# RaduAlexandru/permuto_sdf

Measured on AMD Instinct MI355X. Metric: ray-samples/sec (encode+MLP+composite), higher is better.
Workload: dtype f32 (MLP products on 2 fp16 operand pieces per fp32 value, fp32 accumulation; the 3-piece / 24-bit figure is value_fp32_equivalent_24bit)

## Files before the change

include/psdf.h:

```cpp
#ifndef PSDF_H
#define PSDF_H
#include <stdint.h>
#ifdef __cplusplus
extern "C" {
#endif

int64_t psdf_encode_convention(int which);
int psdf_encode_set_conventions(uint32_t hash_multiplier, int rank_tie_raises_later);

int psdf_encode_set_forward_pairs(int pairs);

int psdf_encode_forward(int pos_dim, int nr_feat, int64_t N, int nr_levels, int capacity, const float* positions,
    const float* lattice, const float* scale_factor, const float* shifts, const float* window, int concat_points,
    float points_scaling, float* sliced, void* stream);

int psdf_encode_forward_mark(int pos_dim, int nr_feat, int64_t N, int nr_levels, int capacity, const float* positions,
    const float* lattice, const float* scale_factor, const float* shifts, const float* window, int concat_points,
    float points_scaling, float* sliced, unsigned char* touched_blocks, int block_rows_log2, void* stream);

int psdf_encode_backward(int pos_dim, int nr_feat, int64_t N, int nr_levels, int capacity, const float* positions,
    const float* lattice, const float* scale_factor, const float* shifts, const float* window, int concat_points,
    float points_scaling, const float* grad_sliced, float* grad_lattice, float* grad_positions, void* stream);

int64_t psdf_encode_backward_workspace_bytes(int pos_dim, int nr_feat, int64_t N, int nr_levels, int capacity);
int psdf_encode_backward_ws(int pos_dim, int nr_feat, int64_t N, int nr_levels, int capacity, const float* positions,
    const float* lattice, const float* scale_factor, const float* shifts, const float* window, int concat_points,
    float points_scaling, const float* grad_sliced, float* grad_lattice, float* grad_positions, void* workspace,
    int64_t workspace_bytes, void* stream);
int psdf_encode_backward_level_shares(int* counts, int max_levels);


int psdf_encode_double_backward(int pos_dim, int nr_feat, int64_t N, int nr_levels, int capacity, const float*
    positions, const float* lattice, const float* scale_factor, const float* shifts, const float* window, int
    concat_points, float points_scaling, const float* dd_positions, const float* grad_sliced, float* grad_lattice,
    float* grad_grad_sliced, void* stream);
int psdf_encode_double_backward_ws(int pos_dim, int nr_feat, int64_t N, int nr_levels, int capacity, const float* positions,
                                   const float* lattice, const float* scale_factor, const float* shifts, const float* window,
                                   int concat_points, float points_scaling, const float* dd_positions, const float* grad_sliced,
                                   float* grad_lattice, float* grad_grad_sliced, const float* grad_sliced_direct,
                                   void* workspace, int64_t workspace_bytes, void* stream);

int psdf_mlp_pack_f16(int n_layers, const int* dims, const float* const* weights, const float* const* biases, float* packed,
    void* stream);
int psdf_mlp_forward_f16(int n_layers, const int* dims, int64_t N, const float* X, const float* packed, float* Y, void* stream);

int psdf_mlp_forward_set_form(int waves);
int psdf_mlp_forward_last_form(void);

int psdf_neus_composite_forward(int nr_rays, const int* start_end, int equal, int fixed, int max_nr_samples, const float* sdf,
    const float* dirs, const float* gradients, const float* dt, const float* rgb, const float* inv_s, float cos_anneal_ratio,
    float* pred, float* bg, float* weights, void* stream);
int psdf_neus_composite_backward(int nr_rays, const int* start_end, int equal, int fixed, int max_nr_samples, int max_per_ray,
    const float* grad_pred, const float* grad_bg, const float* sdf, const float* dirs, const float* gradients, const float* dt,
    const float* rgb, const float* inv_s, float cos_anneal_ratio, int reference_compat, float* grad_sdf, float* grad_gradients,
    float* grad_rgb, float* grad_inv_s, void* stream);

int psdf_nerf_composite_forward(int nr_rays, const int* start_end, int equal, int fixed, int max_nr_samples, const float* raw_density,
                                const float* dt, const float* rgb, const float* fg_pred, const float* fg_bg, float* pred_bg,
                                float* pred, void* stream);
int psdf_nerf_composite_backward(int nr_rays, const int* start_end, int equal, int fixed, int max_nr_samples, int max_per_ray,
                                 const float* grad_pred, const float* fg_bg, const float* raw_density, const float* dt,
                                 const float* rgb, int reference_compat, float* grad_raw_density, float* grad_rgb,
                                 float* grad_fg_bg, void* stream);

int psdf_last_path(int family);
enum {
  PSDF_MLP_OP_FORWARD = 0,
  PSDF_MLP_OP_FORWARD_F16 = 1,
  PSDF_MLP_OP_FORWARD_WIDE_F16 = 2,
  PSDF_MLP_OP_BACKWARD = 3,
  PSDF_MLP_OP_BACKWARD_DATA = 4,
  PSDF_MLP_OP_BACKWARD_DATA_MASKED = 5,
  PSDF_MLP_OP_DOUBLE_BACKWARD = 6,
  PSDF_MLP_OP_DOUBLE_BACKWARD_PLUS = 7
};
int psdf_mlp_supported(int op, int n_layers, const int* dims);

int psdf_mlp_backward_split(int n_layers, const int* dims, int64_t N, const float* X, const float* const* weights,
    const float* const* biases, const float* dY, float* dX, float* const* dW, float* const* db, void* stream);

int psdf_mlp_backward_split_f16(int n_layers, const int* dims, int64_t N, const float* X, const float* const* weights,
    const float* const* biases, const float* dY, float* dX, float* const* dW, float* const* db, void* stream);
int psdf_mlp_backward_split_f16_form(void);
unsigned psdf_mlp_f16_range_events(void);

int psdf_mlp_forward_wide_f16(int n_layers, const int* dims, int64_t N, const float* X, const float* const* weights,
    const float* const* biases, float* Y, void* stream);
int psdf_mlp_backward_wide_form(void);
int psdf_mlp_backward_wide(int n_layers, const int* dims, int64_t N, const float* X, const float* const* weights,
    const float* const* biases, const float* dY, float* dX, float* const* dW, float* const* db, void* stream);

int psdf_lipshitz_normalize_forward(int out, int in, const float* W, const float* c, float* Wn, void* stream);
int psdf_lipshitz_normalize_backward(int out, int in, const float* W, const float* c, const float* grad_Wn, float* grad_W,
    float* grad_c, void* stream);
int psdf_lipshitz_normalize_forward_multi(int n_layers, const int* out, const int* in, const float* const* W, const float* const* c,
                                          float* const* Wn, void* stream);
int psdf_lipshitz_normalize_backward_multi(int n_layers, const int* out, const int* in, const float* const* W, const float* const* c,
                                           const float* const* grad_Wn, float* const* grad_W, float* const* grad_c, void* stream);

int psdf_neus_alpha_forward(int64_t N, const float* sdf, const float* dirs, const float* gradients, const float* dt,
    const float* inv_s, float cos_anneal_ratio, float* alpha, float* one_minus_alpha, void* stream);
int psdf_neus_alpha_backward(int64_t N, const float* grad_alpha, const float* sdf, const float* dirs, const float*
    gradients, const float* dt, const float* inv_s, float cos_anneal_ratio, float* grad_sdf, float* grad_gradients,
    float* grad_inv_s, void* stream);
int psdf_l1_loss(int64_t R, int C, const float* pred, const float* gt, const unsigned char* mask, float scale,
    float* loss, float* grad_pred, void* stream);
int psdf_eikonal_loss(int64_t N, const float* gradients, float scale, float* loss, float* grad_gradients, void* stream);
int psdf_normalize3(int64_t N, const float* x, const float* grad_y, float* out, void* stream);
int psdf_sigmoid_rows(int64_t N, int C, const float* x_fm, float* y, void* stream);
int psdf_sigmoid_rows_backward(int64_t N, int C, const float* grad_y, const float* y, float* grad_x_fm, void* stream);
int psdf_curvature_shift(int64_t N, const float* points, const float* gradients, const float* rand_directions, float
    epsilon, const float* grad_shifted, float* out, void* stream);
int psdf_curvature_loss(int64_t N, const float* gradients, const float* gradients_shifted, float scale, float* loss,
    float* grad_gradients, float* grad_gradients_shifted, void* stream);
int psdf_offsurface_loss(int64_t N, const float* sdf, float sharpness, float scale, float* loss, float* grad_sdf, void*
    stream);
int psdf_nerf_alpha_forward(int64_t N, const float* raw_density, const float* dt, float* alpha, float* one_minus_alpha,
    void* stream);
int psdf_nerf_alpha_backward(int64_t N, const float* raw_density, const float* dt, const float* grad_alpha, const float*
    grad_one_minus_alpha, float* grad_raw_density, void* stream);

int64_t psdf_mlp_packed_size(int n_layers, const int* dims);

int psdf_mlp_pack(int n_layers, const int* dims, const float* const* weights, const float* const* biases, float*
    packed, void* stream);

int psdf_mlp_forward(int n_layers, const int* dims, int64_t N, const float* X, const float* packed, float* Y, void*
    stream);

int psdf_encode_forward_masked(int pos_dim, int nr_feat, int64_t N, int nr_levels, int capacity, const float* positions,
    const float* lattice, const float* scale_factor, const float* shifts, const float* window, int concat_points, float
    points_scaling, const uint8_t* skip, float* sliced, void* stream);
int psdf_mlp_forward_masked(int n_layers, const int* dims, int64_t N, const float* X, const float* packed, const uint8_t*
    skip, float* Y, void* stream);
int psdf_mlp_backward_data_masked(int n_layers, const int* dims, int64_t N, const float* X, const float* const* weights,
    const float* const* biases, const float* dY, const uint8_t* skip, float* dX, void* stream);
int psdf_encode_backward_positions_masked(int pos_dim, int nr_feat, int64_t N, int nr_levels, int capacity, const float*
    positions, const float* lattice, const float* scale_factor, const float* shifts, const float* window, int
    concat_points, float points_scaling, const float* grad_sliced, const uint8_t* skip, float* grad_positions, void*
    stream);

int psdf_mlp_backward(int n_layers, const int* dims, int64_t N, const float* X, const float* const* weights, const
    float* const* biases, const float* dY, float* dX, float* const* dW, float* const* db, void* stream);

int psdf_mlp_double_backward(int n_layers, const int* dims, int64_t N, const float* X, const float* const* weights,
    const float* const* biases, const float* dY, const float* V, float* dX2, float* const* dW, float* const* db,
    void* stream);
int psdf_mlp_double_backward_plus(int n_layers, const int* dims, int64_t N, const float* X, const float* const* weights,
    const float* const* biases, const float* dY, const float* V, const float* dY2, float* dX2, float* const* dW,
    float* const* db, void* stream);

int psdf_encode_mlp_forward(int64_t N, int nr_levels, int capacity, const float* positions, const float* lattice,
    const float* scale_factor, const float* shifts, const float* window, int concat_points, float points_scaling,
    int n_layers, const int* dims, const float* packed, const uint8_t* skip, float* feat, float* Y, void* stream);

int psdf_adamw_step(int64_t n, float* param, const float* grad, float* exp_avg, float* exp_avg_sq, float lr, float
    beta1, float beta2, float eps, float weight_decay, int step, float grad_scale, void* stream);

int psdf_adamw_step_multi(int n_tensors, const int64_t* sizes, float* const* params, const float* const* grads, float*
    const* exp_avgs, float* const* exp_avg_sqs, float lr, float beta1, float beta2, float eps, float weight_decay, int
    step, float grad_scale, void* stream);

int psdf_adamw_step_blocks(int64_t n_blocks, int block_elems, float* param, float* grad, float* exp_avg, float*
    exp_avg_sq, unsigned char* touched, unsigned char* active, float lr, float beta1, float beta2, float eps, int step,
    float grad_scale, int zero_grad, void* stream);
int psdf_adamw_step_blocks_multi(int n_tensors, const int64_t* n_blocks, const int* block_elems, float* const* params,
    float* const* grads, float* const* exp_avgs, float* const* exp_avg_sqs, unsigned char* const* touched,
// ... 219 lines not shown
```

permuto_sdf_amd/csrc/composite_fused.hip:

```cpp
#include <type_traits>

#include "composite_device.h"

using namespace psdf;

namespace {

__global__ void __launch_bounds__(PSDF_BLOCK)
    neus_composite_fwd_kernel(int nr_rays, RayIndex ri, const float* __restrict__ sdf, const float* __restrict__ dirs,
                              const float* __restrict__ gradients, const float* __restrict__ dt, const float* __restrict__ rgb,
                              const float* __restrict__ inv_s_ptr, float cos_anneal_ratio, float* __restrict__ pred,
                              float* __restrict__ bg, float* __restrict__ weights) {
  const int lane = lane_id();
  const float inv_s = inv_s_ptr[0];
  RAY_LOOP(ray, nr_rays) {
    int s, e;
    ri.get(ray, s, e);
    if (!ri.valid(s, e)) {
      if (lane == 0) {
        pred[3 * ray] = pred[3 * ray + 1] = pred[3 * ray + 2] = 0.f;
        if (bg) bg[ray] = 1.f;
      }
      continue;
    }
    float r = 0.f, g = 0.f, b = 0.f;
    const float T_bg = sweep(
        s, e - s, lane,
        [&](int64_t m) {
          return clip01(section(sdf[m], ld3(dirs + 3 * m), ld3(gradients + 3 * m), dt[m], inv_s, cos_anneal_ratio).q);
        },
        [&](int64_t m, float a, float T) {
          const float w = a * T;
          if (weights) weights[m] = w;
          r += w * rgb[3 * m];
          g += w * rgb[3 * m + 1];
          b += w * rgb[3 * m + 2];
        });
    r = wave_sum(r);
    g = wave_sum(g);
    b = wave_sum(b);
    if (lane == 0) {
      pred[3 * ray] = r;
      pred[3 * ray + 1] = g;
      pred[3 * ray + 2] = b;
      if (bg) bg[ray] = T_bg;
    }
  }
}

template <int K>
__global__ void __launch_bounds__(PSDF_BLOCK)
    neus_composite_bwd_kernel(int nr_rays, RayIndex ri, const float* __restrict__ g_pred, const float* __restrict__ g_bg,
                              const float* __restrict__ sdf, const float* __restrict__ dirs, const float* __restrict__ gradients,
                              const float* __restrict__ dt, const float* __restrict__ rgb, const float* __restrict__ inv_s_ptr,
                              float cos_anneal_ratio, int compat, float* __restrict__ g_sdf, float* __restrict__ g_gradients,
                              float* __restrict__ g_rgb, float* __restrict__ g_inv_s) {
  const int lane = lane_id();
  const float inv_s = inv_s_ptr[0], rr = cos_anneal_ratio;
  float gs_acc = 0.f;
  RAY_LOOP(ray, nr_rays) {
    int s, e;
    ri.get(ray, s, e);
    if (!ri.valid(s, e)) continue;
    const int n = e - s;
    if (n > 64 * K) {
      poison_ray(s, n, lane, [&](int64_t m, float bad) {
        g_sdf[m] = bad;
        if (g_rgb) g_rgb[3 * m] = g_rgb[3 * m + 1] = g_rgb[3 * m + 2] = bad;
        if (g_gradients) st3(g_gradients + 3 * m, mk3(bad, bad, bad));
      });
      continue;
    }
    const float gx = g_pred[3 * ray], gy = g_pred[3 * ray + 1], gz = g_pred[3 * ray + 2];
    float a_[K], T_[K], gw_[K], v_[K];
    Transmittance tr;
#pragma unroll
    for (int k = 0; k < K; k++) {
      a_[k] = T_[k] = gw_[k] = v_[k] = 0.f;
      if (64 * k >= n) continue;
      const Sample c = sweep_chunk(tr, s, n, 64 * k, lane, [&](int64_t m) {
        return clip01(section(sdf[m], ld3(dirs + 3 * m), ld3(gradients + 3 * m), dt[m], inv_s, rr).q);
      });
      if (c.in) {
        const float cx = rgb[3 * c.m], cy = rgb[3 * c.m + 1], cz = compat ? cy : rgb[3 * c.m + 2];
        const float w = c.a * c.T;
        const float gw = gx * cx + gy * cy + gz * cz;
        if (g_rgb) {
          g_rgb[3 * c.m] = gx * w;
          g_rgb[3 * c.m + 1] = gy * w;
          g_rgb[3 * c.m + 2] = gz * w;
        }
        a_[k] = c.a;
        T_[k] = c.T;
        gw_[k] = gw;
        v_[k] = (gw * c.a) * c.T;
      }
    }
    const float gb = (g_bg ? g_bg[ray] : 0.f) * tr.carry;
    SuffixStep sfx;
#pragma unroll
    for (int k = K - 1; k >= 0; k--) {
      if (64 * k >= n) continue;
      const int i = 64 * k + lane;
      const float g_om = sfx.g_one_minus(v_[k], a_[k], &gb, i, n, lane);
      if (i < n) {
        const int64_t m = s + i;
        const float g_alpha = gw_[k] * T_[k] - g_om;
        const v3 dir = ld3(dirs + 3 * m);
        const float d = dt[m];
        const Section sc = section(sdf[m], dir, ld3(gradients + 3 * m), d, inv_s, rr);
        const SectionGrad sg = section_backward(sc, g_alpha, d, inv_s, rr);
        gs_acc += sg.g_inv_s;
        g_sdf[m] = sg.g_sdf;
        if (g_gradients) st3(g_gradients + 3 * m, sg.g_tc * dir);
      }
    }
  }
  if (g_inv_s) {
    gs_acc = wave_sum(gs_acc);
    if (lane == 0 && gs_acc != 0.f) atomicAdd(g_inv_s, gs_acc);
  }
}

__global__ void __launch_bounds__(PSDF_BLOCK)
    nerf_composite_fwd_kernel(int nr_rays, RayIndex ri, const float* __restrict__ raw, const float* __restrict__ dt,
                              const float* __restrict__ rgb, const float* __restrict__ fg_pred, const float* __restrict__ fg_bg,
                              float* __restrict__ pred_bg, float* __restrict__ pred) {
  const int lane = lane_id();
  RAY_LOOP(ray, nr_rays) {
    int s, e;
    ri.get(ray, s, e);
    float r = 0.f, g = 0.f, b = 0.f;
    if (ri.valid(s, e)) {
      sweep(
          s, e - s, lane, [&](int64_t m) { return nerf_alpha(raw[m], dt[m]).a; },
          [&](int64_t m, float a, float T) {
            const float w = a * T;
            r += w * rgb[3 * m];
            g += w * rgb[3 * m + 1];
            b += w * rgb[3 * m + 2];
          });
      r = wave_sum(r);
      g = wave_sum(g);
      b = wave_sum(b);
    }
    if (lane == 0) {
      pred_bg[3 * ray] = r;
      pred_bg[3 * ray + 1] = g;
      pred_bg[3 * ray + 2] = b;
      if (pred) {
        const float t = fg_bg[ray];
        pred[3 * ray] = fg_pred[3 * ray] + t * r;
        pred[3 * ray + 1] = fg_pred[3 * ray + 1] + t * g;
        pred[3 * ray + 2] = fg_pred[3 * ray + 2] + t * b;
      }
    }
  }
}

template <int K>
__global__ void __launch_bounds__(PSDF_BLOCK)
    nerf_composite_bwd_kernel(int nr_rays, RayIndex ri, const float* __restrict__ g_pred, const float* __restrict__ fg_bg,
                              const float* __restrict__ raw, const float* __restrict__ dt, const float* __restrict__ rgb,
                              int compat, float* __restrict__ g_raw, float* __restrict__ g_rgb, float* __restrict__ g_fg_bg) {
  const int lane = lane_id();
  RAY_LOOP(ray, nr_rays) {
    int s, e;
    ri.get(ray, s, e);
    const float t = fg_bg ? fg_bg[ray] : 1.f;
    const float ux = g_pred[3 * ray], uy = g_pred[3 * ray + 1], uz = g_pred[3 * ray + 2];
    if (!ri.valid(s, e)) {
      if (g_fg_bg && lane == 0) g_fg_bg[ray] = 0.f;
      continue;
    }
    const int n = e - s;
    if (n > 64 * K) {
      poison_ray(s, n, lane, [&](int64_t m, float bad) {
        g_raw[m] = bad;
        g_rgb[3 * m] = g_rgb[3 * m + 1] = g_rgb[3 * m + 2] = bad;
      });
      if (g_fg_bg && lane == 0) g_fg_bg[ray] = poison();
      continue;
    }
    const float gx = t * ux, gy = t * uy, gz = t * uz;
    float a_[K], T_[K], gw_[K], v_[K], e_[K];
    float ex, pr = 0.f, pg = 0.f, pb = 0.f;
    Transmittance tr;
#pragma unroll
    for (int k = 0; k < K; k++) {
      a_[k] = T_[k] = gw_[k] = v_[k] = e_[k] = 0.f;
      if (64 * k >= n) continue;
      const Sample c = sweep_chunk(tr, s, n, 64 * k, lane, [&](int64_t m) {
        const NerfAlpha o = nerf_alpha(raw[m], dt[m]);
        ex = o.e;
        return o.a;
      });
      if (c.in) {
        const float cx = rgb[3 * c.m], cy = rgb[3 * c.m + 1], cz_true = rgb[3 * c.m + 2];
        const float cz = compat ? cy : cz_true;
        const float w = c.a * c.T;
        pr += w * cx;
        pg += w * cy;
        pb += w * cz_true;
// ... 4 lines not shown
        a_[k] = c.a;
        T_[k] = c.T;
        gw_[k] = gw;
        e_[k] = ex;
        v_[k] = (gw * c.a) * c.T;
      }
    }
    if (g_fg_bg) {
      pr = wave_sum(pr);
      pg = wave_sum(pg);
      pb = wave_sum(pb);
      if (lane == 0) g_fg_bg[ray] = (ux * pr + uy * pg) + uz * pb;
    }
    SuffixStep sfx;
#pragma unroll
    for (int k = K - 1; k >= 0; k--) {
      if (64 * k >= n) continue;
      const int i = 64 * k + lane;
      const float g_om = sfx.g_one_minus(v_[k], a_[k], nullptr, i, n, lane);
      if (i < n) {
        const int64_t m = s + i;
        const float g_alpha = gw_[k] * T_[k] - g_om;
        g_raw[m] = nerf_alpha_backward(g_alpha, e_[k], raw[m], dt[m]);
      }
    }
  }
}

template <int V>
using int_c = std::integral_constant<int, V>;
template <class Fn>
void dispatch_chunks(int max_per_ray, Fn&& fn) {
  if (max_per_ray <= 64) return fn(int_c<1>{});
  if (max_per_ray <= 128) return fn(int_c<2>{});
  return fn(int_c<4>{});
}

}

extern "C" {

int psdf_nerf_composite_forward(int nr_rays, const int* start_end, int equal, int fixed, int max_nr_samples, const float* raw_density,
                                const float* dt, const float* rgb, const float* fg_pred, const float* fg_bg, float* pred_bg,
                                float* pred, void* stream) {
  if (nr_rays <= 0) return PSDF_OK;
  if (!raw_density || !dt || !rgb || !pred_bg || (!equal && !start_end) || ((fg_pred || fg_bg || pred) && !(fg_pred && fg_bg && pred)))
    return PSDF_ERR_ARG;
  hipLaunchKernelGGL(nerf_composite_fwd_kernel, dim3(ray_grid(nr_rays)), dim3(PSDF_BLOCK), 0, (hipStream_t)stream, nr_rays,
                     RayIndex{start_end, equal, fixed, max_nr_samples}, raw_density, dt, rgb, fg_pred, fg_bg, pred_bg, pred);
  PSDF_LAUNCH_CHECK();
  return PSDF_OK;
}

int psdf_nerf_composite_backward(int nr_rays, const int* start_end, int equal, int fixed, int max_nr_samples, int max_per_ray,
                                 const float* grad_pred, const float* fg_bg, const float* raw_density, const float* dt,
                                 const float* rgb, int reference_compat, float* grad_raw_density, float* grad_rgb,
                                 float* grad_fg_bg, void* stream) {
  if (nr_rays <= 0) return PSDF_OK;
  if (!grad_pred || !raw_density || !dt || !rgb || !grad_raw_density || !grad_rgb || (!equal && !start_end) || max_per_ray < 1)
    return PSDF_ERR_ARG;
  if (max_per_ray > 256) return PSDF_ERR_UNSUPPORTED;
  const RayIndex ri{start_end, equal, fixed, max_nr_samples};
  dispatch_chunks(max_per_ray, [&](auto k) {
    hipLaunchKernelGGL(nerf_composite_bwd_kernel<decltype(k)::value>, dim3(ray_grid(nr_rays)), dim3(PSDF_BLOCK), 0,
                       (hipStream_t)stream, nr_rays, ri, grad_pred, fg_bg, raw_density, dt, rgb, reference_compat,
                       grad_raw_density, grad_rgb, grad_fg_bg);
  });
  PSDF_LAUNCH_CHECK();
  return PSDF_OK;
}

int psdf_neus_composite_forward(int nr_rays, const int* start_end, int equal, int fixed, int max_nr_samples, const float* sdf,
                                const float* dirs, const float* gradients, const float* dt, const float* rgb, const float* inv_s,
                                float cos_anneal_ratio, float* pred, float* bg, float* weights, void* stream) {
  if (nr_rays <= 0) return PSDF_OK;
  if (!sdf || !dirs || !gradients || !dt || !rgb || !inv_s || !pred || (!equal && !start_end)) return PSDF_ERR_ARG;
  hipLaunchKernelGGL(neus_composite_fwd_kernel, dim3(ray_grid(nr_rays)), dim3(PSDF_BLOCK), 0, (hipStream_t)stream, nr_rays,
                     RayIndex{start_end, equal, fixed, max_nr_samples}, sdf, dirs, gradients, dt, rgb, inv_s, cos_anneal_ratio,
                     pred, bg, weights);
  PSDF_LAUNCH_CHECK();
  return PSDF_OK;
}

int psdf_neus_composite_backward(int nr_rays, const int* start_end, int equal, int fixed, int max_nr_samples, int max_per_ray,
                                 const float* grad_pred, const float* grad_bg, const float* sdf, const float* dirs,
                                 const float* gradients, const float* dt, const float* rgb, const float* inv_s,
                                 float cos_anneal_ratio, int reference_compat, float* grad_sdf, float* grad_gradients,
                                 float* grad_rgb, float* grad_inv_s, void* stream) {
  if (nr_rays <= 0) return PSDF_OK;
  if (!grad_pred || !sdf || !dirs || !gradients || !dt || !rgb || !inv_s || !grad_sdf || (!equal && !start_end) || max_per_ray < 1)
    return PSDF_ERR_ARG;
  if (max_per_ray > 256) return PSDF_ERR_UNSUPPORTED;
  const RayIndex ri{start_end, equal, fixed, max_nr_samples};
  dispatch_chunks(max_per_ray, [&](auto k) {
    hipLaunchKernelGGL(neus_composite_bwd_kernel<decltype(k)::value>, dim3(ray_grid(nr_rays)), dim3(PSDF_BLOCK), 0,
                       (hipStream_t)stream, nr_rays, ri, grad_pred, grad_bg, sdf, dirs, gradients, dt, rgb, inv_s,
                       cos_anneal_ratio, reference_compat, grad_sdf, grad_gradients, grad_rgb, grad_inv_s);
  });
  PSDF_LAUNCH_CHECK();
  return PSDF_OK;
}

}
```

permuto_sdf_amd/csrc/mlp.hip:

```cpp
#include "psdf_common.h"
#include <type_traits>

#include "mlp_device.h"
#include "mlp_dispatch.h"

namespace {

struct PackArgs {
  MlpPlan plan;
  const float* W[MAXL];
  const float* b[MAXL];
};

__global__ void mlp_pack_kernel(PackArgs a, float* __restrict__ packed) {
  const int e = blockIdx.x * blockDim.x + threadIdx.x;
  const MlpPlan& p = a.plan;
  if (e >= p.total) return;
  int l = 0;
#pragma unroll
  for (int i = 1; i < MAXL; i++)
    if (i < p.n_layers && e >= p.w_off[i]) l = i;
  const int out_d = p.dims[l + 1], in_d = p.dims[l];
  const bool last = (l == p.n_layers - 1);
  float v = 0.f;
  if (e >= p.b_off[l]) {
    const int row = e - p.b_off[l];
    if (row < out_d) v = a.b[l][row];
  } else {
    const int q = e - p.w_off[l];
    int row, col;
    if (l == 0) {
      const int lane = q % WS, s = (q / WS) % p.in_steps0, to = (q / WS) / p.in_steps0;
      row = (lane < 64) ? 32 * to + (lane & 31) : (1 << 20);
      col = 2 * s + (lane >> 5);
    } else if (last && p.final_dot) {
      const int h = q & 1, r = (q >> 1) & 15, ti = (q >> 5) % p.tiles[l], o = (q >> 5) / p.tiles[l];
      row = o;
      col = 32 * ti + row_of(r, h);
    } else {
      const int j = q & 3, lane = (q >> 2) & 63, rq = (q >> 8) & 3, pr = q >> 10;
      const int r = 4 * rq + j, ti = pr % p.tiles[l], to = pr / p.tiles[l];
      row = 32 * to + (lane & 31);
      col = 32 * ti + row_of(r, lane >> 5);
    }
    if (row < out_d && col < in_d) v = a.W[l][(int64_t)row * in_d + col];
  }
  packed[e] = v;
}

__global__ void mlp_pack_split_kernel(PackArgs a, SplitPlan sp, float* __restrict__ packed, int f16) {
  const int w = blockIdx.x * blockDim.x + threadIdx.x;
  const MlpPlan& p = a.plan;
  if (w >= sp.total_rec * 4) return;
  uint32_t* dst = reinterpret_cast<uint32_t*>(packed + sp.base);
  const int nl = p.n_layers;
  const int rec = w >> 2;
  if (rec >= sp.tail_rec) {
    const int f = w - sp.tail_rec * 4;
    float v = 0.f;
    for (int l = 0; l < nl; l++) {
      const bool dot = (l == nl - 1) && p.final_dot;
      const int nb = dot ? 4 : p.tiles[l + 1] * 32;
      if (f >= sp.b_off[l] && f < sp.b_off[l] + nb) {
        const int row = f - sp.b_off[l];
        if (row < p.dims[l + 1]) v = a.b[l][row];
      }
      if (dot && f >= sp.wf_off && f < sp.wf_off + p.dims[nl] * p.tiles[l] * 32) {
        const int q = f - sp.wf_off;
        const int h = q & 1, r = (q >> 1) & 15, ti = (q >> 5) % p.tiles[l], o = (q >> 5) / p.tiles[l];
        const int col = 32 * ti + row_of(r, h);
        if (col < p.dims[l]) v = a.W[l][(int64_t)o * p.dims[l] + col];
      }
    }
    dst[w] = __float_as_uint(v);
    return;
  }
  int l = 0;
  for (int i = 1; i < nl; i++) {
    const bool dot = (i == nl - 1) && p.final_dot;
    if (!dot && rec >= sp.w_rec[i]) l = i;
  }
  const int local = rec - sp.w_rec[l];
  const int lane = local & 63, piece = (local >> 6) % 3, s = (local / 192) % sp.ns[l], to = (local / 192) / sp.ns[l];
  const int row = 32 * to + (lane & 31), hh = lane >> 5;
  uint32_t out = 0;
  for (int e = 0; e < 2; e++) {
    const int j = 2 * (w & 3) + e;
    const int col = l == 0 ? 16 * s + 8 * hh + j : 32 * (s >> 1) + row_of(8 * (s & 1) + j, hh);
    float v = 0.f;
    if (row < p.dims[l + 1] && col < p.dims[l]) v = a.W[l][(int64_t)row * p.dims[l] + col];
    uint32_t pc[3];
    if (f16) split2h_bits(v, pc);
    else split3(v, pc);
    out |= pc[piece] << (16 * e);
  }
  dst[w] = out;
}

template <int T1, int T2, int T3>
struct Net {
  static constexpr int NH = (T3 > 0) ? 3 : 2;
  static constexpr int TL = (T3 > 0) ? T3 : T2;
};

template <int T1, int T2, int T3, int OUT_T, bool FINAL_DOT>
__global__ void __launch_bounds__(PSDF_BLOCK, 2)
    mlp_fwd_kernel(MlpPlan p, int64_t N, const float* __restrict__ X, const float* __restrict__ packed,
                   const unsigned char* __restrict__ skip, float* __restrict__ Y) {
  extern __shared__ __align__(16) float lds[];
  for (int i = threadIdx.x; i < p.total; i += PSDF_BLOCK) lds[i] = packed[i];
  __syncthreads();
  const int lane = threadIdx.x & 63, wave = __builtin_amdgcn_readfirstlane((int)(threadIdx.x >> 6));
  const int h = lane >> 5, sl = lane & 31;
  const int K0 = p.dims[0];
  const int OUT = p.dims[p.n_layers];
  const int64_t ntiles = (N + 31) / 32;
  for (int64_t tile = (int64_t)blockIdx.x * 4 + wave; tile < ntiles; tile += (int64_t)gridDim.x * 4) {
    asm volatile("" ::: "memory");
    const int64_t n = tile * 32 + sl;
    const int64_t nc = n < N ? n : N - 1;
    if (skip && __ballot(n < N && !skip[nc]) == 0) continue;
    f32x16 h1[T1];
    init_bias<T1>(h1, lds + p.b_off[0], h);
    {
      const float* __restrict__ w0 = lds + p.w_off[0];
      const int steps = p.in_steps0;
      constexpr int XC = 16;
      for (int s0 = 0; s0 < steps; s0 += XC) {
        float xb[XC];
#pragma unroll
        for (int i = 0; i < XC; i++) {
          const int k = 2 * (s0 + i) + h;
          xb[i] = (s0 + i < steps && k < K0) ? X[(int64_t)k * N + nc] : 0.f;
        }
#pragma unroll
        for (int i = 0; i < XC; i++) {
          if (s0 + i < steps) {
#pragma unroll
            for (int to = 0; to < T1; to++)
              h1[to] = __builtin_amdgcn_mfma_f32_32x32x2f32(w0[(to * steps + s0 + i) * WS + lane], xb[i], h1[to], 0, 0, 0);
          }
        }
      }
    }
    apply_gelu<T1>(h1);
    f32x16 h2[T2];
    init_bias<T2>(h2, lds + p.b_off[1], h);
    dense_chain<T1, T2>(h1, h2, lds + p.w_off[1], lane);
    apply_gelu<T2>(h2);
    constexpr int TL = (T3 > 0) ? T3 : T2;
    f32x16 hl[TL];
    if constexpr (T3 > 0) {
      init_bias<T3>(hl, lds + p.b_off[2], h);
      dense_chain<T2, T3>(h2, hl, lds + p.w_off[2], lane);
      apply_gelu<T3>(hl);
    } else {
#pragma unroll
      for (int t = 0; t < T2; t++) hl[t] = h2[t];
    }
    const int lf = p.n_layers - 1;
    if constexpr (FINAL_DOT) {
      const float* __restrict__ wf = lds + p.w_off[lf];
      for (int o = 0; o < OUT; o++) {
        float acc = 0.f;
#pragma unroll
        for (int ti = 0; ti < TL; ti++)
#pragma unroll
          for (int r = 0; r < 16; r++) acc = fmaf(wf[((o * TL + ti) * 16 + r) * 2 + h], hl[ti][r], acc);
        acc += __shfl_xor(acc, 32, 64);
        acc += lds[p.b_off[lf] + o];
        if (h == 0 && n < N) Y[(int64_t)o * N + n] = acc;
      }
    } else {
      f32x16 y[OUT_T];
      init_bias<OUT_T>(y, lds + p.b_off[lf], h);
      dense_chain<TL, OUT_T>(hl, y, lds + p.w_off[lf], lane);
      if (n < N) {
#pragma unroll
        for (int to = 0; to < OUT_T; to++)
// ... 260 lines not shown
    return PSDF_ERR_UNSUPPORTED;
}

template <int T1, int T2, int T3, int OUT_T, bool FINAL_DOT, int CH, bool F16 = false>
int launch_fwd_split_ch(const MlpPlan& p, const SplitPlan& sp, int64_t N, const float* X, const float* packed,
                     const unsigned char* skip, float* Y, hipStream_t st) {
  constexpr bool WIDE = split_wide_built<T1, T2, T3, OUT_T, FINAL_DOT, SPLIT_WIDE_W>;
  int form = g_fwd_form_forced;
  if (form == 0) {
    const int64_t ntiles = (N + 31) / 32;
    form = WIDE && ntiles >= (int64_t)SPLIT_WIDE_MIN_TILES_PER_CU * mlp_device_cus() ? SPLIT_WIDE_W : 4;
  }
  if (form == 4)
    return launch_fwd_split_form<4, mlp_fwd_split_kernel<T1, T2, T3, OUT_T, FINAL_DOT, CH, F16>>(p, sp, N, X, packed, skip, Y, st);
  if (form == 8) return launch_fwd_split_wide<T1, T2, T3, OUT_T, FINAL_DOT, CH, F16, 8>(p, sp, N, X, packed, skip, Y, st);
  return launch_fwd_split_wide<T1, T2, T3, OUT_T, FINAL_DOT, CH, F16, 16>(p, sp, N, X, packed, skip, Y, st);
}

template <int T1, int T2, int T3, int OUT_T, bool FINAL_DOT>
int launch_fwd_split(const MlpPlan& p, const SplitPlan& sp, int64_t N, const float* X, const float* packed,
                     const unsigned char* skip, float* Y, hipStream_t st, bool f16 = false) {
  if constexpr (T1 == 2 && T2 == 2 && T3 == 2 && OUT_T == 1 && FINAL_DOT) {
    if (f16) {
      switch (sp.ns[0]) {
        case 1: return launch_fwd_split_ch<T1, T2, T3, OUT_T, FINAL_DOT, 1, true>(p, sp, N, X, packed, skip, Y, st);
        case 2: return launch_fwd_split_ch<T1, T2, T3, OUT_T, FINAL_DOT, 2, true>(p, sp, N, X, packed, skip, Y, st);
        case 3: return launch_fwd_split_ch<T1, T2, T3, OUT_T, FINAL_DOT, 3, true>(p, sp, N, X, packed, skip, Y, st);
        default: return launch_fwd_split_ch<T1, T2, T3, OUT_T, FINAL_DOT, 4, true>(p, sp, N, X, packed, skip, Y, st);
      }
    }
  } else if (f16) {
    return PSDF_ERR_UNSUPPORTED;
  }
  switch (sp.ns[0]) {
    case 1: return launch_fwd_split_ch<T1, T2, T3, OUT_T, FINAL_DOT, 1>(p, sp, N, X, packed, skip, Y, st);
    case 2: return launch_fwd_split_ch<T1, T2, T3, OUT_T, FINAL_DOT, 2>(p, sp, N, X, packed, skip, Y, st);
    case 3: return launch_fwd_split_ch<T1, T2, T3, OUT_T, FINAL_DOT, 3>(p, sp, N, X, packed, skip, Y, st);
    default: return launch_fwd_split_ch<T1, T2, T3, OUT_T, FINAL_DOT, 4>(p, sp, N, X, packed, skip, Y, st);
  }
}

template <int T1, int T2, int T3, int OUT_T, bool FINAL_DOT>
int launch_fwd(const MlpPlan& p, int64_t N, const float* X, const float* packed, const unsigned char* skip, float* Y,
               hipStream_t st) {
  const size_t shmem = (size_t)p.total * sizeof(float);
  auto kern = mlp_fwd_kernel<T1, T2, T3, OUT_T, FINAL_DOT>;
  if (!fwd_fits(p)) return PSDF_ERR_UNSUPPORTED;
  if (shmem > 64 * 1024) {
    hipError_t e = hipFuncSetAttribute((const void*)kern, hipFuncAttributeMaxDynamicSharedMemorySize, (int)shmem);
    if (e != hipSuccess) return (int)e;
  }
  const int64_t ntiles = (N + 31) / 32;
  int64_t blocks = (ntiles + 3) / 4;
  const int64_t cap = 256 * 4;
  if (blocks > cap) blocks = cap;
  hipLaunchKernelGGL(kern, dim3((unsigned)blocks), dim3(PSDF_BLOCK), shmem, st, p, N, X, packed, skip, Y);
  PSDF_LAUNCH_CHECK();
  return PSDF_OK;
}


}

extern "C" {

int64_t psdf_mlp_packed_size(int n_layers, const int* dims) {
  MlpPlan p;
  if (make_plan(n_layers, dims, p) != PSDF_OK) return PSDF_ERR_ARG;
  SplitPlan sp;
  make_split_plan(p, sp);
  return sp.ok ? (int64_t)sp.base + (int64_t)sp.total_rec * 4 : (int64_t)p.total;
}

static int mlp_pack_impl(int n_layers, const int* dims, const float* const* weights, const float* const* biases,
                         float* packed, void* stream, int f16) {
  PackArgs a;
  int rc = make_plan(n_layers, dims, a.plan);
  if (rc != PSDF_OK) return rc;
  if (f16 && !baseline_split_shape(n_layers, dims, 64, 4)) return PSDF_ERR_UNSUPPORTED;
  for (int l = 0; l < MAXL; l++) {
    a.W[l] = l < n_layers ? weights[l] : nullptr;
    a.b[l] = l < n_layers ? biases[l] : nullptr;
  }
  hipLaunchKernelGGL(mlp_pack_kernel, dim3(psdf_blocks(a.plan.total, 256)), dim3(256), 0, (hipStream_t)stream, a,
                     packed);
  PSDF_LAUNCH_CHECK();
  SplitPlan sp;
  make_split_plan(a.plan, sp);
  if (sp.ok) {
    hipLaunchKernelGGL(mlp_pack_split_kernel, dim3(psdf_blocks(sp.total_rec * 4, 256)), dim3(256), 0,
                       (hipStream_t)stream, a, sp, packed, f16);
    PSDF_LAUNCH_CHECK();
  } else if (f16) {
    return PSDF_ERR_UNSUPPORTED;
  }
  return PSDF_OK;
}

int psdf_mlp_pack(int n_layers, const int* dims, const float* const* weights, const float* const* biases,
                  float* packed, void* stream) {
  return mlp_pack_impl(n_layers, dims, weights, biases, packed, stream, 0);
}

int psdf_mlp_pack_f16(int n_layers, const int* dims, const float* const* weights, const float* const* biases,
                      float* packed, void* stream) {
  return mlp_pack_impl(n_layers, dims, weights, biases, packed, stream, 1);
}

static int mlp_forward_impl(int n_layers, const int* dims, int64_t N, const float* X, const float* packed,
                            const unsigned char* skip, float* Y, void* stream, bool f16 = false) {
  MlpPlan p;
  int rc = make_plan(n_layers, dims, p);
  if (rc != PSDF_OK) return rc;
  if (N == 0) return PSDF_OK;
  if (N < 0 || !X || !packed || !Y) return PSDF_ERR_ARG;
  hipStream_t st = (hipStream_t)stream;
  const int t1 = p.tiles[1], t2 = p.tiles[2], t3 = (n_layers == 4) ? p.tiles[3] : 0, to = p.tiles[n_layers];
  if (n_layers != 3 && n_layers != 4) return PSDF_ERR_UNSUPPORTED;
  if (f16 && !baseline_split_shape(n_layers, dims, 64, 4)) return PSDF_ERR_UNSUPPORTED;
  SplitPlan sp;
  make_split_plan(p, sp);
#define CASE(A, B, C, O, D, FWD, S, F16)                                        \
  PSDF_IF(FWD, if (t1 == A && t2 == B && t3 == C && to == O && p.final_dot == D) { \
    if (f16 && !F16) return PSDF_ERR_UNSUPPORTED;                               \
    if constexpr (S) {                                                          \
      if (sp.ok) {                                                              \
        psdf::g_last_path[psdf::PATH_MLP_FWD] = f16 ? 3 : 2;                    \
        return launch_fwd_split<A, B, C, O, D>(p, sp, N, X, packed, skip, Y, st, f16); \
      }                                                                         \
    }                                                                           \
    if (f16) return PSDF_ERR_UNSUPPORTED;                                       \
    psdf::g_last_path[psdf::PATH_MLP_FWD] = 1;                                  \
    return launch_fwd<A, B, C, O, D>(p, N, X, packed, skip, Y, st);             \
  })
  PSDF_MLP32_ROWS(CASE)
#undef CASE
  return PSDF_ERR_UNSUPPORTED;
}


int psdf_mlp_forward(int n_layers, const int* dims, int64_t N, const float* X, const float* packed, float* Y,
                     void* stream) {
  return mlp_forward_impl(n_layers, dims, N, X, packed, nullptr, Y, stream);
}

int psdf_mlp_forward_f16(int n_layers, const int* dims, int64_t N, const float* X, const float* packed, float* Y,
                         void* stream) {
  return mlp_forward_impl(n_layers, dims, N, X, packed, nullptr, Y, stream, true);
}

int psdf_mlp_forward_masked(int n_layers, const int* dims, int64_t N, const float* X, const float* packed,
                            const unsigned char* skip, float* Y, void* stream) {
  return mlp_forward_impl(n_layers, dims, N, X, packed, skip, Y, stream);
}

int psdf_mlp_forward_set_form(int waves) {
  if (waves != 0 && waves != 4 && waves != 8 && waves != 16) return PSDF_ERR_ARG;
  g_fwd_form_forced = waves;
  return PSDF_OK;
}

int psdf_mlp_forward_last_form(void) { return g_fwd_form_last; }

}
```

permuto_sdf_amd/csrc/mlp_bwd.hip:

```cpp
#include <cstdlib>
#include "mlp_device.h"
#include "mlp_dispatch.h"
#include <mutex>
#include <vector>

#define PSDF_MLP_BWD_SPLIT_DEFAULT 2
namespace psdf {
int g_last_path[PATH_FAMILIES] = {};
void* stream_scratch(size_t bytes, hipStream_t st) {
  hipStreamCaptureStatus cs = hipStreamCaptureStatusNone;
  if (hipStreamIsCapturing(st, &cs) != hipSuccess || cs != hipStreamCaptureStatusNone) {
    (void)hipGetLastError();
    return nullptr;
  }
  int dev = 0;
  if (hipGetDevice(&dev) != hipSuccess) return nullptr;
  struct Entry {
    hipStream_t st;
    int dev;
    void* ptr;
    size_t cap;
  };
  static std::mutex mu;
  static std::vector<Entry> entries;
// ... 1060 lines not shown
template <int TI0, int T1, int T2, int T3, int OUT_T, bool FINAL_DOT, bool WITH_DW, int NW_>
int launch_bwd_nw(const Plan16& p, int64_t N, const float* X, const float* dY, float* dX, const BwdPtrs& a, hipStream_t st) {
  constexpr int NW = NW_;
  const int64_t ntiles = (N + 15) / 16;
  int64_t blocks = (ntiles + NW - 1) / NW;
  if (blocks > 256) blocks = 256;
  if (!a.dW[0]) {
    if (!dX) return PSDF_OK;
    const size_t shmem = bwd_lds_bytes<TI0, T1, T2, T3, OUT_T, FINAL_DOT>(p, BW, 2);
    if (shmem > MLP_LDS_MAX) return PSDF_ERR_UNSUPPORTED;
    auto kern = mlp_bwd_kernel<TI0, T1, T2, T3, OUT_T, FINAL_DOT, true, false, BW>;
    hipError_t e = hipFuncSetAttribute((const void*)kern, hipFuncAttributeMaxDynamicSharedMemorySize, (int)shmem);
    if (e != hipSuccess) return (int)e;
    int64_t nb = (ntiles + BW - 1) / BW;
    if (nb > 512) nb = 512;
    hipLaunchKernelGGL(kern, dim3((unsigned)nb), dim3(BW * 64), shmem, st, p, N, X, dY, dX, a);
    PSDF_LAUNCH_CHECK();
    return PSDF_OK;
  }
  if constexpr (!WITH_DW) {
    return PSDF_ERR_UNSUPPORTED;
  } else {
  const size_t shmem = bwd_lds_bytes<TI0, T1, T2, T3, OUT_T, FINAL_DOT>(p, NW, 2);
  if (shmem > MLP_LDS_MAX) return PSDF_ERR_UNSUPPORTED;
#define GO(DX)                                                                                                     \
  do {                                                                                                             \
    auto kern = mlp_bwd_kernel<TI0, T1, T2, T3, OUT_T, FINAL_DOT, DX, true, NW>;                                    \
    hipError_t e = hipFuncSetAttribute((const void*)kern, hipFuncAttributeMaxDynamicSharedMemorySize, (int)shmem);  \
    if (e != hipSuccess) return (int)e;                                                                            \
    hipLaunchKernelGGL(kern, dim3((unsigned)blocks), dim3(NW * 64), shmem, st, p, N, X, dY, dX, ap);                 \
  } while (0)
  BwdPtrs ap = a;
  if (!a.only_if) ap.partial = grad_scratch_alloc((size_t)blocks * p.total, st);
  if (dX)
    GO(true);
  else
    GO(false);
#undef GO
  grad_scratch_reduce(p, ap, (int)blocks, st);
  PSDF_LAUNCH_CHECK();
  return PSDF_OK;
  }
}
template <int TI0, int T1, int T2, int T3, int OUT_T, bool FINAL_DOT, bool WITH_DW = true>
int launch_bwd(const Plan16& p, int64_t N, const float* X, const float* dY, float* dX, const BwdPtrs& a, hipStream_t st) {
  if constexpr (T1 <= 2 && T2 <= 2 && T3 <= 2) {
    if (N >= ((int64_t)1 << 17)) return launch_bwd_nw<TI0, T1, T2, T3, OUT_T, FINAL_DOT, WITH_DW, 8>(p, N, X, dY, dX, a, st);
  }
  return launch_bwd_nw<TI0, T1, T2, T3, OUT_T, FINAL_DOT, WITH_DW, BW>(p, N, X, dY, dX, a, st);
}

}

namespace psdf {
size_t mlp_backward_head_redo_bytes(int64_t N) {
  const int dims[4] = {80, 64, 64, 3};
  Plan16 p;
  if (make_plan16(3, dims, p) != PSDF_OK) return 0;
  int64_t blocks = ((N + 15) / 16 + BW - 1) / BW;
  if (blocks > 256) blocks = 256;
  return ((size_t)blocks * p.total * sizeof(float) + 255) & ~(size_t)255;
}
int mlp_backward_head_redo(const int* dims, int64_t N, const float* X, const float* const* weights, const float* const* biases,
                           const float* dY, float* dX, float* const* dW, float* const* db, hipStream_t st, char* scratch,
                           const uint32_t* only_if, uint32_t token) {
  Plan16 p;
  int rc = make_plan16(3, dims, p);
  if (rc != PSDF_OK) return rc;
  if (!colour_head_shape(3, dims)) return PSDF_ERR_UNSUPPORTED;
  BwdPtrs a;
  for (int l = 0; l < MAXL; l++) {
    a.W[l] = l < 3 ? weights[l] : nullptr;
    a.b[l] = l < 3 ? biases[l] : nullptr;
    a.dW[l] = l < 3 ? dW[l] : nullptr;
    a.db[l] = l < 3 ? db[l] : nullptr;
  }
  a.partial = reinterpret_cast<float*>(scratch);
  a.only_if = only_if;
  a.only_if_token = token;
  return launch_bwd_nw<5, 4, 4, 0, 1, true, true, BW>(p, N, X, dY, dX, a, st);
}
}

#ifdef PSDF_BWD_TIMING
extern "C" int psdf_debug_bwd_timing(unsigned long long* out) {
  return (int)hipMemcpyFromSymbol(out, HIP_SYMBOL(g_bwd_t), sizeof(unsigned long long) * 8);
}
#endif

extern "C" {

int psdf_mlp_backward_split(int n_layers, const int* dims, int64_t N, const float* X, const float* const* weights,
                            const float* const* biases, const float* dY, float* dX, float* const* dW, float* const* db,
                            void* stream);
int psdf_mlp_backward_wide(int n_layers, const int* dims, int64_t N, const float* X, const float* const* weights,
                           const float* const* biases, const float* dY, float* dX, float* const* dW, float* const* db,
                           void* stream);
int psdf_mlp_backward_split_f16(int n_layers, const int* dims, int64_t N, const float* X, const float* const* weights,
                                const float* const* biases, const float* dY, float* dX, float* const* dW, float* const* db,
                                void* stream);

int psdf_mlp_backward(int n_layers, const int* dims, int64_t N, const float* X, const float* const* weights,
                      const float* const* biases, const float* dY, float* dX, float* const* dW, float* const* db,
                      void* stream) {
  Plan16 p;
  int rc = make_plan16(n_layers, dims, p);
  if (rc != PSDF_OK) return rc;
  if (N == 0) return PSDF_OK;
  if (N < 0 || !X || !weights || !biases || ((dW == nullptr) != (db == nullptr))) return PSDF_ERR_ARG;
  if (!dY && dW) return PSDF_ERR_ARG;
  if (n_layers != 3 && n_layers != 4) return PSDF_ERR_UNSUPPORTED;
  if (dW && N >= (1 << 18)) {
    const char* v = getenv("PSDF_MLP_BWD_SPLIT");
    const int which = !v ? PSDF_MLP_BWD_SPLIT_DEFAULT : (v[0] == '0' ? 0 : (v[0] == 'f' ? 2 : 1));
    if (which == 2) {
      const int r = psdf_mlp_backward_split_f16(n_layers, dims, N, X, weights, biases, dY, dX, dW, db, stream);
      if (r != PSDF_ERR_UNSUPPORTED) {
        psdf::g_last_path[psdf::PATH_MLP_BWD] = 4;
        return r;
      }
    }
    if (which != 0) {
      const int r = psdf_mlp_backward_split(n_layers, dims, N, X, weights, biases, dY, dX, dW, db, stream);
      if (r != PSDF_ERR_UNSUPPORTED) {
        psdf::g_last_path[psdf::PATH_MLP_BWD] = 2;
        return r;
      }
    }
  }
  BwdPtrs a;
  a.partial = nullptr;
  for (int l = 0; l < MAXL; l++) {
    a.W[l] = l < n_layers ? weights[l] : nullptr;
    a.b[l] = l < n_layers ? biases[l] : nullptr;
    a.dW[l] = (dW && l < n_layers) ? dW[l] : nullptr;
    a.db[l] = (db && l < n_layers) ? db[l] : nullptr;
    if (l < n_layers && (!a.W[l] || !a.b[l] || (dW && (!a.dW[l] || !a.db[l])))) return PSDF_ERR_ARG;
  }
  hipStream_t st = (hipStream_t)stream;
  const int ti0 = p.tiles[0], t1 = p.tiles[1], t2 = p.tiles[2], t3 = (n_layers == 4) ? p.tiles[3] : 0,
            to = p.tiles[n_layers];
  if (dW && dX && colour_head_shape(n_layers, dims)) {
    const int r = psdf_mlp_backward_wide(n_layers, dims, N, X, weights, biases, dY, dX, dW, db, stream);
    if (r != PSDF_ERR_UNSUPPORTED) {
      psdf::g_last_path[psdf::PATH_MLP_BWD] = 3;
      return r;
    }
  }
  psdf::g_last_path[psdf::PATH_MLP_BWD] = 1;
#define CASE(I, A, B, C, O, D, DW, DX, MASKED, DBL, PLUS)                                        \
  if (ti0 == I && t1 == A && t2 == B && t3 == C && to == O && p.final_dot == D) {               \
    if (!DX && !dW) return PSDF_ERR_UNSUPPORTED;                                                \
    if (!DW && dW) {                                                                            \
      const int r = psdf_mlp_backward_wide(n_layers, dims, N, X, weights, biases, dY, dX, dW, db, stream); \
      if (r != PSDF_ERR_UNSUPPORTED) {                                                          \
        psdf::g_last_path[psdf::PATH_MLP_BWD] = 3;                                              \
        return r;                                                                               \
      }                                                                                         \
    }                                                                                           \
    return launch_bwd<I, A, B, C, O, D, DW != 0>(p, N, X, dY, dX, a, st);                       \
  }
  PSDF_MLP16_ROWS(CASE)
#undef CASE
  psdf::g_last_path[psdf::PATH_MLP_BWD] = 3;
  if (dW) return psdf_mlp_backward_wide(n_layers, dims, N, X, weights, biases, dY, dX, dW, db, stream);
  return PSDF_ERR_UNSUPPORTED;
}

int psdf_last_path(int family) {
  if (family < 0 || family >= psdf::PATH_FAMILIES) return -1;
  return psdf::g_last_path[family];
}

int psdf_mlp_supported(int op, int n_layers, const int* dims) {
  MlpPlan p;
  Plan16 q;
  if (op < PSDF_MLP_OP_FORWARD || op > PSDF_MLP_OP_DOUBLE_BACKWARD_PLUS || !dims || make_plan(n_layers, dims, p) != PSDF_OK ||
      make_plan16(n_layers, dims, q) != PSDF_OK)
    return PSDF_ERR_ARG;
  if (op == PSDF_MLP_OP_FORWARD_WIDE_F16) return colour_net_shape(n_layers, dims) || density_net_shape(n_layers, dims);
  if (n_layers != 3 && n_layers != 4) return 0;
  if (op == PSDF_MLP_OP_FORWARD || op == PSDF_MLP_OP_FORWARD_F16) {
    const bool f16 = op == PSDF_MLP_OP_FORWARD_F16;
    if (f16 && !baseline_split_shape(n_layers, dims, 64, 4)) return 0;
    SplitPlan sp;
    make_split_plan(p, sp);
    const int t1 = p.tiles[1], t2 = p.tiles[2], t3 = (n_layers == 4) ? p.tiles[3] : 0, to = p.tiles[n_layers];
#define ROW(A, B, C, O, D, FWD, S, F16)                                                            \
    if (FWD && t1 == A && t2 == B && t3 == C && to == O && p.final_dot == D)                       \
      return (S && sp.ok) ? (!f16 || F16) : (!f16 && fwd_fits(p));
    PSDF_MLP32_ROWS(ROW)
#undef ROW
    return 0;
  }
  const int ti0 = q.tiles[0], t1 = q.tiles[1], t2 = q.tiles[2], t3 = (n_layers == 4) ? q.tiles[3] : 0, to = q.tiles[n_layers];
#define ROW(I, A, B, C, O, D, DW, DX, MASKED, DBL, PLUS)                                           \
  if (ti0 == I && t1 == A && t2 == B && t3 == C && to == O && q.final_dot == D) {                  \
    const bool bwd = bwd_lds_bytes<I, A, B, C, O, D>(q, BW, 2) <= MLP_LDS_MAX;                     \
    const bool dbl = bwd_lds_bytes<I, A, B, C, O, D>(q, BW, 4) <= MLP_LDS_MAX;                     \
    switch (op) {                                                                                  \
      case PSDF_MLP_OP_BACKWARD: return DW ? bwd : wide_backward_shape(n_layers, dims);            \
      case PSDF_MLP_OP_BACKWARD_DATA: return DX && bwd;                                            \
      case PSDF_MLP_OP_BACKWARD_DATA_MASKED: return MASKED && bwd;                                 \
      case PSDF_MLP_OP_DOUBLE_BACKWARD: return DBL && dbl;                                         \
      default: return PLUS && dbl;                                                                 \
    }                                                                                              \
  }
  PSDF_MLP16_ROWS(ROW)
#undef ROW
  return op == PSDF_MLP_OP_BACKWARD && wide_backward_shape(n_layers, dims);
}

int psdf_mlp_backward_data_masked(int n_layers, const int* dims, int64_t N, const float* X, const float* const* weights,
                                  const float* const* biases, const float* dY, const unsigned char* skip, float* dX,
                                  void* stream) {
  Plan16 p;
  int rc = make_plan16(n_layers, dims, p);
  if (rc != PSDF_OK) return rc;
  if (N == 0) return PSDF_OK;
  if (N < 0 || !X || !weights || !biases || !dX) return PSDF_ERR_ARG;
  if (n_layers != 3 && n_layers != 4) return PSDF_ERR_UNSUPPORTED;
  BwdPtrs a;
  a.partial = nullptr;
  a.skip = skip;
  for (int l = 0; l < MAXL; l++) {
    a.W[l] = l < n_layers ? weights[l] : nullptr;
    a.b[l] = l < n_layers ? biases[l] : nullptr;
    a.dW[l] = nullptr;
    a.db[l] = nullptr;
    if (l < n_layers && (!a.W[l] || !a.b[l])) return PSDF_ERR_ARG;
  }
  hipStream_t st = (hipStream_t)stream;
  const int ti0 = p.tiles[0], t1 = p.tiles[1], t2 = p.tiles[2], t3 = (n_layers == 4) ? p.tiles[3] : 0,
            to = p.tiles[n_layers];
#define CASE(I, A, B, C, O, D, DW, DX, MASKED, DBL, PLUS)                                        \
  PSDF_IF(MASKED, if (ti0 == I && t1 == A && t2 == B && t3 == C && to == O && p.final_dot == D) \
    return launch_bwd<I, A, B, C, O, D>(p, N, X, dY, dX, a, st);)
  PSDF_MLP16_ROWS(CASE)
#undef CASE
  return PSDF_ERR_UNSUPPORTED;
}

static int mlp_double_backward_impl(int n_layers, const int* dims, int64_t N, const float* X, const float* const* weights,
                                    const float* const* biases, const float* dY, const float* V, const float* dY2, float* dX2,
                                    float* const* dW, float* const* db, void* stream) {
  Plan16 p;
  int rc = make_plan16(n_layers, dims, p);
  if (rc != PSDF_OK) return rc;
  if (n_layers != 4) return PSDF_ERR_UNSUPPORTED;
// ... 40 lines not shown
```

permuto_sdf_amd/csrc/mlp_bwd_split.hip:

```cpp
#include "mlp_split_layout.h"

namespace {

using IMG = SplitImage<3>;
constexpr uint32_t ONE_BF16 = 0x3F80u;

template <bool RATIONAL>
__device__ __forceinline__ void gelu_both(float z, float& hval, float& gprime) {
  if constexpr (RATIONAL) gelu_rational_both(z, hval, gprime);
  else gelu_erf(z, hval, gprime);
}

#define MFMA16(a, b, c) __builtin_amdgcn_mfma_f32_16x16x32_bf16((a), (b), (c), 0, 0, 0)

struct BP {
  bf16x8 p[3];
};
__device__ __forceinline__ uint32_t top_pair(float hi, float lo) {
  return __builtin_amdgcn_perm(__float_as_uint(hi), __float_as_uint(lo), 0x07060302u);
}
__device__ __forceinline__ f32x2 trunc_pair(f32x2 v) {
  return f32x2{__uint_as_float(__float_as_uint(v.x) & 0xFFFF0000u), __uint_as_float(__float_as_uint(v.y) & 0xFFFF0000u)};
}
__device__ __forceinline__ void split8(const float (&x)[8], BP& o) {
// ... 278 lines not shown
    if (dX) {
#pragma unroll
      for (int t = 0; t < NT0; t++)
#pragma unroll
        for (int r = 0; r < 4; r++) {
          const int k = 16 * t + 4 * g + r;
          if (k < K0 && live) dX[(int64_t)k * N + n] = dx[t][r];
        }
    }
  }
  asm volatile("s_waitcnt vmcnt(0)" ::: "memory");
  const int lane = lane_k, c = lane & 15, g = lane >> 4;
  __syncthreads();
  float* G = reinterpret_cast<float*>(lds);
  for (int e = threadIdx.x; e < G_TOTAL; e += NWAVES * 64) G[e] = 0.f;
  __syncthreads();
  for (int w = 0; w < NWAVES; w++) {
    if (wave == w) {
#pragma unroll
      for (int to = 0; to < NT; to++)
#pragma unroll
        for (int r = 0; r < 4; r++) {
          const int row = (16 * to + 4 * g + r) * 64;
#pragma unroll
          for (int ti = 0; ti < NT; ti++) {
            G[G_W2 + row + 16 * ti + c] += dW2[to][ti][r];
            G[G_W3 + row + 16 * ti + c] += dW3[to][ti][r];
          }
#pragma unroll
          for (int ti = 0; ti < NT0; ti++) G[G_W1 + row + 16 * ti + c] += dW1[to][ti][r];
        }
#pragma unroll
      for (int t = 0; t < NT; t++) {
        float v1 = db1[t], v2 = db2[t], v3 = db3[t], v4 = dw4[t];
        v1 += __shfl_xor(v1, 16, 64); v2 += __shfl_xor(v2, 16, 64); v3 += __shfl_xor(v3, 16, 64); v4 += __shfl_xor(v4, 16, 64);
        v1 += __shfl_xor(v1, 32, 64); v2 += __shfl_xor(v2, 32, 64); v3 += __shfl_xor(v3, 32, 64); v4 += __shfl_xor(v4, 32, 64);
        if (g == 0) {
          G[G_B1 + 16 * t + c] += v1;
          G[G_B2 + 16 * t + c] += v2;
          G[G_B3 + 16 * t + c] += v3;
          G[G_W4 + 16 * t + c] += v4;
        }
      }
      float b4 = db4;
      b4 += __shfl_xor(b4, 16, 64);
      b4 += __shfl_xor(b4, 32, 64);
      if (lane == 0) G[G_B4] += b4;
    }
    __syncthreads();
  }
  float* dst = partial + (size_t)blockIdx.x * G_TOTAL;
  for (int e = threadIdx.x; e < G_TOTAL; e += NWAVES * 64) dst[e] = G[e];
}

__global__ void mlp_split_reduce_kernel(const float* __restrict__ partial, int nimg, int K0, float* __restrict__ dW0,
                                        float* __restrict__ dW1, float* __restrict__ dW2, float* __restrict__ dW3,
                                        float* __restrict__ db0, float* __restrict__ db1, float* __restrict__ db2,
                                        float* __restrict__ db3, const uint32_t* __restrict__ only_if) {
  if (only_if && only_if[0] == 0u) return;
  const int e = blockIdx.x * blockDim.x + threadIdx.x;
  if (e >= G_TOTAL) return;
  float s = 0.f;
  for (int b = blockIdx.y; b < nimg; b += gridDim.y) s += partial[(size_t)b * G_TOTAL + e];
  if (e < G_W2) {
    const int o = e >> 6, k = e & 63;
    if (k < K0) atomicAdd(&dW0[o * K0 + k], s);
  } else if (e < G_W3) {
    atomicAdd(&dW1[e - G_W2], s);
  } else if (e < G_B1) {
    atomicAdd(&dW2[e - G_W3], s);
  } else if (e < G_B2) {
    atomicAdd(&db0[e - G_B1], s);
  } else if (e < G_B3) {
    atomicAdd(&db1[e - G_B2], s);
  } else if (e < G_W4) {
    atomicAdd(&db2[e - G_B3], s);
  } else if (e < G_B4) {
    atomicAdd(&dW3[e - G_W4], s);
  } else {
    atomicAdd(&db3[0], s);
  }
}

__device__ __forceinline__ void split3(float x, uint16_t (&p)[3]) {
  float r = x;
#pragma unroll
  for (int i = 0; i < 3; i++) {
    const uint32_t u = __float_as_uint(r);
    p[i] = (uint16_t)(u >> 16);
    r -= __uint_as_float(u & 0xFFFF0000u);
  }
}

template <int NT0>
__global__ void mlp_split_pack_kernel(int K0, const float* __restrict__ W0, const float* __restrict__ W1,
                                      const float* __restrict__ W2, const float* __restrict__ W3,
                                      const float* __restrict__ b0, const float* __restrict__ b1,
                                      const float* __restrict__ b2, const float* __restrict__ b3, uint16_t* __restrict__ rec,
                                      const uint32_t* __restrict__ only_if) {
  if (only_if && only_if[0] == 0u) return;
  const int t = blockIdx.x * blockDim.x + threadIdx.x;
  constexpr int PER_IMG = NT * 2 * 64, PER_T0 = NT0 * 2 * 64, NTHR = 5 * PER_IMG + PER_T0;
  if (t < NTHR) {
    const int im = t < 5 * PER_IMG ? t / PER_IMG : 5;
    const int q = t - im * PER_IMG;
    const int lane = q & 63, s = (q >> 6) & 1, tile = q >> 7;
    const int c = lane & 15, g = lane >> 4, row = 16 * tile + c;
    const int off[6] = {IMG::OFF_W0, IMG::OFF_W1, IMG::OFF_W2, IMG::OFF_T2, IMG::OFF_T1, IMG::OFF_T0};
    uint16_t out[3][8];
#pragma unroll
    for (int j = 0; j < 8; j++) {
      const float w = image_weight(im, row, s, g, j, K0, W0, W1, W2);
      uint16_t p[3];
      split3(w, p);
      out[0][j] = p[0]; out[1][j] = p[1]; out[2][j] = p[2];
    }
#pragma unroll
    for (int piece = 0; piece < 3; piece++) {
      uint16_t* dst = rec + ((size_t)(off[im] + ((tile * 2 + s) * 3 + piece) * 64 + lane)) * 8;
#pragma unroll
      for (int j = 0; j < 8; j++) dst[j] = out[piece][j];
    }
  } else {
    const int e = t - NTHR;
    float* tail = reinterpret_cast<float*>(rec + (size_t)IMG::off_f32(NT0) * 8);
    if (e < HID) tail[e] = b0[e];
    else if (e < 2 * HID) tail[e] = b1[e - HID];
    else if (e < 3 * HID) tail[e] = b2[e - 2 * HID];
    else if (e < 4 * HID) tail[e] = W3[e - 3 * HID];
    else if (e == 4 * HID) tail[e] = b3[0];
  }
}

}

namespace psdf {
int mlp_bwd_split_launch_double(unsigned blocks, size_t lds_bytes, hipStream_t st, int64_t N, int K0, int rows4, const float* X,
                                const float* dY, const void* rec, float* dX, float* partial, const uint32_t* only_if);
size_t mlp_backward_split_scratch_bytes(int K0, int64_t N);
int mlp_backward_split_impl(int n_layers, const int* dims, int64_t N, const float* X, const float* const* weights,
                            const float* const* biases, const float* dY, float* dX, float* const* dW, float* const* db,
                            hipStream_t st, char* scratch, const uint32_t* only_if);
}
#if defined(PSDF_SPLIT_TU_DOUBLE)
int psdf::mlp_bwd_split_launch_double(unsigned blocks, size_t lds_bytes, hipStream_t st, int64_t N, int K0, int rows4,
                                      const float* X, const float* dY, const void* rec, float* dX, float* partial,
                                      const uint32_t* only_if) {
  auto kern = mlp_bwd_split_kernel<3, true>;
  hipError_t e = hipFuncSetAttribute((const void*)kern, hipFuncAttributeMaxDynamicSharedMemorySize, (int)lds_bytes);
  if (e != hipSuccess) return (int)e;
  hipLaunchKernelGGL(kern, dim3(blocks), dim3(NWAVES * 64), lds_bytes, st, N, K0, rows4, X, dY,
                     reinterpret_cast<const u32x4*>(rec), dX, partial, only_if);
  return PSDF_OK;
}
#else

extern "C" {

int psdf_mlp_backward_split(int n_layers, const int* dims, int64_t N, const float* X, const float* const* weights,
                            const float* const* biases, const float* dY, float* dX, float* const* dW, float* const* db,
                            void* stream) {
  return psdf::mlp_backward_split_impl(n_layers, dims, N, X, weights, biases, dY, dX, dW, db, (hipStream_t)stream, nullptr, nullptr);
}

}

size_t psdf::mlp_backward_split_scratch_bytes(int K0, int64_t N) {
  return IMG::aligned(K0 <= 48 ? 3 : 4) + (size_t)split_blocks(N) * G_TOTAL * sizeof(float);
}
int psdf::mlp_backward_split_impl(int n_layers, const int* dims, int64_t N, const float* X, const float* const* weights,
                                  const float* const* biases, const float* dY, float* dX, float* const* dW, float* const* db,
                                  hipStream_t st, char* scratch, const uint32_t* only_if) {
  const int rc0 = split_check(n_layers, dims, 52 , N, X, weights, biases, dY, dW, db);
  if (rc0 != PSDF_OK) return rc0;
  const int K0 = dims[0];
  const int rows4 = (K0 + 3) & ~3;
  const int nt0 = K0 <= 48 ? 3 : 4;
  const size_t stage_bytes = (size_t)NWAVES * (rows4 * 16 + 64) * 4;
  const bool dbl = nt0 == 3 && IMG::aligned(3) + 2 * stage_bytes <= 160 * 1024;
  const size_t img_bytes = IMG::aligned(nt0);
  const size_t lds_bytes = img_bytes + (dbl ? 2 : 1) * stage_bytes;
  if (lds_bytes > 160 * 1024) return PSDF_ERR_UNSUPPORTED;
  const int64_t blocks = split_blocks(N);
  const size_t part_bytes = (size_t)blocks * G_TOTAL * sizeof(float);
  if (!scratch) scratch = (char*)psdf::stream_scratch(img_bytes + part_bytes, st);
  if (!scratch) return PSDF_ERR_UNSUPPORTED;
  uint16_t* rec = reinterpret_cast<uint16_t*>(scratch);
  float* partial = reinterpret_cast<float*>(scratch + img_bytes);
  const int pack_threads = (5 * NT + nt0) * 2 * 64 + TAIL_FLOATS;
#define PACK(NT0_)                                                                                                         \
  hipLaunchKernelGGL(mlp_split_pack_kernel<NT0_>, dim3((pack_threads + 255) / 256), dim3(256), 0, st, K0, weights[0],        \
                     weights[1], weights[2], weights[3], biases[0], biases[1], biases[2], biases[3], rec, only_if)
#define MAIN(NT0_, DBL_)                                                                                                    \
  do {                                                                                                                      \
    auto kern = mlp_bwd_split_kernel<NT0_, DBL_>;                                                                            \
    hipError_t e = hipFuncSetAttribute((const void*)kern, hipFuncAttributeMaxDynamicSharedMemorySize, (int)lds_bytes);       \
    if (e != hipSuccess) return (int)e;                                                                                     \
    hipLaunchKernelGGL(kern, dim3((unsigned)blocks), dim3(NWAVES * 64), lds_bytes, st, N, K0, rows4, X, dY,                  \
                       reinterpret_cast<const u32x4*>(rec), dX, partial, only_if);                                          \
  } while (0)
  if (nt0 == 3) {
    PACK(3);
    if (dbl) {
      const int rc = psdf::mlp_bwd_split_launch_double((unsigned)blocks, lds_bytes, st, N, K0, rows4, X, dY, rec, dX, partial, only_if);
      if (rc != PSDF_OK) return rc;
    } else {
      MAIN(3, false);
    }
  } else {
    PACK(4);
    MAIN(4, false);
  }
#undef PACK
#undef MAIN
  hipLaunchKernelGGL(mlp_split_reduce_kernel, dim3((G_TOTAL + 255) / 256, 16), dim3(256), 0, st, partial, (int)blocks, K0, dW[0],
                     dW[1], dW[2], dW[3], db[0], db[1], db[2], db[3], only_if);
  PSDF_LAUNCH_CHECK();
  return PSDF_OK;
}
#endif
```

permuto_sdf_amd/csrc/mlp_bwd_split_f16.hip:

```cpp
#include "mlp_split_layout.h"
#include <stdio.h>
#include <type_traits>
#include <stdlib.h>

namespace {

constexpr int NP = 2;
using IMG = SplitImage<NP>;
constexpr uint32_t ONE_F16 = 0x3C00u;


#define MFMA16(a, b, c) __builtin_amdgcn_mfma_f32_16x16x32_f16((a), (b), (c), 0, 0, 0)

struct BP {
  f16x8 p[NP];
};
__device__ __forceinline__ void split2(float x0, float x1, uint32_t& hi, uint32_t& lo) {
  float one = 1.0f;
  asm("" : "+s"(one));
  const h2v_t h2 = __builtin_convertvector(f32x2{x0, x1}, h2v_t);
  h2v_t l;
  l[0] = (_Float16)__builtin_fmaf(x0, one, -(float)h2[0]);
  l[1] = (_Float16)__builtin_fmaf(x1, one, -(float)h2[1]);
  hi = __builtin_bit_cast(uint32_t, h2);
// ... 353 lines not shown
    {
      const float dy_read = xb[OFF_DY + c];
      dy_parts(live ? dy_read : 0.f, dy, dy_pow2);
    }
#pragma unroll
    for (int t = 0; t < NT; t++) dz[t] = mul4(dz[t], mul4s(w4[t], dy));
    zero_init<NT>(a);
    layer_bwd<NT, NT, PAIR>(dz, a, lds + IMG::OFF_T2, lane, id, h2T, dW3, db3, rT);
#pragma unroll
    for (int t = 0; t < NT; t++) a[t] = mul4(a[t], GLDS ? gl[(NT + t) * 64] : g2[t]);
    if (tile + tstride < ntiles) prefetch(tile + tstride, stage + (cur ^ 1) * stage_floats);
    zero_init<NT>(dz);
    layer_bwd<NT, NT, PAIR>(a, dz, lds + IMG::OFF_T1, lane, id, h1T, dW2, db2, rT);
#pragma unroll
    for (int t = 0; t < NT; t++) dz[t] = mul4(dz[t], GLDS ? gl[t * 64] : g1[t]);
    f32x4 xT[NT0], dx[NT0];
#pragma unroll
    for (int u = 0; u < NT0; u++) {
      const int feat = 16 * u + c;
      xT[u] = *reinterpret_cast<const f32x4*>(xb + feat * 16 + 4 * g);
    }
    zero_init<NT0>(dx);
    layer_bwd<NT0, NT0, PAIR>(dz, dx, lds + IMG::OFF_T0, lane, id, xT, dW1, db1, rT);
    if (dX && live) {
      float* p0 = dX + (int64_t)(4 * g) * N + n;
#pragma unroll
      for (int t = 0; t < NT0; t++) {
        if (16 * (t + 1) <= K0) {
#pragma unroll
          for (int r = 0; r < 4; r++) p0[(int64_t)(16 * t + r) * N] = dx[t][r] * dy_pow2;
        } else if (16 * t < K0) {
#pragma unroll
          for (int r = 0; r < 4; r++)
            if (16 * t + 4 * g + r < K0) p0[(int64_t)(16 * t + r) * N] = dx[t][r] * dy_pow2;
        }
      }
    }
  }
  asm volatile("s_waitcnt vmcnt(0)" ::: "memory");
  if (out_of_range && lane_k == 0) atomicOr(absmax + 1, 1u);
  const int lane = lane_k, c = lane & 15, g = lane >> 4;
  __syncthreads();
  float* G = reinterpret_cast<float*>(lds);
  for (int e = threadIdx.x; e < G_TOTAL; e += NWAVES * 64) G[e] = 0.f;
  __syncthreads();
  for (int w = 0; w < NWAVES; w++) {
    if (wave == w) {
#pragma unroll
      for (int to = 0; to < NT; to++)
#pragma unroll
        for (int r = 0; r < 4; r++) {
          const int row = (16 * to + 4 * g + r) * 64;
#pragma unroll
          for (int ti = 0; ti < NT; ti++) {
            G[G_W2 + row + 16 * ti + c] += dW2[to][ti][r];
            G[G_W3 + row + 16 * ti + c] += dW3[to][ti][r];
          }
#pragma unroll
          for (int ti = 0; ti < NT0; ti++) G[G_W1 + row + 16 * ti + c] += dW1[to][ti][r];
        }
#pragma unroll
      for (int t = 0; t < NT; t++) {
        float v1 = db1[t].total(), v2 = db2[t].total(), v3 = db3[t].total(), v4 = dw4[t].total();
        v1 += __shfl_xor(v1, 16, 64); v2 += __shfl_xor(v2, 16, 64); v3 += __shfl_xor(v3, 16, 64); v4 += __shfl_xor(v4, 16, 64);
        v1 += __shfl_xor(v1, 32, 64); v2 += __shfl_xor(v2, 32, 64); v3 += __shfl_xor(v3, 32, 64); v4 += __shfl_xor(v4, 32, 64);
        if (g == 0) {
          G[G_B1 + 16 * t + c] += v1;
          G[G_B2 + 16 * t + c] += v2;
          G[G_B3 + 16 * t + c] += v3;
          G[G_W4 + 16 * t + c] += v4;
        }
      }
      float b4 = db4;
      b4 += __shfl_xor(b4, 16, 64);
      b4 += __shfl_xor(b4, 32, 64);
      if (lane == 0) G[G_B4] += b4;
    }
    __syncthreads();
  }
  float* dst = partial + (size_t)blockIdx.x * G_TOTAL;
  for (int e = threadIdx.x; e < G_TOTAL; e += NWAVES * 64) dst[e] = G[e];
}

__global__ void mlp_split_reduce_kernel(const float* __restrict__ partial, const uint32_t* __restrict__ absmax, int nimg, int K0, float* __restrict__ dW0,
                                        float* __restrict__ dW1, float* __restrict__ dW2, float* __restrict__ dW3,
                                        float* __restrict__ db0, float* __restrict__ db1, float* __restrict__ db2,
                                        float* __restrict__ db3, int guard_drops, volatile uint32_t* events) {
  const int e = blockIdx.x * blockDim.x + threadIdx.x;
  if (absmax[1]) {
    if (events && e == 0 && blockIdx.y == 0) events[0] = events[0] + 1u;
    if (guard_drops) return;
  }
  if (e >= G_TOTAL) return;
  float s = 0.f;
  for (int b = blockIdx.y; b < nimg; b += gridDim.y) s += partial[(size_t)b * G_TOTAL + e];
  float sc, isc;
  dy_scale(absmax[0], sc, isc);
  s *= isc;
  if (e < G_W4) s *= __uint_as_float((uint32_t)(127 - H_PRESCALE_EXP) << 23);
  if (e < G_W2) {
    const int o = e >> 6, k = e & 63;
    if (k < K0) atomicAdd(&dW0[o * K0 + k], s);
  } else if (e < G_W3) {
    atomicAdd(&dW1[e - G_W2], s);
  } else if (e < G_B1) {
    atomicAdd(&dW2[e - G_W3], s);
  } else if (e < G_B2) {
    atomicAdd(&db0[e - G_B1], s);
  } else if (e < G_B3) {
    atomicAdd(&db1[e - G_B2], s);
  } else if (e < G_W4) {
    atomicAdd(&db2[e - G_B3], s);
  } else if (e < G_B4) {
    atomicAdd(&dW3[e - G_W4], s);
  } else {
    atomicAdd(&db3[0], s);
  }
}

__global__ void __launch_bounds__(256) mlp_absmax_kernel(int64_t N, const float* __restrict__ dY, uint32_t* __restrict__ out) {
  uint32_t m = 0;
  const int64_t n4 = (((uintptr_t)dY & 15) == 0) ? (N >> 2) : 0;
  const uint4* __restrict__ p4 = reinterpret_cast<const uint4*>(dY);
  for (int64_t i = (int64_t)blockIdx.x * blockDim.x + threadIdx.x; i < n4; i += (int64_t)gridDim.x * blockDim.x) {
    const uint4 v = p4[i];
    const uint32_t a = v.x & 0x7FFFFFFFu, b = v.y & 0x7FFFFFFFu, c = v.z & 0x7FFFFFFFu, d = v.w & 0x7FFFFFFFu;
    const uint32_t ab = a > b ? a : b, cd = c > d ? c : d, q = ab > cd ? ab : cd;
    m = q > m ? q : m;
  }
  for (int64_t i = (n4 << 2) + (int64_t)blockIdx.x * blockDim.x + threadIdx.x; i < N; i += (int64_t)gridDim.x * blockDim.x) {
    const uint32_t b = __float_as_uint(dY[i]) & 0x7FFFFFFFu;
    m = b > m ? b : m;
  }
#pragma unroll
  for (int o = 32; o > 0; o >>= 1) {
    const uint32_t t = (uint32_t)__shfl_xor((int)m, o, 64);
    m = t > m ? t : m;
  }
  __shared__ uint32_t wmax[4];
  if ((threadIdx.x & 63) == 0) wmax[threadIdx.x >> 6] = m;
  __syncthreads();
  if (threadIdx.x == 0) {
    const uint32_t a = wmax[0] > wmax[1] ? wmax[0] : wmax[1], b = wmax[2] > wmax[3] ? wmax[2] : wmax[3];
    const uint32_t q = a > b ? a : b;
    if (q) atomicMax(out, q);
  }
}

template <int NT0>
__global__ void mlp_split_pack_kernel(int K0, const float* __restrict__ W0, const float* __restrict__ W1,
                                      const float* __restrict__ W2, const float* __restrict__ W3,
                                      const float* __restrict__ b0, const float* __restrict__ b1,
                                      const float* __restrict__ b2, const float* __restrict__ b3, uint32_t* __restrict__ rec,
                                      uint32_t* __restrict__ absmax) {
  const int t = blockIdx.x * blockDim.x + threadIdx.x;
  constexpr int PER_IMG = NT * 2 * 64, PER_T0 = NT0 * 2 * 64, NTHR = 5 * PER_IMG + PER_T0;
  if (t < NTHR) {
    const int im = t < 5 * PER_IMG ? t / PER_IMG : 5;
    const int q = t - im * PER_IMG;
    const int lane = q & 63, s = (q >> 6) & 1, tile = q >> 7;
    const int c = lane & 15, g = lane >> 4, row = 16 * tile + c;
    const int off[6] = {IMG::OFF_W0, IMG::OFF_W1, IMG::OFF_W2, IMG::OFF_T2, IMG::OFF_T1, IMG::OFF_T0};
    float w[8];
#pragma unroll
    for (int j = 0; j < 8; j++) w[j] = image_weight(im, row, s, g, j, K0, W0, W1, W2);
    u32x4 hi, lo;
    float wmax = 0.f;
#pragma unroll
    for (int i = 0; i < 4; i++) {
      uint32_t h, l;
      split2(w[2 * i], w[2 * i + 1], h, l);
      hi[i] = h;
      lo[i] = l;
      wmax = __builtin_fmaxf(__builtin_fmaxf(wmax, __builtin_fabsf(w[2 * i])), __builtin_fabsf(w[2 * i + 1]));
    }
    if (wmax >= 65504.f) atomicOr(absmax + 1, 1u);
    u32x4* dst = reinterpret_cast<u32x4*>(rec) + (off[im] + ((tile * 2 + s) * NP) * 64 + lane);
    dst[0] = hi;
    dst[64] = lo;
  } else {
    const int e = t - NTHR;
    float* tail = reinterpret_cast<float*>(rec + (size_t)IMG::off_f32(NT0) * 4);
    if (e < HID) tail[e] = b0[e];
    else if (e < 2 * HID) tail[e] = b1[e - HID];
    else if (e < 3 * HID) tail[e] = b2[e - 2 * HID];
    else if (e < 4 * HID) {
      tail[e] = W3[e - 3 * HID];
      if (__builtin_fabsf(W3[e - 3 * HID]) >= W4_LIMIT) atomicOr(absmax + 1, 1u);
    }
    else if (e == 4 * HID) tail[e] = b3[0];
  }
}

}

static int g_f16_form = 0;
namespace psdf {
size_t mlp_backward_split_scratch_bytes(int K0, int64_t N);
int mlp_backward_split_impl(int n_layers, const int* dims, int64_t N, const float* X, const float* const* weights,
                            const float* const* biases, const float* dY, float* dX, float* const* dW, float* const* db,
                            hipStream_t st, char* scratch, const uint32_t* only_if);
}
static uint32_t g_range_warned = 0;
static volatile uint32_t* range_events() {
  static uint32_t* dev_ptr = [] {
    uint32_t* h = nullptr;
    if (hipHostMalloc((void**)&h, 64, hipHostMallocMapped) != hipSuccess || !h) {
      (void)hipGetLastError();
      return (uint32_t*)nullptr;
    }
    h[0] = 0u;
    return h;
  }();
  return dev_ptr;
}

extern "C" {

int psdf_mlp_backward_split_f16_form(void) { return g_f16_form; }

int psdf_mlp_backward_split_f16(int n_layers, const int* dims, int64_t N, const float* X, const float* const* weights,
                                const float* const* biases, const float* dY, float* dX, float* const* dW, float* const* db,
                                void* stream) {
  const int rc0 = split_check(n_layers, dims, 64, N, X, weights, biases, dY, dW, db);
  if (rc0 != PSDF_OK) return rc0;
  const int K0 = dims[0];
  const int rows4 = (K0 + 3) & ~3;
  const int nt0 = K0 <= 48 ? 3 : 4;
  const size_t stage_bytes = (size_t)NWAVES * (64 * 16 + 64) * 4;
  const size_t img_bytes = IMG::aligned(nt0);
  const size_t g_bytes = nt0 == 3 ? (size_t)NWAVES * 2 * NT * 64 * 16 : 0;
  const size_t lds_bytes = img_bytes + 2 * stage_bytes + g_bytes;
  if (lds_bytes > 160 * 1024) return PSDF_ERR_UNSUPPORTED;
  hipStream_t st = (hipStream_t)stream;
  g_f16_form = 1;
  const int64_t blocks = split_blocks(N);
  const size_t part_bytes = ((size_t)blocks * G_TOTAL * sizeof(float) + 15) & ~(size_t)15;
  const bool guarded = K0 <= 52 && !getenv("PSDF_MLP_F16_NO_GUARD");
  const size_t fb_bytes = guarded ? psdf::mlp_backward_split_scratch_bytes(K0, N) : 0;
  char* scratch = (char*)psdf::stream_scratch(img_bytes + 16 + part_bytes + fb_bytes, st);
  if (!scratch) return PSDF_ERR_UNSUPPORTED;
  uint32_t* rec = reinterpret_cast<uint32_t*>(scratch);
  uint32_t* absmax = reinterpret_cast<uint32_t*>(scratch + img_bytes);
  float* partial = reinterpret_cast<float*>(scratch + img_bytes + 16);
  volatile uint32_t* events = range_events();
  if (events && events[0] != g_range_warned) {
    if (!g_range_warned)
      fprintf(stderr, "psdf: MLP inputs / activations beyond the split-fp16 range (|value| >= 255): such batches are redone by the "
                      "three-piece bf16 kernel (slower); PSDF_MLP_BWD_SPLIT=bf16 selects it outright\n");
    g_range_warned = events[0];
  }
  if (hipMemsetAsync(absmax, 0, 16, st) != hipSuccess) return PSDF_ERR_UNSUPPORTED;
  const int pack_threads = (5 * NT + nt0) * 2 * 64 + TAIL_FLOATS;
#define PACK(NT0_)                                                                                                         \
  hipLaunchKernelGGL(mlp_split_pack_kernel<NT0_>, dim3((pack_threads + 255) / 256), dim3(256), 0, st, K0, weights[0],        \
                     weights[1], weights[2], weights[3], biases[0], biases[1], biases[2], biases[3], rec, absmax)
#define MAIN(NT0_)                                                                                                          \
  do {                                                                                                                      \
    auto kern = mlp_bwd_split_f16_kernel<NT0_>;                                                                              \
    hipError_t e = hipFuncSetAttribute((const void*)kern, hipFuncAttributeMaxDynamicSharedMemorySize, (int)lds_bytes);       \
    if (e != hipSuccess) return (int)e;                                                                                     \
    hipLaunchKernelGGL(kern, dim3((unsigned)blocks), dim3(NWAVES * 64), lds_bytes, st, N, K0, rows4, X, dY,                  \
                       reinterpret_cast<const u32x4*>(rec), absmax, dX, partial);                                           \
  } while (0)
  if (nt0 == 3) PACK(3); else PACK(4);
  {
    int64_t ab = ((N >> 2) + 1023) / 1024;
    ab = ab < 1 ? 1 : (ab > 512 ? 512 : ab);
    hipLaunchKernelGGL(mlp_absmax_kernel, dim3((unsigned)ab), dim3(256), 0, st, N, dY, absmax);
  }
  if (nt0 == 3) MAIN(3); else MAIN(4);
#undef PACK
#undef MAIN
  hipLaunchKernelGGL(mlp_split_reduce_kernel, dim3((G_TOTAL + 255) / 256, 16), dim3(256), 0, st, partial, absmax, (int)blocks, K0,
                     dW[0], dW[1], dW[2], dW[3], db[0], db[1], db[2], db[3], guarded ? 1 : 0, events);
  PSDF_LAUNCH_CHECK();
  if (guarded) {
    const int rc = psdf::mlp_backward_split_impl(n_layers, dims, N, X, weights, biases, dY, dX, dW, db, st,
                                                 scratch + img_bytes + 16 + part_bytes, absmax + 1);
    if (rc != PSDF_OK) return rc;
  }
  return PSDF_OK;
}

unsigned psdf_mlp_f16_range_events(void) {
  volatile uint32_t* e = range_events();
  return e ? e[0] : 0u;
}

}
```

permuto_sdf_amd/csrc/mlp_split_layout.h:

```cpp
#pragma once
#include "psdf_common.h"
#include "mlp_dispatch.h"
#include "gelu_device.h"

namespace {

constexpr int HID = 64, NT = 4 ;
constexpr int NWAVES = 4;
__host__ __device__ inline int kf(int s, int g, int j) { return 32 * s + 16 * (j >> 2) + 4 * g + (j & 3); }

constexpr int TAIL_FLOATS = 3 * HID + HID + 1;
template <int NP>
struct SplitImage {
  static constexpr int RECL = NT * 2 * NP * 64;
  static constexpr int OFF_W0 = 0, OFF_W1 = RECL, OFF_W2 = 2 * RECL, OFF_T2 = 3 * RECL, OFF_T1 = 4 * RECL, OFF_T0 = 5 * RECL;
  static constexpr int off_f32(int nt0) { return 5 * RECL + nt0 * 2 * NP * 64; }
  static constexpr size_t aligned(int nt0) { return ((size_t)off_f32(nt0) * 16 + TAIL_FLOATS * 4 + 15) / 16 * 16; }
};
constexpr int G_W1 = 0, G_W2 = 4096, G_W3 = 8192, G_B1 = 12288, G_B2 = 12352, G_B3 = 12416, G_W4 = 12480, G_B4 = 12544,
              G_TOTAL = 12545;

__device__ __forceinline__ void step_operand(const f32x4 (&act)[NT], int s, float (&x)[8]) {
#pragma unroll
  for (int j = 0; j < 4; j++) {
    x[j] = act[2 * s][j];
    x[4 + j] = act[2 * s + 1][j];
  }
}
template <typename OP>
__device__ __forceinline__ OP halves(uint32_t a0, uint32_t a1, uint32_t b0, uint32_t b1) {
  const u32x4 q = {a0, a1, b0, b1};
  return __builtin_bit_cast(OP, q);
}
template <typename OP, uint32_t ONE>
__device__ __forceinline__ OP ident_op(int u, int lane) {
  const int c = lane & 15, g = lane >> 4;
  u32x4 q;
#pragma unroll
  for (int i = 0; i < 4; i++) {
    const int j0 = 2 * i, j1 = 2 * i + 1;
    const uint32_t lo = ((j0 >> 2) == u && 4 * g + (j0 & 3) == c) ? ONE : 0u;
    const uint32_t hi = ((j1 >> 2) == u && 4 * g + (j1 & 3) == c) ? ONE : 0u;
    q[i] = lo | (hi << 16);
  }
  return __builtin_bit_cast(OP, q);
}
__device__ __forceinline__ f32x4 zero4() { return f32x4{0.f, 0.f, 0.f, 0.f}; }
template <int NTILE>
__device__ __forceinline__ void bias_init(f32x4 (&acc)[NTILE], const float* __restrict__ b, int g) {
#pragma unroll
  for (int t = 0; t < NTILE; t++) acc[t] = *reinterpret_cast<const f32x4*>(b + 16 * t + 4 * g);
}
template <int NTILE>
__device__ __forceinline__ void zero_init(f32x4 (&acc)[NTILE]) {
#pragma unroll
  for (int t = 0; t < NTILE; t++) acc[t] = zero4();
}

__device__ __forceinline__ float image_weight(int im, int row, int s, int g, int j, int K0, const float* W0,
                                              const float* W1, const float* W2) {
  const int k0 = 32 * s + 8 * g + j, kc = kf(s, g, j);
  switch (im) {
    case 0: return k0 < K0 ? W0[row * K0 + k0] : 0.f;
    case 1: return W1[row * HID + kc];
    case 2: return W2[row * HID + kc];
    case 3: return W2[kc * HID + row];
    case 4: return W1[kc * HID + row];
    default: return row < K0 ? W0[kc * K0 + row] : 0.f;
  }
}

inline int64_t split_blocks(int64_t N) {
  const int64_t ntiles = (N + 15) / 16;
  const int64_t blocks = (ntiles + NWAVES - 1) / NWAVES;
  return blocks > 256 ? 256 : blocks;
}
inline int split_check(int n_layers, const int* dims, int max_k0, int64_t N, const float* X, const float* const* weights,
                       const float* const* biases, const float* dY, float* const* dW, float* const* db) {
  if (!dims || !dW || !db || !baseline_split_shape(n_layers, dims, max_k0, 1)) return PSDF_ERR_UNSUPPORTED;
  if (N <= 0 || !X || !weights || !biases || !dY) return PSDF_ERR_ARG;
  for (int l = 0; l < 4; l++)
    if (!weights[l] || !biases[l] || !dW[l] || !db[l]) return PSDF_ERR_ARG;
  return PSDF_OK;
}

}
```

permuto_sdf_amd/csrc/optim.hip:

```cpp
#include "psdf_common.h"

namespace {
__device__ __forceinline__ void adamw_range(int64_t n, float* __restrict__ p, const float* __restrict__ g,
                                            float* __restrict__ m, float* __restrict__ v, float lr, float beta1,
                                            float beta2, float eps, float weight_decay, float bias_corr1,
                                            float bias_corr2_sqrt, float grad_scale, int64_t first, int64_t stride) {
  for (int64_t i = first; i < n; i += stride) {
    if (i + 3 < n) {
      float4 P = *reinterpret_cast<float4*>(p + i);
      const float4 G = *reinterpret_cast<const float4*>(g + i);
      float4 M = *reinterpret_cast<float4*>(m + i);
      float4 V = *reinterpret_cast<float4*>(v + i);
      float* pp = &P.x;
      const float* gp = &G.x;
      float* mp = &M.x;
      float* vp = &V.x;
#pragma unroll
      for (int k = 0; k < 4; k++) {
        const float gk = gp[k] * grad_scale;
        pp[k] = pp[k] * (1.f - lr * weight_decay);
        mp[k] = beta1 * mp[k] + (1.f - beta1) * gk;
        vp[k] = beta2 * vp[k] + (1.f - beta2) * gk * gk;
        const float denom = sqrtf(vp[k]) / bias_corr2_sqrt + eps;
        pp[k] = pp[k] - (lr / bias_corr1) * (mp[k] / denom);
      }
      *reinterpret_cast<float4*>(p + i) = P;
      *reinterpret_cast<float4*>(m + i) = M;
      *reinterpret_cast<float4*>(v + i) = V;
    } else {
      for (int64_t j = i; j < n; j++) {
        const float gk = g[j] * grad_scale;
        float pj = p[j] * (1.f - lr * weight_decay);
        const float mj = beta1 * m[j] + (1.f - beta1) * gk;
        const float vj = beta2 * v[j] + (1.f - beta2) * gk * gk;
        const float denom = sqrtf(vj) / bias_corr2_sqrt + eps;
        pj = pj - (lr / bias_corr1) * (mj / denom);
        p[j] = pj;
        m[j] = mj;
        v[j] = vj;
      }
    }
  }
}

__global__ void __launch_bounds__(PSDF_BLOCK)
    adamw_kernel(int64_t n, float* __restrict__ p, const float* __restrict__ g, float* __restrict__ m,
                 float* __restrict__ v, float lr, float beta1, float beta2, float eps, float weight_decay,
                 float bias_corr1, float bias_corr2_sqrt, float grad_scale) {
  adamw_range(n, p, g, m, v, lr, beta1, beta2, eps, weight_decay, bias_corr1, bias_corr2_sqrt, grad_scale,
              ((int64_t)blockIdx.x * PSDF_BLOCK + threadIdx.x) * 4, (int64_t)gridDim.x * PSDF_BLOCK * 4);
}

constexpr int ADAMW_MAX_TENSORS = 64;
struct AdamwMulti {
  int64_t n[ADAMW_MAX_TENSORS];
  float* p[ADAMW_MAX_TENSORS];
  const float* g[ADAMW_MAX_TENSORS];
  float* m[ADAMW_MAX_TENSORS];
  float* v[ADAMW_MAX_TENSORS];
};
__global__ void __launch_bounds__(PSDF_BLOCK)
    adamw_multi_kernel(AdamwMulti a, float lr, float beta1, float beta2, float eps, float weight_decay, float bias_corr1,
                       float bias_corr2_sqrt, float grad_scale) {
  const int t = blockIdx.y;
  adamw_range(a.n[t], a.p[t], a.g[t], a.m[t], a.v[t], lr, beta1, beta2, eps, weight_decay, bias_corr1, bias_corr2_sqrt,
              grad_scale, ((int64_t)blockIdx.x * PSDF_BLOCK + threadIdx.x) * 4, (int64_t)gridDim.x * PSDF_BLOCK * 4);
}
__device__ __forceinline__ void adamw_blocks_body(int64_t n_blocks, int block_elems, float* __restrict__ p, float* __restrict__ g,
                        float* __restrict__ m, float* __restrict__ v, unsigned char* __restrict__ touched,
                        unsigned char* __restrict__ active, float lr, float beta1, float beta2, float eps, float bias_corr1,
                        float bias_corr2_sqrt, float grad_scale, int zero_grad) {
  const int lane = threadIdx.x & 63;
  for (int64_t b = (int64_t)blockIdx.x * (PSDF_BLOCK / 64) + (threadIdx.x >> 6); b < n_blocks;
       b += (int64_t)gridDim.x * (PSDF_BLOCK / 64)) {
    const unsigned char t = touched[b], a = active[b];
    if (!(t | a)) continue;
    if (lane == 0) {
      if (!a) active[b] = 1;
      if (t) touched[b] = 0;
    }
    const int64_t base = b * block_elems;
    for (int i = lane * 4; i < block_elems; i += 256) {
      float4 P = *reinterpret_cast<float4*>(p + base + i);
      float4 G = *reinterpret_cast<float4*>(g + base + i);
      float4 M = *reinterpret_cast<float4*>(m + base + i);
      float4 V = *reinterpret_cast<float4*>(v + base + i);
      float* pp = &P.x;
      const float* gp = &G.x;
      float* mp = &M.x;
      float* vp = &V.x;
#pragma unroll
      for (int k = 0; k < 4; k++) {
        const float gk = gp[k] * grad_scale;
        pp[k] = pp[k] * (1.f - lr * 0.f);
        mp[k] = beta1 * mp[k] + (1.f - beta1) * gk;
        vp[k] = beta2 * vp[k] + (1.f - beta2) * gk * gk;
        const float denom = sqrtf(vp[k]) / bias_corr2_sqrt + eps;
        pp[k] = pp[k] - (lr / bias_corr1) * (mp[k] / denom);
      }
      *reinterpret_cast<float4*>(p + base + i) = P;
      *reinterpret_cast<float4*>(m + base + i) = M;
      *reinterpret_cast<float4*>(v + base + i) = V;
      if (zero_grad) *reinterpret_cast<float4*>(g + base + i) = make_float4(0.f, 0.f, 0.f, 0.f);
    }
  }
}
__global__ void __launch_bounds__(PSDF_BLOCK)
    adamw_blocks_kernel(int64_t n_blocks, int block_elems, float* __restrict__ p, float* __restrict__ g,
                        float* __restrict__ m, float* __restrict__ v, unsigned char* __restrict__ touched,
                        unsigned char* __restrict__ active, float lr, float beta1, float beta2, float eps, float bias_corr1,
                        float bias_corr2_sqrt, float grad_scale, int zero_grad) {
  adamw_blocks_body(n_blocks, block_elems, p, g, m, v, touched, active, lr, beta1, beta2, eps, bias_corr1, bias_corr2_sqrt,
                    grad_scale, zero_grad);
}
constexpr int ADAMW_BLOCKS_MAX = 8;
struct AdamwBlocksMulti {
  int64_t n_blocks[ADAMW_BLOCKS_MAX];
  int block_elems[ADAMW_BLOCKS_MAX];
  float *p[ADAMW_BLOCKS_MAX], *g[ADAMW_BLOCKS_MAX], *m[ADAMW_BLOCKS_MAX], *v[ADAMW_BLOCKS_MAX];
  unsigned char *touched[ADAMW_BLOCKS_MAX], *active[ADAMW_BLOCKS_MAX];
  float lr[ADAMW_BLOCKS_MAX], beta1[ADAMW_BLOCKS_MAX], beta2[ADAMW_BLOCKS_MAX], eps[ADAMW_BLOCKS_MAX], bc1[ADAMW_BLOCKS_MAX],
      bc2[ADAMW_BLOCKS_MAX];
};
__global__ void __launch_bounds__(PSDF_BLOCK) adamw_blocks_multi_kernel(AdamwBlocksMulti a, float grad_scale, int zero_grad) {
  const int t = blockIdx.y;
  adamw_blocks_body(a.n_blocks[t], a.block_elems[t], a.p[t], a.g[t], a.m[t], a.v[t], a.touched[t], a.active[t], a.lr[t], a.beta1[t],
                    a.beta2[t], a.eps[t], a.bc1[t], a.bc2[t], grad_scale, zero_grad);
}
}

extern "C" {
int psdf_adamw_step_blocks(int64_t n_blocks, int block_elems, float* param, float* grad, float* exp_avg, float* exp_avg_sq,
                           unsigned char* touched, unsigned char* active, float lr, float beta1, float beta2, float eps,
                           int step, float grad_scale, int zero_grad, void* stream) {
  if (n_blocks <= 0) return PSDF_OK;
  if (!param || !grad || !exp_avg || !exp_avg_sq || !touched || !active || step < 1 || block_elems <= 0 || (block_elems & 3))
    return PSDF_ERR_ARG;
  if ((((uintptr_t)param | (uintptr_t)grad | (uintptr_t)exp_avg | (uintptr_t)exp_avg_sq) & 15) != 0) return PSDF_ERR_ARG;
  const float bc1 = 1.f - powf(beta1, (float)step);
  const float bc2 = sqrtf(1.f - powf(beta2, (float)step));
  unsigned blocks = psdf_blocks(n_blocks, PSDF_BLOCK / 64);
  if (blocks > 8192u) blocks = 8192u;
  hipLaunchKernelGGL(adamw_blocks_kernel, dim3(blocks), dim3(PSDF_BLOCK), 0, (hipStream_t)stream, n_blocks, block_elems,
                     param, grad, exp_avg, exp_avg_sq, touched, active, lr, beta1, beta2, eps, bc1, bc2, grad_scale, zero_grad);
  PSDF_LAUNCH_CHECK();
  return PSDF_OK;
}

int psdf_adamw_step_blocks_multi(int n_tensors, const int64_t* n_blocks, const int* block_elems, float* const* params,
                                 float* const* grads, float* const* exp_avgs, float* const* exp_avg_sqs,
                                 unsigned char* const* touched, unsigned char* const* active, const float* lr,
                                 const float* beta1, const float* beta2, const float* eps, const int* step, float grad_scale,
                                 int zero_grad, void* stream) {
  if (n_tensors <= 0) return PSDF_OK;
  if (n_tensors > ADAMW_BLOCKS_MAX || !n_blocks || !block_elems || !params || !grads || !exp_avgs || !exp_avg_sqs || !touched ||
      !active || !lr || !beta1 || !beta2 || !eps || !step)
    return PSDF_ERR_ARG;
  AdamwBlocksMulti a;
  int64_t most = 0;
  for (int t = 0; t < n_tensors; t++) {
    if (n_blocks[t] < 0 || !params[t] || !grads[t] || !exp_avgs[t] || !exp_avg_sqs[t] || !touched[t] || !active[t] || step[t] < 1 ||
        block_elems[t] <= 0 || (block_elems[t] & 3))
      return PSDF_ERR_ARG;
    if ((((uintptr_t)params[t] | (uintptr_t)grads[t] | (uintptr_t)exp_avgs[t] | (uintptr_t)exp_avg_sqs[t]) & 15) != 0) return PSDF_ERR_ARG;
    a.n_blocks[t] = n_blocks[t];
    a.block_elems[t] = block_elems[t];
    a.p[t] = params[t]; a.g[t] = grads[t]; a.m[t] = exp_avgs[t]; a.v[t] = exp_avg_sqs[t];
    a.touched[t] = touched[t]; a.active[t] = active[t];
    a.lr[t] = lr[t]; a.beta1[t] = beta1[t]; a.beta2[t] = beta2[t]; a.eps[t] = eps[t];
    a.bc1[t] = 1.f - powf(beta1[t], (float)step[t]);
    a.bc2[t] = sqrtf(1.f - powf(beta2[t], (float)step[t]));
    most = n_blocks[t] > most ? n_blocks[t] : most;
  }
  if (most == 0) return PSDF_OK;
  unsigned blocks = psdf_blocks(most, PSDF_BLOCK / 64);
  if (blocks > 8192u) blocks = 8192u;
  hipLaunchKernelGGL(adamw_blocks_multi_kernel, dim3(blocks, n_tensors), dim3(PSDF_BLOCK), 0, (hipStream_t)stream, a, grad_scale,
                     zero_grad);
  PSDF_LAUNCH_CHECK();
  return PSDF_OK;
}

int psdf_adamw_step(int64_t n, float* param, const float* grad, float* exp_avg, float* exp_avg_sq, float lr, float beta1,
                    float beta2, float eps, float weight_decay, int step, float grad_scale, void* stream) {
  if (n <= 0) return PSDF_OK;
  if (!param || !grad || !exp_avg || !exp_avg_sq || step < 1) return PSDF_ERR_ARG;
  if ((((uintptr_t)param | (uintptr_t)grad | (uintptr_t)exp_avg | (uintptr_t)exp_avg_sq) & 15) != 0) return PSDF_ERR_ARG;
  const float bc1 = 1.f - powf(beta1, (float)step);
  const float bc2 = sqrtf(1.f - powf(beta2, (float)step));
  unsigned blocks = psdf_blocks((n + 3) / 4, PSDF_BLOCK);
  if (blocks > 4096u) blocks = 4096u;
  hipLaunchKernelGGL(adamw_kernel, dim3(blocks), dim3(PSDF_BLOCK), 0, (hipStream_t)stream, n, param, grad, exp_avg,
                     exp_avg_sq, lr, beta1, beta2, eps, weight_decay, bc1, bc2, grad_scale);
  PSDF_LAUNCH_CHECK();
  return PSDF_OK;
}

int psdf_adamw_step_multi(int n_tensors, const int64_t* sizes, float* const* params, const float* const* grads,
                          float* const* exp_avgs, float* const* exp_avg_sqs, float lr, float beta1, float beta2, float eps,
                          float weight_decay, int step, float grad_scale, void* stream) {
  if (n_tensors <= 0) return PSDF_OK;
  if (n_tensors > ADAMW_MAX_TENSORS || !sizes || !params || !grads || !exp_avgs || !exp_avg_sqs || step < 1)
    return PSDF_ERR_ARG;
  AdamwMulti a;
  int64_t nmax = 0;
  for (int t = 0; t < n_tensors; t++) {
    if (sizes[t] < 0 || !params[t] || !grads[t] || !exp_avgs[t] || !exp_avg_sqs[t]) return PSDF_ERR_ARG;
    if ((((uintptr_t)params[t] | (uintptr_t)grads[t] | (uintptr_t)exp_avgs[t] | (uintptr_t)exp_avg_sqs[t]) & 15) != 0)
      return PSDF_ERR_ARG;
    a.n[t] = sizes[t];
    a.p[t] = params[t];
    a.g[t] = grads[t];
    a.m[t] = exp_avgs[t];
    a.v[t] = exp_avg_sqs[t];
    if (sizes[t] > nmax) nmax = sizes[t];
  }
  const float bc1 = 1.f - powf(beta1, (float)step);
  const float bc2 = sqrtf(1.f - powf(beta2, (float)step));
  unsigned blocks = psdf_blocks((nmax + 3) / 4, PSDF_BLOCK);
  if (blocks > 64u) blocks = 64u;
  hipLaunchKernelGGL(adamw_multi_kernel, dim3(blocks, (unsigned)n_tensors), dim3(PSDF_BLOCK), 0, (hipStream_t)stream, a, lr,
                     beta1, beta2, eps, weight_decay, bc1, bc2, grad_scale);
  PSDF_LAUNCH_CHECK();
  return PSDF_OK;
}
}
```

permuto_sdf_amd/hotpath.py:

```python
import torch

from . import _lib as L
from . import parallel
from .bridge import VolumeRendering as VR
from .encoding import PermutoEncoding, encode_backward_raw, encode_forward_raw
from .mlp import FusedMLP, f16_forward_supported, mlp_backward_raw, mlp_forward_raw, pack_params
from .neus import (FUSED_MAX_PER_RAY, neus_alpha_backward_raw, neus_alpha_forward_raw, neus_composite_backward_raw,
                   neus_composite_forward_raw)


class SdfHotPath:
    def __init__(self, nr_levels=16, hidden=64, out_channels=1, capacity=2 ** 18, device="cuda", seed=0, lr=1e-3):
        import numpy as np
        torch.manual_seed(seed)
        self.dev = torch.device(device)
        self.enc = PermutoEncoding(3, capacity, nr_levels, 2, np.geomspace(1.0, 1e-4, nr_levels),
                                   appply_random_shift_per_level=True, concat_points=True, concat_points_scaling=1e-3,
                                   init_scale=1e-2).to(self.dev)
        C = self.enc.output_dims()
        self.mlp = FusedMLP([C, hidden, hidden, hidden, out_channels]).to(self.dev)
        with torch.no_grad():
            self.mlp.layers[-1].bias.fill_(0.05)
        self.window = torch.ones(nr_levels, device=self.dev)
        self.inv_s = torch.full((1,), float(torch.exp(torch.tensor(5.0))), device=self.dev)
        self.cos_anneal_ratio = 1.0
        self.params = [self.enc.lattice_values] + [p for l in self.mlp.layers for p in (l.weight, l.bias)]
        from .optim import FusedAdamW
        self.opt = FusedAdamW(self.params, lr=lr)
        self.events = None
        self.fuse_compositing = True
        self.want_rgb_grad = True
        import os
        self.fwd_f16 = os.environ.get("PSDF_MLP_FWD_SPLIT", "f16") != "bf16"
        self.shard_optimizer = parallel.sharded_optimizer_default()
        self.last_dp = None

    @staticmethod
    def _max_per_ray(rs):
        if rs.rays_have_equal_nr_of_samples and 0 < int(rs.fixed_nr_of_samples_per_ray) <= FUSED_MAX_PER_RAY:
            return int(rs.fixed_nr_of_samples_per_ray)
        return None

    def forward(self, rs, rgb_samples, normals):
        cfg = self.enc.cfg
        pos = rs.samples_pos
        f16 = self.fwd_f16 and f16_forward_supported(self.mlp.dims)
        packed = pack_params(self.mlp.dims, [l.weight for l in self.mlp.layers], [l.bias for l in self.mlp.layers], f16=f16)
        feat = encode_forward_raw(cfg, pos, self.enc.lattice_values.detach(), self.enc.scale_factor,
                                  self.enc.random_shift_per_level.detach(), self.window)
        timed = self.events is not None and "mlp_fwd" in self.events
        if timed:
            self.events["mlp_fwd"][0].record()
        sdf = mlp_forward_raw(self.mlp.dims, feat, packed, f16=f16)
        if timed:
            self.events["mlp_fwd"][1].record()
        sdf_col = sdf.view(-1, 1)
        per_ray = self._max_per_ray(rs)
        if self.fuse_compositing and per_ray is not None:
            pred, bg, _ = neus_composite_forward_raw(rs, sdf_col, normals, rgb_samples, self.inv_s, self.cos_anneal_ratio)
            return pred, dict(feat=feat, packed=packed, sdf=sdf, bg=bg, normals=normals, fused_per_ray=per_ray)
        alpha, one_minus = neus_alpha_forward_raw(sdf_col, rs.samples_dirs, normals, rs.samples_dt, self.inv_s,
                                                  self.cos_anneal_ratio)
        T, bg = VR.cumprod_alpha2transmittance(rs, one_minus)
        w = alpha * T
        pred = VR.integrate_with_weights(rs, rgb_samples, w)
        return pred, dict(feat=feat, packed=packed, sdf=sdf, alpha=alpha, one_minus=one_minus, T=T, bg=bg, w=w,
                          normals=normals)

    def backward(self, rs, rgb_samples, saved, grad_pred, reduce=True, optimizer_step=True, split_levels=None):
        cfg = self.enc.cfg
        N = rs.samples_pos.shape[0]
        if "fused_per_ray" in saved:
            g_sdf, _, g_rgb, _ = neus_composite_backward_raw(rs, saved["fused_per_ray"], grad_pred, None, saved["sdf"].view(-1, 1),
                                                             saved["normals"], rgb_samples, self.inv_s, self.cos_anneal_ratio,
                                                             need_grad=False, need_rgb=self.want_rgb_grad, need_inv_s=False)
            g_om = g_alpha = None
        else:
            g_rgb, g_w = VR.integrate_with_weights_backward(grad_pred, rs, rgb_samples, saved["w"], None)
            g_T = g_w * saved["alpha"]
            cs = VR.cumsum_over_each_ray(rs, g_T * saved["T"], True)
            g_om = VR.cumprod_alpha2transmittance_backward(g_T, torch.zeros_like(saved["bg"]), rs, saved["one_minus"], saved["T"],
                                                           saved["bg"], cs)
            g_alpha = torch.addcmul(-g_om, g_w, saved["T"])
            g_sdf, _, _ = neus_alpha_backward_raw(g_alpha, saved["sdf"].view(-1, 1), rs.samples_dirs, saved["normals"],
                                                   rs.samples_dt, self.inv_s, self.cos_anneal_ratio, need_grad=False,
                                                   need_inv_s=False)
        grad_sdf = g_sdf.view(1, N)
        if self.events is not None:
            self.events["mlp_bwd"][0].record()
        d_feat, dWs, dbs = mlp_backward_raw(self.mlp.dims, saved["feat"], [l.weight for l in self.mlp.layers],
                                            [l.bias for l in self.mlp.layers], grad_sdf, need_dx=True)
        if self.events is not None:
            self.events["mlp_bwd"][1].record()
        buckets = parallel.GradientBuckets()
        su = parallel.ShardedUpdate()
        sharded = reduce and optimizer_step and self.shard_optimizer and parallel.collectives_active()
        lat_owned, lat_mine = [], []
        per_level = self.enc.lattice_values[0].numel()

        def reduce_lattice(l0, l1):
            if not reduce:
                return
            own = su.reduce_scatter(g_lat[l0:l1].view(-1), unit=4) if sharded else None
            base = l0 * per_level
            if own is None:
                buckets.reduce([g_lat[l0:l1]])
                if sharded:
                    lat_owned.append((base, l1 * per_level))
            else:
                n = (l1 - l0) * per_level
                lat_owned.extend((base + lo, base + hi) for lo, hi in
                                 (parallel.shard_bounds(n, 4, rank_=r) for r in su.virtual_ranks()))
                lat_mine.append((base, l1 * per_level, own))
        if reduce:
            buckets.reduce(dWs + dbs)
        g_lat = torch.zeros_like(self.enc.lattice_values)
        if self.events is not None:
            self.events["enc_bwd"][0].record()
        if split_levels is None:
            split_levels = reduce and parallel.collectives_active()
        if split_levels:
            L_ = cfg.nr_levels
            cut = max(1, min(L_ - 1, (3 * L_ + 4) // 8))
            for l0, l1 in ((0, cut), (cut, L_)):
                self._encode_backward_levels(rs.samples_pos, d_feat, g_lat, l0, l1)
                reduce_lattice(l0, l1)
        else:
            encode_backward_raw(cfg, rs.samples_pos, self.enc.lattice_values, self.enc.scale_factor,
                                self.enc.random_shift_per_level, self.window, d_feat, g_lat, None)
            reduce_lattice(0, cfg.nr_levels)
        if self.events is not None:
            self.events["enc_bwd"][1].record()
        if reduce:
            if self.events is not None and "comm_wait" in self.events:
                self.events["comm_wait"][0].record()
            buckets.finish()
            su.wait()
            if self.events is not None and "comm_wait" in self.events:
                self.events["comm_wait"][1].record()
            self.last_bucket_bytes = list(buckets.bytes) + list(su.bytes)
        grads = [g_lat] + [t for pair in zip(dWs, dbs) for t in pair]
        if optimizer_step:
            for p, g in zip(self.params, grads):
                p.grad = g
            lat = self.enc.lattice_values
            self.opt.step(grad_scale=1.0 / parallel.world_size(), owned={lat: lat_owned} if (sharded and lat_owned) else None)
            if sharded and lat_mine:
                flat = lat.data.view(-1)
                for b0, b1, own in lat_mine:
                    su.all_gather(flat[b0:b1], own)
                su.wait()
            self.last_dp = {"optimizer": "sharded" if (sharded and lat_mine) else "replicated"}
        return dict(g_rgb=g_rgb, g_one_minus=g_om, g_alpha=g_alpha, g_sdf=g_sdf, grads=grads)

    def _encode_backward_levels(self, pos, d_feat, g_lat, l0, l1):
        from .encoding import _Cfg
        c = self.enc.cfg
        sub = _Cfg(c.pos_dim, c.capacity, l1 - l0, c.nr_feat, False, 1.0)
        F = c.nr_feat
        encode_backward_raw(sub, pos, self.enc.lattice_values[l0:l1], self.enc.scale_factor[l0:l1],
                            self.enc.random_shift_per_level[l0:l1], self.window[l0:l1], d_feat[F * l0:F * l1],
                            g_lat[l0:l1], None)

    def step(self, rs, rgb_samples, normals, gt, **kw):
        from .neus import l1_loss_raw
        pred, saved = self.forward(rs, rgb_samples, normals)
        loss, g_pred = l1_loss_raw(pred, gt)
        out = self.backward(rs, rgb_samples, saved, g_pred, **kw)
        out["loss"] = loss
        return pred, saved, out
```

permuto_sdf_amd/mlp.py:

```python
import ctypes
import math

import torch

from . import _lib as L


def _dims_array(dims):
    return (ctypes.c_int * len(dims))(*dims)


def packed_size(dims):
    n = L.lib().psdf_mlp_packed_size
    n.restype = ctypes.c_int64
    r = n(L.c_i(len(dims) - 1), _dims_array(dims))
    if r < 0:
        raise L.PsdfError("psdf_mlp_packed_size: bad layer widths %s" % (dims,))
    return int(r)


(OP_FORWARD, OP_FORWARD_F16, OP_FORWARD_WIDE_F16, OP_BACKWARD, OP_BACKWARD_DATA, OP_BACKWARD_DATA_MASKED, OP_DOUBLE_BACKWARD,
 OP_DOUBLE_BACKWARD_PLUS) = range(8)
_SUPPORTED = {}

# ... 3 lines not shown
    r = _SUPPORTED.get(key)
    if r is None:
        r = _SUPPORTED[key] = L.lib().psdf_mlp_supported(L.c_i(op), L.c_i(len(dims) - 1), _dims_array(dims)) == 1
    return r


def f16_forward_supported(dims):
    return supported(OP_FORWARD_F16, dims)


def pack_params(dims, weights, biases, f16=False):
    n_layers = len(dims) - 1
    L.require_cuda(*weights)
    packed = torch.empty(packed_size(dims), dtype=torch.float32, device=weights[0].device)
    ws = [w.detach().contiguous() for w in weights]
    bs = [b.detach().contiguous() for b in biases]
    W = (ctypes.c_void_p * n_layers)(*[w.data_ptr() for w in ws])
    B = (ctypes.c_void_p * n_layers)(*[b.data_ptr() for b in bs])
    L.call("psdf_mlp_pack_f16" if f16 else "psdf_mlp_pack", L.c_i(n_layers), _dims_array(dims), W, B, L.ptr(packed), L.stream())
    return packed


def mlp_forward_raw(dims, x_fm, packed, skip=None, out=None, f16=False):
    N = x_fm.shape[1]
    y = out if out is not None else torch.empty((dims[-1], N), dtype=torch.float32, device=x_fm.device)
    if f16:
        assert skip is None
        L.call("psdf_mlp_forward_f16", L.c_i(len(dims) - 1), _dims_array(dims), L.c_l(N), L.ptr(x_fm), L.ptr(packed), L.ptr(y),
               L.stream())
    elif skip is None:
        L.call("psdf_mlp_forward", L.c_i(len(dims) - 1), _dims_array(dims), L.c_l(N), L.ptr(x_fm), L.ptr(packed), L.ptr(y),
               L.stream())
    else:
        L.call("psdf_mlp_forward_masked", L.c_i(len(dims) - 1), _dims_array(dims), L.c_l(N), L.ptr(x_fm), L.ptr(packed),
               L.ptr(skip), L.ptr(y), L.stream())
    return y


def set_forward_form(waves):
    L.call("psdf_mlp_forward_set_form", L.c_i(waves))


def last_forward_form():
    return int(L.lib().psdf_mlp_forward_last_form())


_wide_f16_fn = None


def mlp_forward_wide_f16_raw(dims, x_fm, weights, biases, out=None):
    global _wide_f16_fn
    if len(dims) != 5:
        return None
    if _wide_f16_fn is None:
        _wide_f16_fn = L.lib().psdf_mlp_forward_wide_f16
        _wide_f16_fn.restype = ctypes.c_int
    N = x_fm.shape[1]
    y = out if out is not None else torch.empty((dims[-1], N), dtype=torch.float32, device=x_fm.device)
    arr = lambda ts: (ctypes.c_void_p * 4)(*[t.data_ptr() for t in ts])
    ws = [w.detach() if w.is_contiguous() else w.detach().contiguous() for w in weights]
    bs = [b.detach() for b in biases]
    rc = _wide_f16_fn(L.c_i(4), _dims_array(dims), L.c_l(N), L.ptr(x_fm), arr(ws), arr(bs), L.ptr(y), L.stream())
    if rc == -2:
        return None
    if rc != 0:
        L.check(rc, "psdf_mlp_forward_wide_f16")
    return y


def _grad_views(dims, flat=None, dev=None):
    n_layers = len(dims) - 1
    sizes = [dims[l + 1] * dims[l] for l in range(n_layers)] + [dims[l + 1] for l in range(n_layers)]
    offs, tot = [], 0
    for sz in sizes:
        offs.append(tot)
        tot += (sz + 3) & ~3
    if flat is None:
        flat = torch.zeros(tot, dtype=torch.float32, device=dev)
    dWs = [flat[offs[l]:offs[l] + sizes[l]].view(dims[l + 1], dims[l]) for l in range(n_layers)]
    dbs = [flat[offs[n_layers + l]:offs[n_layers + l] + sizes[n_layers + l]] for l in range(n_layers)]
    return flat, dWs, dbs


def _zero_grads(dims, dev):
    _, dWs, dbs = _grad_views(dims, dev=dev)
    return dWs, dbs


class GradBuffer:

    def __init__(self, dims, device):
        self.flat, self.dWs, self.dbs = _grad_views(dims, dev=device)
        self.accumulating = False

    def accumulate(self):
        from .encoding import _Flag
        return _Flag(self, "accumulating")

    def zero(self):
        self.flat.zero_()


def mlp_backward_raw(dims, x_fm, weights, biases, gy_fm, need_dx=True, need_dw=True, into=None, dx=None):
    assert gy_fm is not None or not need_dw
    N = x_fm.shape[1]
    n_layers = len(dims) - 1
    dev = x_fm.device
    ws = [w.detach().contiguous() for w in weights]
    bs = [b.detach().contiguous() for b in biases]
    if not need_dx:
        dx = None
    elif dx is None:
        dx = torch.empty((dims[0], N), dtype=torch.float32, device=dev)
    else:
        assert dx.shape == (dims[0], N) and dx.dtype == torch.float32 and dx.is_contiguous() and dx.device == dev
    Wp = (ctypes.c_void_p * n_layers)(*[w.data_ptr() for w in ws])
    Bp = (ctypes.c_void_p * n_layers)(*[b.data_ptr() for b in bs])
    if need_dw:
        dWs, dbs = into if into is not None else _zero_grads(dims, dev)
        W = (ctypes.c_void_p * n_layers)(*[w.data_ptr() for w in dWs])
        B = (ctypes.c_void_p * n_layers)(*[b.data_ptr() for b in dbs])
    else:
        dWs, dbs, W, B = [], [], None, None
    L.call("psdf_mlp_backward", L.c_i(n_layers), _dims_array(dims), L.c_l(N), L.ptr(x_fm), Wp, Bp, L.ptr(gy_fm),
           L.ptr(dx), W, B, L.stream())
    return dx, dWs, dbs


def backward_supported(dims):
    return supported(OP_BACKWARD, dims)


_ANNOUNCED = set()


def torch_fallback_allowed(module=None):
    import os
    return bool(getattr(module, "allow_torch_fallback", False)) or os.environ.get("PSDF_MLP_TORCH_FALLBACK") == "1"


def _announce(kind, dims, module=None):
    if not torch_fallback_allowed(module):
        raise L.PsdfError("permuto_sdf_amd: no fused %s kernel is instantiated for the MLP widths %s (csrc/mlp_dispatch.h lists "
                          "the instantiated widths).  Refusing to fall back to torch/rocBLAS silently: pass allow_torch_fallback=True "
                          "to FusedMLP or set PSDF_MLP_TORCH_FALLBACK=1 to opt in." % (kind, list(dims)))
    key = (kind, tuple(dims))
    if key not in _ANNOUNCED:
        _ANNOUNCED.add(key)
        import warnings
        warnings.warn("permuto_sdf_amd: no fused %s kernel is instantiated for the MLP widths %s; using torch autograd over "
                      "rocBLAS on the GPU for it (csrc/mlp_dispatch.h lists the instantiated widths)" % (kind, list(dims)),
                      RuntimeWarning, stacklevel=3)


def _torch_gpu_backward(dims, x_fm, weights, biases, gy_fm, need_dx, module=None):
    _announce("backward", dims, module)
    n_layers = len(dims) - 1
    with torch.enable_grad():
        x = x_fm.t().detach().requires_grad_(need_dx)
        ws = [w.detach().requires_grad_(True) for w in weights]
        bs = [b.detach().requires_grad_(True) for b in biases]
        h = x
        for i in range(n_layers):
            h = torch.nn.functional.linear(h, ws[i], bs[i])
            if i < n_layers - 1:
                h = torch.nn.functional.gelu(h)
        outs = torch.autograd.grad(h, ([x] if need_dx else []) + ws + bs, gy_fm.t())
    k = 1 if need_dx else 0
    dx = outs[0].t().contiguous() if need_dx else None
    return dx, list(outs[k:k + n_layers]), list(outs[k + n_layers:])


def _torch_gpu_double_backward(dims, x_fm, weights, biases, gy_fm, v_fm, module=None):
    _announce("double backward", dims, module)
    n_layers = len(dims) - 1
    with torch.enable_grad():
        x = x_fm.t().detach().requires_grad_(True)
        ws = [w.detach().requires_grad_(True) for w in weights]
        bs = [b.detach().requires_grad_(True) for b in biases]
        h = x
        for i in range(n_layers):
            h = torch.nn.functional.linear(h, ws[i], bs[i])
            if i < n_layers - 1:
                h = torch.nn.functional.gelu(h)
        (gx,) = torch.autograd.grad(h, x, gy_fm.t(), create_graph=True)
        outs = torch.autograd.grad(gx, [x] + ws + bs, v_fm.t(), allow_unused=True)
    outs = [o if o is not None else torch.zeros_like(t) for o, t in zip(outs, [x] + ws + bs)]
    return outs[0].t().contiguous(), list(outs[1:1 + n_layers]), list(outs[1 + n_layers:])


class _InputGradOnly:

    def __init__(self, modules):
        self.modules = modules

    def __enter__(self):
        self.prev = [m._input_grad_only for m in self.modules]
        for m in self.modules:
            m._input_grad_only = True

    def __exit__(self, *exc):
        for m, v in zip(self.modules, self.prev):
            m._input_grad_only = v


def input_gradient_only(*modules):
# ... 315 lines not shown
```

permuto_sdf_amd/neus.py:

```python
import torch

from . import _lib as L


def neus_alpha_forward_raw(sdf, dirs, gradients, dt, inv_s, cos_anneal_ratio):
    N = sdf.shape[0]
    L.require_cuda(sdf, dirs, gradients, dt, inv_s)
    alpha = torch.empty((N, 1), dtype=torch.float32, device=sdf.device)
    one_minus = torch.empty((N, 1), dtype=torch.float32, device=sdf.device)
    L.call("psdf_neus_alpha_forward", L.c_l(N), L.ptr(sdf), L.ptr(dirs), L.ptr(gradients), L.ptr(dt), L.ptr(inv_s),
           L.c_f(float(cos_anneal_ratio)), L.ptr(alpha), L.ptr(one_minus), L.stream())
    return alpha, one_minus


def neus_alpha_backward_raw(g_alpha, sdf, dirs, gradients, dt, inv_s, cos_anneal_ratio, need_grad=True, need_inv_s=True):
    N = sdf.shape[0]
    g_sdf = torch.empty((N, 1), dtype=torch.float32, device=sdf.device)
    g_grad = torch.empty((N, 3), dtype=torch.float32, device=sdf.device) if need_grad else None
    g_inv_s = L.zeroed_scalar(sdf.device) if need_inv_s else None
    L.call("psdf_neus_alpha_backward", L.c_l(N), L.ptr(g_alpha), L.ptr(sdf), L.ptr(dirs), L.ptr(gradients), L.ptr(dt),
           L.ptr(inv_s), L.c_f(float(cos_anneal_ratio)), L.ptr(g_sdf), L.ptr(g_grad), L.ptr(g_inv_s), L.stream())
    return g_sdf, g_grad, g_inv_s


def _c(t):
    return t.detach().to(torch.float32).contiguous()


class NeusAlphaFunc(torch.autograd.Function):
    @staticmethod
    def forward(ctx, sdf, dirs, gradients, dt, inv_s, cos_anneal_ratio):
        sdf_c, dirs_c, grad_c, dt_c = _c(sdf).view(-1, 1), _c(dirs), _c(gradients), _c(dt).view(-1, 1)
        inv_s_c = _c(inv_s).view(1)
        alpha, one_minus = neus_alpha_forward_raw(sdf_c, dirs_c, grad_c, dt_c, inv_s_c, cos_anneal_ratio)
        ctx.save_for_backward(sdf_c, dirs_c, grad_c, dt_c, inv_s_c)
        ctx.r = float(cos_anneal_ratio)
        ctx.inv_s_shape = inv_s.shape
        return alpha, one_minus

    @staticmethod
    def backward(ctx, g_alpha, g_one_minus):
        sdf, dirs, grad, dt, inv_s = ctx.saved_tensors
        g = g_alpha if g_one_minus is None else (g_alpha - g_one_minus if g_alpha is not None else -g_one_minus)
        g_sdf, g_grad, g_inv_s = neus_alpha_backward_raw(g.contiguous(), sdf, dirs, grad, dt, inv_s, ctx.r,
                                                          need_grad=ctx.needs_input_grad[2],
                                                          need_inv_s=ctx.needs_input_grad[4])
        return (g_sdf if ctx.needs_input_grad[0] else None, None, g_grad, None,
                g_inv_s.view(ctx.inv_s_shape) if g_inv_s is not None else None, None)


def neus_alpha(sdf, dirs, gradients, dt, inv_s, cos_anneal_ratio):
    return NeusAlphaFunc.apply(sdf, dirs, gradients, dt, inv_s, cos_anneal_ratio)


def neus_composite_forward_raw(rs, sdf, gradients, rgb, inv_s, cos_anneal_ratio, want_weights=False):
    R, N, dev = rs.ray_start_end_idx.shape[0], sdf.shape[0], sdf.device
    L.require_cuda(sdf, gradients, rgb, inv_s)
    pred = torch.empty((R, 3), dtype=torch.float32, device=dev)
    bg = torch.empty((R, 1), dtype=torch.float32, device=dev)
    w = torch.zeros((N, 1), dtype=torch.float32, device=dev) if want_weights else None
    L.call("psdf_neus_composite_forward", *rs._ri(), L.ptr(sdf), L.ptr(rs.samples_dirs), L.ptr(gradients), L.ptr(rs.samples_dt),
           L.ptr(rgb), L.ptr(inv_s), L.c_f(float(cos_anneal_ratio)), L.ptr(pred), L.ptr(bg), L.ptr(w), L.stream())
    return pred, bg, w


def neus_composite_backward_raw(rs, max_per_ray, g_pred, g_bg, sdf, gradients, rgb, inv_s, cos_anneal_ratio, need_grad=True,
                                need_rgb=True, need_inv_s=True):
    from .bridge import VolumeRendering, _per_sample
    N, dev = sdf.shape[0], sdf.device
    g_sdf = _per_sample(rs, (N, 1), dev)
    g_grad = _per_sample(rs, (N, 3), dev) if need_grad else None
    g_rgb = _per_sample(rs, (N, 3), dev) if need_rgb else None
    g_inv_s = L.zeroed_scalar(dev) if need_inv_s else None
    L.call("psdf_neus_composite_backward", *rs._ri(), L.c_i(int(max_per_ray)), L.ptr(g_pred), L.ptr(g_bg), L.ptr(sdf),
           L.ptr(rs.samples_dirs), L.ptr(gradients), L.ptr(rs.samples_dt), L.ptr(rgb), L.ptr(inv_s),
           L.c_f(float(cos_anneal_ratio)), L.c_i(int(VolumeRendering.reference_compat)), L.ptr(g_sdf), L.ptr(g_grad),
           L.ptr(g_rgb), L.ptr(g_inv_s), L.stream())
    return g_sdf, g_grad, g_rgb, g_inv_s


FUSED_MAX_PER_RAY = 256


class NeusCompositeFunc(torch.autograd.Function):

    @staticmethod
    def forward(ctx, rs, max_per_ray, sdf, gradients, rgb, inv_s, cos_anneal_ratio):
        sdf_c, grad_c, rgb_c, inv_s_c = _c(sdf).view(-1, 1), _c(gradients), _c(rgb), _c(inv_s).view(1)
        pred, bg, _ = neus_composite_forward_raw(rs, sdf_c, grad_c, rgb_c, inv_s_c, cos_anneal_ratio)
        ctx.save_for_backward(sdf_c, grad_c, rgb_c, inv_s_c)
        ctx.rs, ctx.max_per_ray, ctx.r, ctx.inv_s_shape = rs, int(max_per_ray), float(cos_anneal_ratio), inv_s.shape
        return pred, bg

    @staticmethod
    def backward(ctx, g_pred, g_bg):
        sdf, grad, rgb, inv_s = ctx.saved_tensors
        need = ctx.needs_input_grad
        g_sdf, g_grad, g_rgb, g_inv_s = neus_composite_backward_raw(
            ctx.rs, ctx.max_per_ray, g_pred.contiguous(), None if g_bg is None else g_bg.contiguous(), sdf, grad, rgb, inv_s, ctx.r,
            need_grad=need[3], need_rgb=need[4], need_inv_s=need[5])
        return (None, None, g_sdf if need[2] else None, g_grad, g_rgb,
                g_inv_s.view(ctx.inv_s_shape) if g_inv_s is not None else None, None)


def neus_composite(rs, max_per_ray, sdf, gradients, rgb, inv_s, cos_anneal_ratio):
    return NeusCompositeFunc.apply(rs, max_per_ray, sdf, gradients, rgb, inv_s, cos_anneal_ratio)


def l1_loss_raw(pred, gt, mask=None, scale=None, want_grad=True, loss=None):
    L.require_cuda(pred, gt)
    R, C = pred.shape
    scale = 1.0 / max(1, R * C) if scale is None else float(scale)
    loss = L.zeroed_scalar(pred.device) if loss is None else loss
    g = torch.empty_like(pred) if want_grad else None
    m = None if mask is None else mask.reshape(-1).to(torch.uint8).contiguous()
    L.call("psdf_l1_loss", L.c_l(R), L.c_i(C), L.ptr(pred.contiguous()), L.ptr(gt.contiguous()), L.ptr(m), L.c_f(scale),
           L.ptr(loss), L.ptr(g), L.stream())
    return loss, g


def eikonal_loss_raw(gradients, scale=None, want_grad=True, loss=None):
    N = gradients.shape[0]
    scale = 1.0 / max(1, N) if scale is None else float(scale)
    loss = L.zeroed_scalar(gradients.device) if loss is None else loss
    g = torch.empty_like(gradients) if want_grad else None
    L.call("psdf_eikonal_loss", L.c_l(N), L.ptr(gradients.contiguous()), L.c_f(scale), L.ptr(loss), L.ptr(g), L.stream())
    return loss, g


class _L1Loss(torch.autograd.Function):
    @staticmethod
    def forward(ctx, pred, gt, mask):
        loss, g = l1_loss_raw(pred.detach(), gt.detach(), mask)
        ctx.save_for_backward(g)
        return loss.view(())

    @staticmethod
    def backward(ctx, go):
        (g,) = ctx.saved_tensors
        return g * go, None, None


class _EikonalLoss(torch.autograd.Function):

    @staticmethod
    def forward(ctx, gradients):
        loss, g = eikonal_loss_raw(gradients.detach())
        ctx.save_for_backward(g)
        return loss.view(())

    @staticmethod
    def backward(ctx, go):
        (g,) = ctx.saved_tensors
        return g * go


def l1_loss(pred, gt, mask=None):
    return _L1Loss.apply(pred, gt, mask)


def eikonal_loss(gradients):
# ... 175 lines not shown
```

permuto_sdf_amd/optim.py:

```python
import torch

from . import _lib as L


class FusedAdamW(torch.optim.Optimizer):
    def __init__(self, params, lr=1e-3, betas=(0.9, 0.99), eps=1e-15, weight_decay=0.0):
        super().__init__(params, dict(lr=lr, betas=betas, eps=eps, weight_decay=weight_decay))
        self.generation = 0

    SMALL = 1 << 16

    def attach(self, param, touched_rows):
        if not hasattr(self, "_touched"):
            self._touched = {}
        self._touched[param] = touched_rows
        self._rebuild_active(param)

    def _rebuild_active(self, param):
        tr = self._touched[param]
        st = self.state.get(param)
        if not st or "exp_avg" not in st:
            tr.active.zero_()
            return
        nz = (st["exp_avg"] != 0) | (st["exp_avg_sq"] != 0)
        tr.active.copy_(nz.reshape(tr.touched.numel(), tr.block_elems).any(dim=1).view_as(tr.active).to(torch.uint8))

    def load_state_dict(self, state_dict):
        super().load_state_dict(state_dict)
        self.__dict__.pop("_small_ok", None)
        for p in getattr(self, "_touched", {}):
            self._rebuild_active(p)
        self._moments_loaded = True

    def state_dict(self, allow_partial=False):
        sharded = getattr(self, "_sharded_params", None)
        if sharded and not allow_partial:
            from . import parallel
            if parallel.world_size() > 1:
                raise L.PsdfError("FusedAdamW.state_dict(): %d parameter(s) are updated sharded over %d ranks -- this rank holds only "
                                  "its own ranges' moments; save parallel.consolidated_state_dict(optimizer) instead"
                                  % (len(sharded), parallel.world_size()))
        return super().state_dict()

    @torch.no_grad()
    def step(self, grad_scale=1.0, owned=None):
        import ctypes
        owned = owned or {}
        if owned:
            if not hasattr(self, "_sharded_params"):
                self._sharded_params = set()
                self._sharded_ranges = {}
            self._sharded_params.update(owned.keys())
            for p, ranges in owned.items():
                ranges = sorted((int(lo), int(hi)) for lo, hi in ranges)
                if self._sharded_ranges.get(p) != ranges or getattr(self, "_moments_loaded", False):
                    st = self.state.get(p)
                    if st and "exp_avg" in st:
                        for k in ("exp_avg", "exp_avg_sq"):
                            f, prev = st[k].view(-1), 0
                            for lo, hi in ranges + [(f.numel(), f.numel())]:
                                if lo > prev:
                                    f[prev:lo].zero_()
                                prev = max(prev, hi)
                    self._sharded_ranges[p] = ranges
            self._moments_loaded = False
        self.generation += 1
        blocks_pending = []
        touched_rows = getattr(self, "_touched", {})
        small_cache = self.__dict__.setdefault("_small_ok", {})
        for group in self.param_groups:
            b1, b2 = group["betas"]
            small = {}
            for p in group["params"]:
                tr = touched_rows.get(p)
                if tr is not None:
                    st = self.state[p]
                    if not st:
                        st["step"] = 0
                        st["exp_avg"] = torch.zeros_like(p)
                        st["exp_avg_sq"] = torch.zeros_like(p)
                    st["step"] += 1
                    if p.grad is not None:
                        tr.grad.add_(p.grad)
                        p.grad = None
                    be = tr.block_elems
                    ranges = owned.get(p, [(0, p.numel())])
                    pf, gf, mf, vf = p.view(-1), tr.grad.view(-1), st["exp_avg"].view(-1), st["exp_avg_sq"].view(-1)
                    tf, af = tr.touched.view(-1), tr.active.view(-1)
                    for lo, hi in ranges:
                        if lo % be or hi % be:
                            raise L.PsdfError("owned ranges of a touched-rows parameter must be aligned to its row blocks")
                        blo, bhi = lo // be, hi // be
                        if lo == 0 and hi == pf.numel() and group["weight_decay"] == 0.0:
                            blocks_pending.append((bhi, be, pf, gf, mf, vf, tf, af, group["lr"], b1, b2, group["eps"], st["step"]))
                            continue
                        if group["weight_decay"] != 0.0:
                            L.call("psdf_adamw_step", L.c_l(hi - lo), L.ptr(pf[lo:hi]), L.ptr(gf[lo:hi]), L.ptr(mf[lo:hi]),
                                   L.ptr(vf[lo:hi]), L.c_f(group["lr"]), L.c_f(b1), L.c_f(b2), L.c_f(group["eps"]),
                                   L.c_f(group["weight_decay"]), L.c_i(st["step"]), L.c_f(float(grad_scale)), L.stream())
                            gf[lo:hi].zero_()
                            af[blo:bhi].fill_(1)
                            tf[blo:bhi].zero_()
                        else:
                            blocks_pending.append((bhi - blo, be, pf[lo:hi], gf[lo:hi], mf[lo:hi], vf[lo:hi], tf[blo:bhi], af[blo:bhi],
                                                   group["lr"], b1, b2, group["eps"], st["step"]))
                    if p in owned:
                        prev = 0
                        for lo, hi in sorted(ranges) + [(p.numel(), p.numel())]:
                            if lo > prev:
                                gf[prev:lo].zero_()
                                tf[prev // be:lo // be].zero_()
                            prev = max(prev, hi)
                    continue
                if p.grad is None:
                    continue
                if p.dtype != torch.float32 or not p.is_contiguous():
                    raise L.PsdfError("FusedAdamW handles contiguous fp32 parameters only")
                st = self.state[p]
                if not st:
                    st["step"] = 0
                    st["exp_avg"] = torch.zeros_like(p)
                    st["exp_avg_sq"] = torch.zeros_like(p)
                st["step"] += 1
                g = p.grad if p.grad.is_contiguous() else p.grad.contiguous()
                if p in owned:
                    pf, gf, mf, vf = p.view(-1), g.view(-1), st["exp_avg"].view(-1), st["exp_avg_sq"].view(-1)
                    for lo, hi in owned[p]:
                        if lo % 4 or hi % 4:
                            raise L.PsdfError("owned ranges must be aligned to 4 elements")
                        L.call("psdf_adamw_step", L.c_l(hi - lo), L.ptr(pf[lo:hi]), L.ptr(gf[lo:hi]), L.ptr(mf[lo:hi]),
                               L.ptr(vf[lo:hi]), L.c_f(group["lr"]), L.c_f(b1), L.c_f(b2), L.c_f(group["eps"]),
                               L.c_f(group["weight_decay"]), L.c_i(st["step"]), L.c_f(float(grad_scale)), L.stream())
                    continue
                c = small_cache.get(p)
                if c is None or c[1] is not st["exp_avg"] or c[2] is not st["exp_avg_sq"] or c[3] != p.data_ptr():
                    c = small_cache[p] = (p.numel() < self.SMALL
                                          and all(t.data_ptr() % 16 == 0 for t in (p, st["exp_avg"], st["exp_avg_sq"])),
                                          st["exp_avg"], st["exp_avg_sq"], p.data_ptr())
                small_ok = c[0]
                if small_ok and g.data_ptr() % 16 == 0:
                    small.setdefault(st["step"], []).append((p, g, st["exp_avg"], st["exp_avg_sq"]))
                    continue
                L.call("psdf_adamw_step", L.c_l(p.numel()), L.ptr(p), L.ptr(g), L.ptr(st["exp_avg"]), L.ptr(st["exp_avg_sq"]),
                       L.c_f(group["lr"]), L.c_f(b1), L.c_f(b2), L.c_f(group["eps"]), L.c_f(group["weight_decay"]),
                       L.c_i(st["step"]), L.c_f(float(grad_scale)), L.stream())
            for step, items in small.items():
                for i in range(0, len(items), 64):
                    chunk = items[i:i + 64]
                    n = len(chunk)
                    sizes = (ctypes.c_int64 * n)(*[c[0].numel() for c in chunk])
                    arrs = [(ctypes.c_void_p * n)(*[c[k].data_ptr() for c in chunk]) for k in range(4)]
                    L.call("psdf_adamw_step_multi", L.c_i(n), sizes, *arrs, L.c_f(group["lr"]), L.c_f(b1), L.c_f(b2),
                           L.c_f(group["eps"]), L.c_f(group["weight_decay"]), L.c_i(step), L.c_f(float(grad_scale)),
                           L.stream())
        for i in range(0, len(blocks_pending), 8):
            chunk = blocks_pending[i:i + 8]
            n = len(chunk)
            if n == 1:
                c = chunk[0]
                L.call("psdf_adamw_step_blocks", L.c_l(c[0]), L.c_i(c[1]), L.ptr(c[2]), L.ptr(c[3]), L.ptr(c[4]), L.ptr(c[5]),
                       L.ptr(c[6]), L.ptr(c[7]), L.c_f(c[8]), L.c_f(c[9]), L.c_f(c[10]), L.c_f(c[11]), L.c_i(c[12]),
                       L.c_f(float(grad_scale)), L.c_i(1), L.stream())
                continue
            nb = (ctypes.c_int64 * n)(*[c[0] for c in chunk])
            be = (ctypes.c_int * n)(*[c[1] for c in chunk])
            ptrs = [(ctypes.c_void_p * n)(*[c[k].data_ptr() for c in chunk]) for k in range(2, 8)]
            fl = [(ctypes.c_float * n)(*[float(c[k]) for c in chunk]) for k in range(8, 12)]
            steps = (ctypes.c_int * n)(*[int(c[12]) for c in chunk])
            L.call("psdf_adamw_step_blocks_multi", L.c_i(n), nb, be, *ptrs, *fl, steps, L.c_f(float(grad_scale)), L.c_i(1),
                   L.stream())
```

Baseline: 1.048 billion.

## Hand over composite dy max to MLP backward and merge small launches

```diff
diff --git a/include/psdf.h b/include/psdf.h
--- a/include/psdf.h
+++ b/include/psdf.h
@@ -54,6 +54,11 @@
     const float* grad_pred, const float* grad_bg, const float* sdf, const float* dirs, const float* gradients, const float* dt,
     const float* rgb, const float* inv_s, float cos_anneal_ratio, int reference_compat, float* grad_sdf, float* grad_gradients,
     float* grad_rgb, float* grad_inv_s, void* stream);
+int psdf_neus_composite_dymax_words(int nr_rays);
+int psdf_neus_composite_backward_dymax(int nr_rays, const int* start_end, int equal, int fixed, int max_nr_samples,
+    int max_per_ray, const float* grad_pred, const float* grad_bg, const float* sdf, const float* dirs, const float* gradients,
+    const float* dt, const float* rgb, const float* inv_s, float cos_anneal_ratio, int reference_compat, float* grad_sdf,
+    float* grad_gradients, float* grad_rgb, float* grad_inv_s, uint32_t* dy_wg_max, int* n_max, void* stream);
 
 int psdf_nerf_composite_forward(int nr_rays, const int* start_end, int equal, int fixed, int max_nr_samples, const float* raw_density,
                                 const float* dt, const float* rgb, const float* fg_pred, const float* fg_bg, float* pred_bg,
@@ -83,6 +88,9 @@
     const float* const* biases, const float* dY, float* dX, float* const* dW, float* const* db, void* stream);
 int psdf_mlp_backward_split_f16_form(void);
 unsigned psdf_mlp_f16_range_events(void);
+int psdf_mlp_backward_dymax(int n_layers, const int* dims, int64_t N, const float* X, const float* const* weights,
+    const float* const* biases, const float* dY, float* dX, float* const* dW, float* const* db, const uint32_t* dy_max, int n_max,
+    int zero_grads, void* stream);
 
 int psdf_mlp_forward_wide_f16(int n_layers, const int* dims, int64_t N, const float* X, const float* const* weights,
     const float* const* biases, float* Y, void* stream);
diff --git a/permuto_sdf_amd/csrc/composite_fused.hip b/permuto_sdf_amd/csrc/composite_fused.hip
--- a/permuto_sdf_amd/csrc/composite_fused.hip
+++ b/permuto_sdf_amd/csrc/composite_fused.hip
@@ -54,10 +54,11 @@
                               const float* __restrict__ sdf, const float* __restrict__ dirs, const float* __restrict__ gradients,
                               const float* __restrict__ dt, const float* __restrict__ rgb, const float* __restrict__ inv_s_ptr,
                               float cos_anneal_ratio, int compat, float* __restrict__ g_sdf, float* __restrict__ g_gradients,
-                              float* __restrict__ g_rgb, float* __restrict__ g_inv_s) {
+                              float* __restrict__ g_rgb, float* __restrict__ g_inv_s, uint32_t* __restrict__ dy_wg_max) {
   const int lane = lane_id();
   const float inv_s = inv_s_ptr[0], rr = cos_anneal_ratio;
   float gs_acc = 0.f;
+  uint32_t dmax = 0u;
   RAY_LOOP(ray, nr_rays) {
     int s, e;
     ri.get(ray, s, e);
@@ -66,6 +67,7 @@
     if (n > 64 * K) {
       poison_ray(s, n, lane, [&](int64_t m, float bad) {
         g_sdf[m] = bad;
+        dmax = max(dmax, __float_as_uint(bad) & 0x7FFFFFFFu);
         if (g_rgb) g_rgb[3 * m] = g_rgb[3 * m + 1] = g_rgb[3 * m + 2] = bad;
         if (g_gradients) st3(g_gradients + 3 * m, mk3(bad, bad, bad));
       });
@@ -112,6 +114,7 @@
         const SectionGrad sg = section_backward(sc, g_alpha, d, inv_s, rr);
         gs_acc += sg.g_inv_s;
         g_sdf[m] = sg.g_sdf;
+        dmax = max(dmax, __float_as_uint(sg.g_sdf) & 0x7FFFFFFFu);
         if (g_gradients) st3(g_gradients + 3 * m, sg.g_tc * dir);
       }
     }
@@ -119,6 +122,19 @@
   if (g_inv_s) {
     gs_acc = wave_sum(gs_acc);
     if (lane == 0 && gs_acc != 0.f) atomicAdd(g_inv_s, gs_acc);
+  }
+  if (dy_wg_max) {
+#pragma unroll
+    for (int o = 32; o > 0; o >>= 1) dmax = max(dmax, (uint32_t)__shfl_xor((int)dmax, o, 64));
+    __shared__ uint32_t wave_max[PSDF_BLOCK / 64];
+    if (lane == 0) wave_max[threadIdx.x >> 6] = dmax;
+    __syncthreads();
+    if (threadIdx.x == 0) {
+      uint32_t q = wave_max[0];
+#pragma unroll
+      for (int w = 1; w < PSDF_BLOCK / 64; w++) q = max(q, wave_max[w]);
+      dy_wg_max[blockIdx.x] = q;
+    }
   }
 }
 
@@ -289,11 +305,11 @@
   return PSDF_OK;
 }
 
-int psdf_neus_composite_backward(int nr_rays, const int* start_end, int equal, int fixed, int max_nr_samples, int max_per_ray,
-                                 const float* grad_pred, const float* grad_bg, const float* sdf, const float* dirs,
-                                 const float* gradients, const float* dt, const float* rgb, const float* inv_s,
-                                 float cos_anneal_ratio, int reference_compat, float* grad_sdf, float* grad_gradients,
-                                 float* grad_rgb, float* grad_inv_s, void* stream) {
+static int neus_composite_backward_impl(int nr_rays, const int* start_end, int equal, int fixed, int max_nr_samples, int max_per_ray,
+                                        const float* grad_pred, const float* grad_bg, const float* sdf, const float* dirs,
+                                        const float* gradients, const float* dt, const float* rgb, const float* inv_s,
+                                        float cos_anneal_ratio, int reference_compat, float* grad_sdf, float* grad_gradients,
+                                        float* grad_rgb, float* grad_inv_s, uint32_t* dy_wg_max, void* stream) {
   if (nr_rays <= 0) return PSDF_OK;
   if (!grad_pred || !sdf || !dirs || !gradients || !dt || !rgb || !inv_s || !grad_sdf || (!equal && !start_end) || max_per_ray < 1)
     return PSDF_ERR_ARG;
@@ -302,10 +318,34 @@
   dispatch_chunks(max_per_ray, [&](auto k) {
     hipLaunchKernelGGL(neus_composite_bwd_kernel<decltype(k)::value>, dim3(ray_grid(nr_rays)), dim3(PSDF_BLOCK), 0,
                        (hipStream_t)stream, nr_rays, ri, grad_pred, grad_bg, sdf, dirs, gradients, dt, rgb, inv_s,
-                       cos_anneal_ratio, reference_compat, grad_sdf, grad_gradients, grad_rgb, grad_inv_s);
+                       cos_anneal_ratio, reference_compat, grad_sdf, grad_gradients, grad_rgb, grad_inv_s, dy_wg_max);
   });
   PSDF_LAUNCH_CHECK();
   return PSDF_OK;
 }
 
-}
+int psdf_neus_composite_backward(int nr_rays, const int* start_end, int equal, int fixed, int max_nr_samples, int max_per_ray,
+                                 const float* grad_pred, const float* grad_bg, const float* sdf, const float* dirs,
+                                 const float* gradients, const float* dt, const float* rgb, const float* inv_s,
+                                 float cos_anneal_ratio, int reference_compat, float* grad_sdf, float* grad_gradients,
+                                 float* grad_rgb, float* grad_inv_s, void* stream) {
+  return neus_composite_backward_impl(nr_rays, start_end, equal, fixed, max_nr_samples, max_per_ray, grad_pred, grad_bg, sdf, dirs,
+                                      gradients, dt, rgb, inv_s, cos_anneal_ratio, reference_compat, grad_sdf, grad_gradients,
+                                      grad_rgb, grad_inv_s, nullptr, stream);
+}
+
+int psdf_neus_composite_dymax_words(int nr_rays) { return nr_rays <= 0 ? 0 : (int)ray_grid(nr_rays); }
+
+int psdf_neus_composite_backward_dymax(int nr_rays, const int* start_end, int equal, int fixed, int max_nr_samples, int max_per_ray,
+                                       const float* grad_pred, const float* grad_bg, const float* sdf, const float* dirs,
+                                       const float* gradients, const float* dt, const float* rgb, const float* inv_s,
+                                       float cos_anneal_ratio, int reference_compat, float* grad_sdf, float* grad_gradients,
+                                       float* grad_rgb, float* grad_inv_s, uint32_t* dy_wg_max, int* n_max, void* stream) {
+  if (!dy_wg_max || !n_max) return PSDF_ERR_ARG;
+  *n_max = psdf_neus_composite_dymax_words(nr_rays);
+  return neus_composite_backward_impl(nr_rays, start_end, equal, fixed, max_nr_samples, max_per_ray, grad_pred, grad_bg, sdf, dirs,
+                                      gradients, dt, rgb, inv_s, cos_anneal_ratio, reference_compat, grad_sdf, grad_gradients,
+                                      grad_rgb, grad_inv_s, dy_wg_max, stream);
+}
+
+}
diff --git a/permuto_sdf_amd/csrc/mlp.hip b/permuto_sdf_amd/csrc/mlp.hip
--- a/permuto_sdf_amd/csrc/mlp.hip
+++ b/permuto_sdf_amd/csrc/mlp.hip
@@ -12,8 +12,7 @@
   const float* b[MAXL];
 };
 
-__global__ void mlp_pack_kernel(PackArgs a, float* __restrict__ packed) {
-  const int e = blockIdx.x * blockDim.x + threadIdx.x;
+__device__ __forceinline__ void pack_float(const PackArgs& a, int e, float* __restrict__ packed) {
   const MlpPlan& p = a.plan;
   if (e >= p.total) return;
   int l = 0;
@@ -47,9 +46,11 @@
   }
   packed[e] = v;
 }
-
-__global__ void mlp_pack_split_kernel(PackArgs a, SplitPlan sp, float* __restrict__ packed, int f16) {
-  const int w = blockIdx.x * blockDim.x + threadIdx.x;
+__global__ void mlp_pack_kernel(PackArgs a, float* __restrict__ packed) {
+  pack_float(a, blockIdx.x * blockDim.x + threadIdx.x, packed);
+}
+
+__device__ __forceinline__ void pack_split_word(const PackArgs& a, const SplitPlan& sp, int w, float* __restrict__ packed, int f16) {
   const MlpPlan& p = a.plan;
   if (w >= sp.total_rec * 4) return;
   uint32_t* dst = reinterpret_cast<uint32_t*>(packed + sp.base);
@@ -95,6 +96,13 @@
     out |= pc[piece] << (16 * e);
   }
   dst[w] = out;
+}
+__global__ void mlp_pack_split_kernel(PackArgs a, SplitPlan sp, float* __restrict__ packed, int f16) {
+  pack_split_word(a, sp, blockIdx.x * blockDim.x + threadIdx.x, packed, f16);
+}
+__global__ void mlp_pack_both_kernel(PackArgs a, SplitPlan sp, int blocks_f32, float* __restrict__ packed, int f16) {
+  if ((int)blockIdx.x < blocks_f32) pack_float(a, blockIdx.x * blockDim.x + threadIdx.x, packed);
+  else pack_split_word(a, sp, (blockIdx.x - blocks_f32) * blockDim.x + threadIdx.x, packed, f16);
 }
 
 template <int T1, int T2, int T3>
@@ -521,11 +529,19 @@
     a.W[l] = l < n_layers ? weights[l] : nullptr;
     a.b[l] = l < n_layers ? biases[l] : nullptr;
   }
+  SplitPlan sp;
+  make_split_plan(a.plan, sp);
+  static const bool two_launches = [] { const char* v = getenv("PSDF_MLP_PACK_TWO_LAUNCHES"); return v && v[0] == '1'; }();
+  if (sp.ok && !two_launches) {
+    const unsigned blocks_f32 = psdf_blocks(a.plan.total, 256);
+    hipLaunchKernelGGL(mlp_pack_both_kernel, dim3(blocks_f32 + psdf_blocks(sp.total_rec * 4, 256)), dim3(256), 0,
+                       (hipStream_t)stream, a, sp, (int)blocks_f32, packed, f16);
+    PSDF_LAUNCH_CHECK();
+    return PSDF_OK;
+  }
   hipLaunchKernelGGL(mlp_pack_kernel, dim3(psdf_blocks(a.plan.total, 256)), dim3(256), 0, (hipStream_t)stream, a,
                      packed);
   PSDF_LAUNCH_CHECK();
-  SplitPlan sp;
-  make_split_plan(a.plan, sp);
   if (sp.ok) {
     hipLaunchKernelGGL(mlp_pack_split_kernel, dim3(psdf_blocks(sp.total_rec * 4, 256)), dim3(256), 0,
                        (hipStream_t)stream, a, sp, packed, f16);
diff --git a/permuto_sdf_amd/csrc/mlp_bwd.hip b/permuto_sdf_amd/csrc/mlp_bwd.hip
--- a/permuto_sdf_amd/csrc/mlp_bwd.hip
+++ b/permuto_sdf_amd/csrc/mlp_bwd.hip
@@ -1166,6 +1166,22 @@
 }
 }
 
+namespace psdf {
+int mlp_backward_split_f16_dymax(int n_layers, const int* dims, int64_t N, const float* X, const float* const* weights,
+                                 const float* const* biases, const float* dY, float* dX, float* const* dW, float* const* db,
+                                 const uint32_t* dy_max, int n_max, int zero_grads, void* stream);
+}
+namespace {
+struct ZeroArgs {
+  float* p[2 * MAXL];
+  int n[2 * MAXL];
+};
+__global__ void mlp_zero_grads_kernel(ZeroArgs z) {
+  const int i = blockIdx.x * blockDim.x + threadIdx.x;
+  if (i < z.n[blockIdx.y]) z.p[blockIdx.y][i] = 0.f;
+}
+}
+
 #ifdef PSDF_BWD_TIMING
 extern "C" int psdf_debug_bwd_timing(unsigned long long* out) {
   return (int)hipMemcpyFromSymbol(out, HIP_SYMBOL(g_bwd_t), sizeof(unsigned long long) * 8);
@@ -1249,6 +1265,42 @@
   psdf::g_last_path[psdf::PATH_MLP_BWD] = 3;
   if (dW) return psdf_mlp_backward_wide(n_layers, dims, N, X, weights, biases, dY, dX, dW, db, stream);
   return PSDF_ERR_UNSUPPORTED;
+}
+
+int psdf_mlp_backward_dymax(int n_layers, const int* dims, int64_t N, const float* X, const float* const* weights,
+                            const float* const* biases, const float* dY, float* dX, float* const* dW, float* const* db,
+                            const uint32_t* dy_max, int n_max, int zero_grads, void* stream) {
+  if ((dy_max != nullptr) != (n_max > 0) || n_max < 0) return PSDF_ERR_ARG;
+  Plan16 p;
+  const int rc = make_plan16(n_layers, dims, p);
+  if (rc != PSDF_OK) return rc;
+  if (N < 0 || !X || !weights || !biases || ((dW == nullptr) != (db == nullptr)) || (!dY && dW)) return PSDF_ERR_ARG;
+  const char* v = getenv("PSDF_MLP_BWD_SPLIT");
+  const int which = !v ? PSDF_MLP_BWD_SPLIT_DEFAULT : (v[0] == '0' ? 0 : (v[0] == 'f' ? 2 : 1));
+  if (which == 2 && dW && N > 0) {
+    const int r = psdf::mlp_backward_split_f16_dymax(n_layers, dims, N, X, weights, biases, dY, dX, dW, db, dy_max, n_max,
+                                                     zero_grads, stream);
+    if (r != PSDF_ERR_UNSUPPORTED) {
+      psdf::g_last_path[psdf::PATH_MLP_BWD] = 4;
+      return r;
+    }
+  }
+  if (zero_grads && dW) {
+    ZeroArgs z;
+    int most = 0;
+    for (int l = 0; l < MAXL; l++) {
+      const bool on = l < n_layers;
+      if (on && (!dW[l] || !db[l])) return PSDF_ERR_ARG;
+      z.p[l] = on ? dW[l] : nullptr;
+      z.p[MAXL + l] = on ? db[l] : nullptr;
+      z.n[l] = on ? dims[l + 1] * dims[l] : 0;
+      z.n[MAXL + l] = on ? dims[l + 1] : 0;
+      most = z.n[l] > most ? z.n[l] : most;
+    }
+    hipLaunchKernelGGL(mlp_zero_grads_kernel, dim3(psdf_blocks(most, 256), 2 * MAXL), dim3(256), 0, (hipStream_t)stream, z);
+    PSDF_LAUNCH_CHECK();
+  }
+  return psdf_mlp_backward(n_layers, dims, N, X, weights, biases, dY, dX, dW, db, stream);
 }
 
 int psdf_last_path(int family) {
diff --git a/permuto_sdf_amd/csrc/mlp_bwd_split.hip b/permuto_sdf_amd/csrc/mlp_bwd_split.hip
--- a/permuto_sdf_amd/csrc/mlp_bwd_split.hip
+++ b/permuto_sdf_amd/csrc/mlp_bwd_split.hip
@@ -384,16 +384,6 @@
   }
 }
 
-__device__ __forceinline__ void split3(float x, uint16_t (&p)[3]) {
-  float r = x;
-#pragma unroll
-  for (int i = 0; i < 3; i++) {
-    const uint32_t u = __float_as_uint(r);
-    p[i] = (uint16_t)(u >> 16);
-    r -= __uint_as_float(u & 0xFFFF0000u);
-  }
-}
-
 template <int NT0>
 __global__ void mlp_split_pack_kernel(int K0, const float* __restrict__ W0, const float* __restrict__ W1,
                                       const float* __restrict__ W2, const float* __restrict__ W3,
@@ -401,37 +391,7 @@
                                       const float* __restrict__ b2, const float* __restrict__ b3, uint16_t* __restrict__ rec,
                                       const uint32_t* __restrict__ only_if) {
   if (only_if && only_if[0] == 0u) return;
-  const int t = blockIdx.x * blockDim.x + threadIdx.x;
-  constexpr int PER_IMG = NT * 2 * 64, PER_T0 = NT0 * 2 * 64, NTHR = 5 * PER_IMG + PER_T0;
-  if (t < NTHR) {
-    const int im = t < 5 * PER_IMG ? t / PER_IMG : 5;
-    const int q = t - im * PER_IMG;
-    const int lane = q & 63, s = (q >> 6) & 1, tile = q >> 7;
-    const int c = lane & 15, g = lane >> 4, row = 16 * tile + c;
-    const int off[6] = {IMG::OFF_W0, IMG::OFF_W1, IMG::OFF_W2, IMG::OFF_T2, IMG::OFF_T1, IMG::OFF_T0};
-    uint16_t out[3][8];
-#pragma unroll
-    for (int j = 0; j < 8; j++) {
-      const float w = image_weight(im, row, s, g, j, K0, W0, W1, W2);
-      uint16_t p[3];
-      split3(w, p);
-      out[0][j] = p[0]; out[1][j] = p[1]; out[2][j] = p[2];
-    }
-#pragma unroll
-    for (int piece = 0; piece < 3; piece++) {
-      uint16_t* dst = rec + ((size_t)(off[im] + ((tile * 2 + s) * 3 + piece) * 64 + lane)) * 8;
-#pragma unroll
-      for (int j = 0; j < 8; j++) dst[j] = out[piece][j];
-    }
-  } else {
-    const int e = t - NTHR;
-    float* tail = reinterpret_cast<float*>(rec + (size_t)IMG::off_f32(NT0) * 8);
-    if (e < HID) tail[e] = b0[e];
-    else if (e < 2 * HID) tail[e] = b1[e - HID];
-    else if (e < 3 * HID) tail[e] = b2[e - 2 * HID];
-    else if (e < 4 * HID) tail[e] = W3[e - 3 * HID];
-    else if (e == 4 * HID) tail[e] = b3[0];
-  }
+  split_pack_item_bf16<NT0>(blockIdx.x * blockDim.x + threadIdx.x, K0, W0, W1, W2, W3, b0, b1, b2, b3, rec);
 }
 
 }
@@ -442,7 +402,7 @@
 size_t mlp_backward_split_scratch_bytes(int K0, int64_t N);
 int mlp_backward_split_impl(int n_layers, const int* dims, int64_t N, const float* X, const float* const* weights,
                             const float* const* biases, const float* dY, float* dX, float* const* dW, float* const* db,
-                            hipStream_t st, char* scratch, const uint32_t* only_if);
+                            hipStream_t st, char* scratch, const uint32_t* only_if, bool image_ready);
 }
 #if defined(PSDF_SPLIT_TU_DOUBLE)
 int psdf::mlp_bwd_split_launch_double(unsigned blocks, size_t lds_bytes, hipStream_t st, int64_t N, int K0, int rows4,
@@ -462,7 +422,7 @@
 int psdf_mlp_backward_split(int n_layers, const int* dims, int64_t N, const float* X, const float* const* weights,
                             const float* const* biases, const float* dY, float* dX, float* const* dW, float* const* db,
                             void* stream) {
-  return psdf::mlp_backward_split_impl(n_layers, dims, N, X, weights, biases, dY, dX, dW, db, (hipStream_t)stream, nullptr, nullptr);
+  return psdf::mlp_backward_split_impl(n_layers, dims, N, X, weights, biases, dY, dX, dW, db, (hipStream_t)stream, nullptr, nullptr, false);
 }
 
 }
@@ -472,7 +432,8 @@
 }
 int psdf::mlp_backward_split_impl(int n_layers, const int* dims, int64_t N, const float* X, const float* const* weights,
                                   const float* const* biases, const float* dY, float* dX, float* const* dW, float* const* db,
-                                  hipStream_t st, char* scratch, const uint32_t* only_if) {
+                                  hipStream_t st, char* scratch, const uint32_t* only_if, bool image_ready) {
+  if (image_ready && (!only_if || !scratch)) return PSDF_ERR_ARG;
   const int rc0 = split_check(n_layers, dims, 52 , N, X, weights, biases, dY, dW, db);
   if (rc0 != PSDF_OK) return rc0;
   const int K0 = dims[0];
@@ -491,6 +452,7 @@
   float* partial = reinterpret_cast<float*>(scratch + img_bytes);
   const int pack_threads = (5 * NT + nt0) * 2 * 64 + TAIL_FLOATS;
 #define PACK(NT0_)                                                                                                         \
+  if (!image_ready)                                                                                                        \
   hipLaunchKernelGGL(mlp_split_pack_kernel<NT0_>, dim3((pack_threads + 255) / 256), dim3(256), 0, st, K0, weights[0],        \
                      weights[1], weights[2], weights[3], biases[0], biases[1], biases[2], biases[3], rec, only_if)
 #define MAIN(NT0_, DBL_)                                                                                                    \
diff --git a/permuto_sdf_amd/csrc/mlp_bwd_split_f16.hip b/permuto_sdf_amd/csrc/mlp_bwd_split_f16.hip
--- a/permuto_sdf_amd/csrc/mlp_bwd_split_f16.hip
+++ b/permuto_sdf_amd/csrc/mlp_bwd_split_f16.hip
@@ -459,14 +459,25 @@
   for (int e = threadIdx.x; e < G_TOTAL; e += NWAVES * 64) dst[e] = G[e];
 }
 
+struct RedoImage {
+  const float *W0, *W1, *W2, *W3, *b0, *b1, *b2, *b3;
+  uint16_t* rec;
+  int nt0;
+};
 __global__ void mlp_split_reduce_kernel(const float* __restrict__ partial, const uint32_t* __restrict__ absmax, int nimg, int K0, float* __restrict__ dW0,
                                         float* __restrict__ dW1, float* __restrict__ dW2, float* __restrict__ dW3,
                                         float* __restrict__ db0, float* __restrict__ db1, float* __restrict__ db2,
-                                        float* __restrict__ db3, int guard_drops, volatile uint32_t* events) {
+                                        float* __restrict__ db3, int guard_drops, volatile uint32_t* events, RedoImage redo) {
   const int e = blockIdx.x * blockDim.x + threadIdx.x;
   if (absmax[1]) {
     if (events && e == 0 && blockIdx.y == 0) events[0] = events[0] + 1u;
-    if (guard_drops) return;
+    if (guard_drops) {
+      if (blockIdx.y == 0) {
+        if (redo.nt0 == 3) split_pack_item_bf16<3>(e, K0, redo.W0, redo.W1, redo.W2, redo.W3, redo.b0, redo.b1, redo.b2, redo.b3, redo.rec);
+        else split_pack_item_bf16<4>(e, K0, redo.W0, redo.W1, redo.W2, redo.W3, redo.b0, redo.b1, redo.b2, redo.b3, redo.rec);
+      }
+      return;
+    }
   }
   if (e >= G_TOTAL) return;
   float s = 0.f;
@@ -525,47 +536,131 @@
 }
 
 template <int NT0>
+struct PackItems {
+  static constexpr int PER_IMG = NT * 2 * 64, PER_T0 = NT0 * 2 * 64, RECORDS = 5 * PER_IMG + PER_T0, ITEMS = RECORDS + TAIL_FLOATS;
+};
+template <int NT0>
+__device__ __forceinline__ void record_weights(int t, int K0, const float* __restrict__ W0, const float* __restrict__ W1,
+                                               const float* __restrict__ W2, float (&w)[8]) {
+  using P = PackItems<NT0>;
+  const int im = t < 5 * P::PER_IMG ? t / P::PER_IMG : 5;
+  const int q = t - im * P::PER_IMG;
+  const int lane = q & 63, s = (q >> 6) & 1, tile = q >> 7;
+  const int c = lane & 15, g = lane >> 4, row = 16 * tile + c;
+#pragma unroll
+  for (int j = 0; j < 8; j++) w[j] = image_weight(im, row, s, g, j, K0, W0, W1, W2);
+}
+template <int NT0, class Raise>
+__device__ __forceinline__ void record_store(int t, const float (&w)[8], uint32_t* __restrict__ rec, Raise&& raise) {
+  using P = PackItems<NT0>;
+  const int im = t < 5 * P::PER_IMG ? t / P::PER_IMG : 5;
+  const int q = t - im * P::PER_IMG;
+  const int lane = q & 63, s = (q >> 6) & 1, tile = q >> 7;
+  const int off[6] = {IMG::OFF_W0, IMG::OFF_W1, IMG::OFF_W2, IMG::OFF_T2, IMG::OFF_T1, IMG::OFF_T0};
+  u32x4 hi, lo;
+  float wmax = 0.f;
+#pragma unroll
+  for (int i = 0; i < 4; i++) {
+    uint32_t h, l;
+    split2(w[2 * i], w[2 * i + 1], h, l);
+    hi[i] = h;
+    lo[i] = l;
+    wmax = __builtin_fmaxf(__builtin_fmaxf(wmax, __builtin_fabsf(w[2 * i])), __builtin_fabsf(w[2 * i + 1]));
+  }
+  if (wmax >= 65504.f) raise();
+  u32x4* dst = reinterpret_cast<u32x4*>(rec) + (off[im] + ((tile * 2 + s) * NP) * 64 + lane);
+  dst[0] = hi;
+  dst[64] = lo;
+}
+template <int NT0, class Raise>
+__device__ __forceinline__ void tail_item(int e, const float* __restrict__ W3, const float* __restrict__ b0,
+                                          const float* __restrict__ b1, const float* __restrict__ b2,
+                                          const float* __restrict__ b3, uint32_t* __restrict__ rec, Raise&& raise) {
+  float* tail = reinterpret_cast<float*>(rec + (size_t)IMG::off_f32(NT0) * 4);
+  if (e < HID) tail[e] = b0[e];
+  else if (e < 2 * HID) tail[e] = b1[e - HID];
+  else if (e < 3 * HID) tail[e] = b2[e - 2 * HID];
+  else if (e < 4 * HID) {
+    tail[e] = W3[e - 3 * HID];
+    if (__builtin_fabsf(W3[e - 3 * HID]) >= W4_LIMIT) raise();
+  }
+  else if (e == 4 * HID) tail[e] = b3[0];
+}
+template <int NT0, class Raise>
+__device__ __forceinline__ void split_pack_item(int t, int K0, const float* __restrict__ W0, const float* __restrict__ W1,
+                                                const float* __restrict__ W2, const float* __restrict__ W3,
+                                                const float* __restrict__ b0, const float* __restrict__ b1,
+                                                const float* __restrict__ b2, const float* __restrict__ b3,
+                                                uint32_t* __restrict__ rec, Raise&& raise) {
+  if (t < PackItems<NT0>::RECORDS) {
+    float w[8];
+    record_weights<NT0>(t, K0, W0, W1, W2, w);
+    record_store<NT0>(t, w, rec, raise);
+  } else {
+    tail_item<NT0>(t - PackItems<NT0>::RECORDS, W3, b0, b1, b2, b3, rec, raise);
+  }
+}
+
+template <int NT0>
 __global__ void mlp_split_pack_kernel(int K0, const float* __restrict__ W0, const float* __restrict__ W1,
                                       const float* __restrict__ W2, const float* __restrict__ W3,
                                       const float* __restrict__ b0, const float* __restrict__ b1,
                                       const float* __restrict__ b2, const float* __restrict__ b3, uint32_t* __restrict__ rec,
                                       uint32_t* __restrict__ absmax) {
-  const int t = blockIdx.x * blockDim.x + threadIdx.x;
-  constexpr int PER_IMG = NT * 2 * 64, PER_T0 = NT0 * 2 * 64, NTHR = 5 * PER_IMG + PER_T0;
-  if (t < NTHR) {
-    const int im = t < 5 * PER_IMG ? t / PER_IMG : 5;
-    const int q = t - im * PER_IMG;
-    const int lane = q & 63, s = (q >> 6) & 1, tile = q >> 7;
-    const int c = lane & 15, g = lane >> 4, row = 16 * tile + c;
-    const int off[6] = {IMG::OFF_W0, IMG::OFF_W1, IMG::OFF_W2, IMG::OFF_T2, IMG::OFF_T1, IMG::OFF_T0};
-    float w[8];
-#pragma unroll
-    for (int j = 0; j < 8; j++) w[j] = image_weight(im, row, s, g, j, K0, W0, W1, W2);
-    u32x4 hi, lo;
-    float wmax = 0.f;
-#pragma unroll
-    for (int i = 0; i < 4; i++) {
-      uint32_t h, l;
-      split2(w[2 * i], w[2 * i + 1], h, l);
-      hi[i] = h;
-      lo[i] = l;
-      wmax = __builtin_fmaxf(__builtin_fmaxf(wmax, __builtin_fabsf(w[2 * i])), __builtin_fabsf(w[2 * i + 1]));
-    }
-    if (wmax >= 65504.f) atomicOr(absmax + 1, 1u);
-    u32x4* dst = reinterpret_cast<u32x4*>(rec) + (off[im] + ((tile * 2 + s) * NP) * 64 + lane);
-    dst[0] = hi;
-    dst[64] = lo;
-  } else {
-    const int e = t - NTHR;
-    float* tail = reinterpret_cast<float*>(rec + (size_t)IMG::off_f32(NT0) * 4);
-    if (e < HID) tail[e] = b0[e];
-    else if (e < 2 * HID) tail[e] = b1[e - HID];
-    else if (e < 3 * HID) tail[e] = b2[e - 2 * HID];
-    else if (e < 4 * HID) {
-      tail[e] = W3[e - 3 * HID];
-      if (__builtin_fabsf(W3[e - 3 * HID]) >= W4_LIMIT) atomicOr(absmax + 1, 1u);
-    }
-    else if (e == 4 * HID) tail[e] = b3[0];
+  split_pack_item<NT0>(blockIdx.x * blockDim.x + threadIdx.x, K0, W0, W1, W2, W3, b0, b1, b2, b3, rec,
+                       [&] { atomicOr(absmax + 1, 1u); });
+}
+
+constexpr int PREPARE_THREADS = 1024;
+struct ZeroList {
+  float* p[8];
+  int n[8];
+};
+template <int NT0>
+__global__ void __launch_bounds__(PREPARE_THREADS)
+    mlp_split_prepare_kernel(int K0, const float* __restrict__ W0, const float* __restrict__ W1, const float* __restrict__ W2,
+                             const float* __restrict__ W3, const float* __restrict__ b0, const float* __restrict__ b1,
+                             const float* __restrict__ b2, const float* __restrict__ b3, uint32_t* __restrict__ rec,
+                             uint32_t* __restrict__ absmax, const uint32_t* __restrict__ dy_max, int n_max, ZeroList zero) {
+  __shared__ uint32_t guard, wave_max[PREPARE_THREADS / 64];
+  if (threadIdx.x == 0) guard = 0u;
+  __syncthreads();
+  using P = PackItems<NT0>;
+  constexpr int ROUNDS = (P::RECORDS + PREPARE_THREADS - 1) / PREPARE_THREADS;
+  const auto raise = [&] { guard = 1u; };
+  float w[ROUNDS][8];
+#pragma unroll
+  for (int r = 0; r < ROUNDS; r++) {
+    const int t = threadIdx.x + r * PREPARE_THREADS;
+    if (t < P::RECORDS) record_weights<NT0>(t, K0, W0, W1, W2, w[r]);
+  }
+  uint32_t m = 0u;
+  if (dy_max)
+    for (int i = threadIdx.x; i < n_max; i += 4 * PREPARE_THREADS) {
+      uint32_t v[4];
+#pragma unroll
+      for (int u = 0; u < 4; u++) v[u] = i + u * PREPARE_THREADS < n_max ? dy_max[i + u * PREPARE_THREADS] : 0u;
+      m = max(max(m, max(v[0], v[1])), max(v[2], v[3]));
+    }
+#pragma unroll
+  for (int k = 0; k < 8; k++)
+    for (int i = threadIdx.x; i < zero.n[k]; i += PREPARE_THREADS) zero.p[k][i] = 0.f;
+  if (threadIdx.x < TAIL_FLOATS) tail_item<NT0>(threadIdx.x, W3, b0, b1, b2, b3, rec, raise);
+#pragma unroll
+  for (int r = 0; r < ROUNDS; r++) {
+    const int t = threadIdx.x + r * PREPARE_THREADS;
+    if (t < P::RECORDS) record_store<NT0>(t, w[r], rec, raise);
+  }
+#pragma unroll
+  for (int o = 32; o > 0; o >>= 1) m = max(m, (uint32_t)__shfl_xor((int)m, o, 64));
+  if ((threadIdx.x & 63) == 0) wave_max[threadIdx.x >> 6] = m;
+  __syncthreads();
+  if (threadIdx.x == 0) {
+    uint32_t q = wave_max[0];
+#pragma unroll
+    for (int k = 1; k < PREPARE_THREADS / 64; k++) q = max(q, wave_max[k]);
+    absmax[0] = q;
+    absmax[1] = guard;
   }
 }
 
@@ -576,7 +671,7 @@
 size_t mlp_backward_split_scratch_bytes(int K0, int64_t N);
 int mlp_backward_split_impl(int n_layers, const int* dims, int64_t N, const float* X, const float* const* weights,
                             const float* const* biases, const float* dY, float* dX, float* const* dW, float* const* db,
-                            hipStream_t st, char* scratch, const uint32_t* only_if);
+                            hipStream_t st, char* scratch, const uint32_t* only_if, bool image_ready);
 }
 static uint32_t g_range_warned = 0;
 static volatile uint32_t* range_events() {
@@ -596,9 +691,9 @@
 
 int psdf_mlp_backward_split_f16_form(void) { return g_f16_form; }
 
-int psdf_mlp_backward_split_f16(int n_layers, const int* dims, int64_t N, const float* X, const float* const* weights,
-                                const float* const* biases, const float* dY, float* dX, float* const* dW, float* const* db,
-                                void* stream) {
+static int split_f16_impl(int n_layers, const int* dims, int64_t N, const float* X, const float* const* weights,
+                          const float* const* biases, const float* dY, float* dX, float* const* dW, float* const* db,
+                          const uint32_t* dy_max, int n_max, int zero_grads, void* stream) {
   const int rc0 = split_check(n_layers, dims, 64, N, X, weights, biases, dY, dW, db);
   if (rc0 != PSDF_OK) return rc0;
   const int K0 = dims[0];
@@ -627,8 +722,20 @@
                       "three-piece bf16 kernel (slower); PSDF_MLP_BWD_SPLIT=bf16 selects it outright\n");
     g_range_warned = events[0];
   }
-  if (hipMemsetAsync(absmax, 0, 16, st) != hipSuccess) return PSDF_ERR_UNSUPPORTED;
+  static const bool two_step = [] { const char* v = getenv("PSDF_MLP_F16_PREPARE"); return v && v[0] == '0'; }();
+  const bool prepare = !two_step || dy_max || zero_grads;
+  if (!prepare && hipMemsetAsync(absmax, 0, 16, st) != hipSuccess) return PSDF_ERR_UNSUPPORTED;
   const int pack_threads = (5 * NT + nt0) * 2 * 64 + TAIL_FLOATS;
+  ZeroList zero;
+  for (int l = 0; l < 4; l++) {
+    zero.p[l] = dW[l];
+    zero.p[4 + l] = db[l];
+    zero.n[l] = zero_grads ? dims[l + 1] * dims[l] : 0;
+    zero.n[4 + l] = zero_grads ? dims[l + 1] : 0;
+  }
+#define PREPARE(NT0_)                                                                                                      \
+  hipLaunchKernelGGL(mlp_split_prepare_kernel<NT0_>, dim3(1), dim3(PREPARE_THREADS), 0, st, K0, weights[0], weights[1],      \
+                     weights[2], weights[3], biases[0], biases[1], biases[2], biases[3], rec, absmax, dy_max, n_max, zero)
 #define PACK(NT0_)                                                                                                         \
   hipLaunchKernelGGL(mlp_split_pack_kernel<NT0_>, dim3((pack_threads + 255) / 256), dim3(256), 0, st, K0, weights[0],        \
                      weights[1], weights[2], weights[3], biases[0], biases[1], biases[2], biases[3], rec, absmax)
@@ -640,24 +747,39 @@
     hipLaunchKernelGGL(kern, dim3((unsigned)blocks), dim3(NWAVES * 64), lds_bytes, st, N, K0, rows4, X, dY,                  \
                        reinterpret_cast<const u32x4*>(rec), absmax, dX, partial);                                           \
   } while (0)
-  if (nt0 == 3) PACK(3); else PACK(4);
-  {
+  if (prepare) {
+    if (nt0 == 3) PREPARE(3); else PREPARE(4);
+  } else {
+    if (nt0 == 3) PACK(3); else PACK(4);
+  }
+  if (!dy_max) {
     int64_t ab = ((N >> 2) + 1023) / 1024;
     ab = ab < 1 ? 1 : (ab > 512 ? 512 : ab);
     hipLaunchKernelGGL(mlp_absmax_kernel, dim3((unsigned)ab), dim3(256), 0, st, N, dY, absmax);
   }
   if (nt0 == 3) MAIN(3); else MAIN(4);
 #undef PACK
+#undef PREPARE
 #undef MAIN
+  char* fb_scratch = scratch + img_bytes + 16 + part_bytes;
+  const RedoImage redo{weights[0], weights[1], weights[2], weights[3], biases[0], biases[1], biases[2], biases[3],
+                       reinterpret_cast<uint16_t*>(fb_scratch), nt0};
+  static_assert((G_TOTAL + 255) / 256 * 256 >= (5 * NT + 4) * 2 * 64 + TAIL_FLOATS, "the reduce grid's first row covers the image's items");
   hipLaunchKernelGGL(mlp_split_reduce_kernel, dim3((G_TOTAL + 255) / 256, 16), dim3(256), 0, st, partial, absmax, (int)blocks, K0,
-                     dW[0], dW[1], dW[2], dW[3], db[0], db[1], db[2], db[3], guarded ? 1 : 0, events);
+                     dW[0], dW[1], dW[2], dW[3], db[0], db[1], db[2], db[3], guarded ? 1 : 0, events, redo);
   PSDF_LAUNCH_CHECK();
   if (guarded) {
-    const int rc = psdf::mlp_backward_split_impl(n_layers, dims, N, X, weights, biases, dY, dX, dW, db, st,
-                                                 scratch + img_bytes + 16 + part_bytes, absmax + 1);
+    const int rc = psdf::mlp_backward_split_impl(n_layers, dims, N, X, weights, biases, dY, dX, dW, db, st, fb_scratch,
+                                                 absmax + 1, true);
     if (rc != PSDF_OK) return rc;
   }
   return PSDF_OK;
+}
+
+int psdf_mlp_backward_split_f16(int n_layers, const int* dims, int64_t N, const float* X, const float* const* weights,
+                                const float* const* biases, const float* dY, float* dX, float* const* dW, float* const* db,
+                                void* stream) {
+  return split_f16_impl(n_layers, dims, N, X, weights, biases, dY, dX, dW, db, nullptr, 0, 0, stream);
 }
 
 unsigned psdf_mlp_f16_range_events(void) {
@@ -666,3 +788,11 @@
 }
 
 }
+
+namespace psdf {
+int mlp_backward_split_f16_dymax(int n_layers, const int* dims, int64_t N, const float* X, const float* const* weights,
+                                 const float* const* biases, const float* dY, float* dX, float* const* dW, float* const* db,
+                                 const uint32_t* dy_max, int n_max, int zero_grads, void* stream) {
+  return split_f16_impl(n_layers, dims, N, X, weights, biases, dY, dX, dW, db, dy_max, n_max, zero_grads, stream);
+}
+}
diff --git a/permuto_sdf_amd/csrc/mlp_split_layout.h b/permuto_sdf_amd/csrc/mlp_split_layout.h
--- a/permuto_sdf_amd/csrc/mlp_split_layout.h
+++ b/permuto_sdf_amd/csrc/mlp_split_layout.h
@@ -69,6 +69,53 @@
     default: return row < K0 ? W0[kc * K0 + row] : 0.f;
   }
 }
+__device__ __forceinline__ void split3(float x, uint16_t (&p)[3]) {
+  float r = x;
+#pragma unroll
+  for (int i = 0; i < 3; i++) {
+    const uint32_t u = __float_as_uint(r);
+    p[i] = (uint16_t)(u >> 16);
+    r -= __uint_as_float(u & 0xFFFF0000u);
+  }
+}
+template <int NT0>
+__device__ __forceinline__ void split_pack_item_bf16(int t, int K0, const float* __restrict__ W0, const float* __restrict__ W1,
+                                                     const float* __restrict__ W2, const float* __restrict__ W3,
+                                                     const float* __restrict__ b0, const float* __restrict__ b1,
+                                                     const float* __restrict__ b2, const float* __restrict__ b3,
+                                                     uint16_t* __restrict__ rec) {
+  using I3 = SplitImage<3>;
+  constexpr int PER_IMG = NT * 2 * 64, PER_T0 = NT0 * 2 * 64, NTHR = 5 * PER_IMG + PER_T0;
+  if (t < NTHR) {
+    const int im = t < 5 * PER_IMG ? t / PER_IMG : 5;
+    const int q = t - im * PER_IMG;
+    const int lane = q & 63, s = (q >> 6) & 1, tile = q >> 7;
+    const int c = lane & 15, g = lane >> 4, row = 16 * tile + c;
+    const int off[6] = {I3::OFF_W0, I3::OFF_W1, I3::OFF_W2, I3::OFF_T2, I3::OFF_T1, I3::OFF_T0};
+    uint16_t out[3][8];
+#pragma unroll
+    for (int j = 0; j < 8; j++) {
+      const float w = image_weight(im, row, s, g, j, K0, W0, W1, W2);
+      uint16_t p[3];
+      split3(w, p);
+      out[0][j] = p[0]; out[1][j] = p[1]; out[2][j] = p[2];
+    }
+#pragma unroll
+    for (int piece = 0; piece < 3; piece++) {
+      uint16_t* dst = rec + ((size_t)(off[im] + ((tile * 2 + s) * 3 + piece) * 64 + lane)) * 8;
+#pragma unroll
+      for (int j = 0; j < 8; j++) dst[j] = out[piece][j];
+    }
+  } else if (t < NTHR + TAIL_FLOATS) {
+    const int e = t - NTHR;
+    float* tail = reinterpret_cast<float*>(rec + (size_t)I3::off_f32(NT0) * 8);
+    if (e < HID) tail[e] = b0[e];
+    else if (e < 2 * HID) tail[e] = b1[e - HID];
+    else if (e < 3 * HID) tail[e] = b2[e - 2 * HID];
+    else if (e < 4 * HID) tail[e] = W3[e - 3 * HID];
+    else tail[e] = b3[0];
+  }
+}
 
 inline int64_t split_blocks(int64_t N) {
   const int64_t ntiles = (N + 15) / 16;
diff --git a/permuto_sdf_amd/csrc/optim.hip b/permuto_sdf_amd/csrc/optim.hip
--- a/permuto_sdf_amd/csrc/optim.hip
+++ b/permuto_sdf_amd/csrc/optim.hip
@@ -53,6 +53,8 @@
 
 constexpr int ADAMW_MAX_TENSORS = 64;
 struct AdamwMulti {
+  int n_tensors;
+  int first_block[ADAMW_MAX_TENSORS + 1];
   int64_t n[ADAMW_MAX_TENSORS];
   float* p[ADAMW_MAX_TENSORS];
   const float* g[ADAMW_MAX_TENSORS];
@@ -62,9 +64,12 @@
 __global__ void __launch_bounds__(PSDF_BLOCK)
     adamw_multi_kernel(AdamwMulti a, float lr, float beta1, float beta2, float eps, float weight_decay, float bias_corr1,
                        float bias_corr2_sqrt, float grad_scale) {
-  const int t = blockIdx.y;
+  int t = 0;
+  for (int i = 1; i < a.n_tensors; i++)
+    if ((int)blockIdx.x >= a.first_block[i]) t = i;
+  const int b = blockIdx.x - a.first_block[t], nb = a.first_block[t + 1] - a.first_block[t];
   adamw_range(a.n[t], a.p[t], a.g[t], a.m[t], a.v[t], lr, beta1, beta2, eps, weight_decay, bias_corr1, bias_corr2_sqrt,
-              grad_scale, ((int64_t)blockIdx.x * PSDF_BLOCK + threadIdx.x) * 4, (int64_t)gridDim.x * PSDF_BLOCK * 4);
+              grad_scale, ((int64_t)b * PSDF_BLOCK + threadIdx.x) * 4, (int64_t)nb * PSDF_BLOCK * 4);
 }
 __device__ __forceinline__ void adamw_blocks_body(int64_t n_blocks, int block_elems, float* __restrict__ p, float* __restrict__ g,
                         float* __restrict__ m, float* __restrict__ v, unsigned char* __restrict__ touched,
@@ -203,7 +208,8 @@
   if (n_tensors > ADAMW_MAX_TENSORS || !sizes || !params || !grads || !exp_avgs || !exp_avg_sqs || step < 1)
     return PSDF_ERR_ARG;
   AdamwMulti a;
-  int64_t nmax = 0;
+  a.n_tensors = n_tensors;
+  a.first_block[0] = 0;
   for (int t = 0; t < n_tensors; t++) {
     if (sizes[t] < 0 || !params[t] || !grads[t] || !exp_avgs[t] || !exp_avg_sqs[t]) return PSDF_ERR_ARG;
     if ((((uintptr_t)params[t] | (uintptr_t)grads[t] | (uintptr_t)exp_avgs[t] | (uintptr_t)exp_avg_sqs[t]) & 15) != 0)
@@ -213,15 +219,16 @@
     a.g[t] = grads[t];
     a.m[t] = exp_avgs[t];
     a.v[t] = exp_avg_sqs[t];
-    if (sizes[t] > nmax) nmax = sizes[t];
-  }
+    unsigned blocks = psdf_blocks((sizes[t] + 3) / 4, PSDF_BLOCK);
+    if (blocks > 4096u) blocks = 4096u;
+    a.first_block[t + 1] = a.first_block[t] + (int)blocks;
+  }
+  if (a.first_block[n_tensors] == 0) return PSDF_OK;
   const float bc1 = 1.f - powf(beta1, (float)step);
   const float bc2 = sqrtf(1.f - powf(beta2, (float)step));
-  unsigned blocks = psdf_blocks((nmax + 3) / 4, PSDF_BLOCK);
-  if (blocks > 64u) blocks = 64u;
-  hipLaunchKernelGGL(adamw_multi_kernel, dim3(blocks, (unsigned)n_tensors), dim3(PSDF_BLOCK), 0, (hipStream_t)stream, a, lr,
-                     beta1, beta2, eps, weight_decay, bc1, bc2, grad_scale);
-  PSDF_LAUNCH_CHECK();
-  return PSDF_OK;
-}
-}
+  hipLaunchKernelGGL(adamw_multi_kernel, dim3((unsigned)a.first_block[n_tensors]), dim3(PSDF_BLOCK), 0, (hipStream_t)stream, a,
+                     lr, beta1, beta2, eps, weight_decay, bc1, bc2, grad_scale);
+  PSDF_LAUNCH_CHECK();
+  return PSDF_OK;
+}
+}
diff --git a/permuto_sdf_amd/hotpath.py b/permuto_sdf_amd/hotpath.py
--- a/permuto_sdf_amd/hotpath.py
+++ b/permuto_sdf_amd/hotpath.py
@@ -30,6 +30,8 @@
         self.events = None
         self.fuse_compositing = True
         self.want_rgb_grad = True
+        self.fold_min_samples = 1 << 18
+        self.dy_handover = True
         import os
         self.fwd_f16 = os.environ.get("PSDF_MLP_FWD_SPLIT", "f16") != "bf16"
         self.shard_optimizer = parallel.sharded_optimizer_default()
@@ -70,10 +72,15 @@
     def backward(self, rs, rgb_samples, saved, grad_pred, reduce=True, optimizer_step=True, split_levels=None):
         cfg = self.enc.cfg
         N = rs.samples_pos.shape[0]
+        folded = N >= self.fold_min_samples
+        dy_max = None
         if "fused_per_ray" in saved:
-            g_sdf, _, g_rgb, _ = neus_composite_backward_raw(rs, saved["fused_per_ray"], grad_pred, None, saved["sdf"].view(-1, 1),
-                                                             saved["normals"], rgb_samples, self.inv_s, self.cos_anneal_ratio,
-                                                             need_grad=False, need_rgb=self.want_rgb_grad, need_inv_s=False)
+            handover = folded and self.dy_handover
+            res = neus_composite_backward_raw(rs, saved["fused_per_ray"], grad_pred, None, saved["sdf"].view(-1, 1),
+                                              saved["normals"], rgb_samples, self.inv_s, self.cos_anneal_ratio, need_grad=False,
+                                              need_rgb=self.want_rgb_grad, need_inv_s=False, want_dy_max=handover)
+            g_sdf, g_rgb = res[0], res[2]
+            dy_max = res[4] if handover else None
             g_om = g_alpha = None
         else:
             g_rgb, g_w = VR.integrate_with_weights_backward(grad_pred, rs, rgb_samples, saved["w"], None)
@@ -89,7 +96,8 @@
         if self.events is not None:
             self.events["mlp_bwd"][0].record()
         d_feat, dWs, dbs = mlp_backward_raw(self.mlp.dims, saved["feat"], [l.weight for l in self.mlp.layers],
-                                            [l.bias for l in self.mlp.layers], grad_sdf, need_dx=True)
+                                            [l.bias for l in self.mlp.layers], grad_sdf, need_dx=True, dy_max=dy_max,
+                                            folded=folded)
         if self.events is not None:
             self.events["mlp_bwd"][1].record()
         buckets = parallel.GradientBuckets()
diff --git a/permuto_sdf_amd/mlp.py b/permuto_sdf_amd/mlp.py
--- a/permuto_sdf_amd/mlp.py
+++ b/permuto_sdf_amd/mlp.py
@@ -109,6 +109,11 @@
     return flat, dWs, dbs
 
 
+def _grad_floats(dims):
+    n_layers = len(dims) - 1
+    return sum((sz + 3) & ~3 for sz in [dims[l + 1] * dims[l] for l in range(n_layers)] + [dims[l + 1] for l in range(n_layers)])
+
+
 def _zero_grads(dims, dev):
     _, dWs, dbs = _grad_views(dims, dev=dev)
     return dWs, dbs
@@ -128,8 +133,10 @@
         self.flat.zero_()
 
 
-def mlp_backward_raw(dims, x_fm, weights, biases, gy_fm, need_dx=True, need_dw=True, into=None, dx=None):
+def mlp_backward_raw(dims, x_fm, weights, biases, gy_fm, need_dx=True, need_dw=True, into=None, dx=None, dy_max=None,
+                     folded=False):
     assert gy_fm is not None or not need_dw
+    folded = (folded or dy_max is not None) and need_dw
     N = x_fm.shape[1]
     n_layers = len(dims) - 1
     dev = x_fm.device
@@ -144,11 +151,23 @@
     Wp = (ctypes.c_void_p * n_layers)(*[w.data_ptr() for w in ws])
     Bp = (ctypes.c_void_p * n_layers)(*[b.data_ptr() for b in bs])
     if need_dw:
-        dWs, dbs = into if into is not None else _zero_grads(dims, dev)
+        if into is not None:
+            dWs, dbs = into
+        elif folded:
+            _, dWs, dbs = _grad_views(dims, flat=torch.empty(_grad_floats(dims), dtype=torch.float32, device=dev))
+        else:
+            dWs, dbs = _zero_grads(dims, dev)
         W = (ctypes.c_void_p * n_layers)(*[w.data_ptr() for w in dWs])
         B = (ctypes.c_void_p * n_layers)(*[b.data_ptr() for b in dbs])
     else:
         dWs, dbs, W, B = [], [], None, None
+    if folded:
+        if dy_max is not None:
+            assert dy_max.dtype == torch.int32 and dy_max.is_contiguous() and dy_max.device == dev and dy_max.numel() > 0
+        L.call("psdf_mlp_backward_dymax", L.c_i(n_layers), _dims_array(dims), L.c_l(N), L.ptr(x_fm), Wp, Bp, L.ptr(gy_fm),
+               L.ptr(dx), W, B, L.ptr(dy_max), L.c_i(0 if dy_max is None else dy_max.numel()), L.c_i(int(into is None)),
+               L.stream())
+        return dx, dWs, dbs
     L.call("psdf_mlp_backward", L.c_i(n_layers), _dims_array(dims), L.c_l(N), L.ptr(x_fm), Wp, Bp, L.ptr(gy_fm),
            L.ptr(dx), W, B, L.stream())
     return dx, dWs, dbs
diff --git a/permuto_sdf_amd/neus.py b/permuto_sdf_amd/neus.py
--- a/permuto_sdf_amd/neus.py
+++ b/permuto_sdf_amd/neus.py
@@ -65,10 +65,28 @@
 
 
 def neus_composite_backward_raw(rs, max_per_ray, g_pred, g_bg, sdf, gradients, rgb, inv_s, cos_anneal_ratio, need_grad=True,
-                                need_rgb=True, need_inv_s=True):
+                                need_rgb=True, need_inv_s=True, want_dy_max=False):
     from .bridge import VolumeRendering, _per_sample
     N, dev = sdf.shape[0], sdf.device
     g_sdf = _per_sample(rs, (N, 1), dev)
+    if want_dy_max:
+        ri = rs._ri()
+        n_words = int(L.lib().psdf_neus_composite_dymax_words(ri[0])) if _covers_every_sample(rs, N) else 0
+        if n_words == 0:
+            return neus_composite_backward_raw(rs, max_per_ray, g_pred, g_bg, sdf, gradients, rgb, inv_s, cos_anneal_ratio,
+                                               need_grad, need_rgb, need_inv_s) + (None,)
+        import ctypes
+        g_grad = _per_sample(rs, (N, 3), dev) if need_grad else None
+        g_rgb = _per_sample(rs, (N, 3), dev) if need_rgb else None
+        g_inv_s = L.zeroed_scalar(dev) if need_inv_s else None
+        dy_max = torch.empty(n_words, dtype=torch.int32, device=dev)
+        n_max = ctypes.c_int(0)
+        L.call("psdf_neus_composite_backward_dymax", *ri, L.c_i(int(max_per_ray)), L.ptr(g_pred), L.ptr(g_bg), L.ptr(sdf),
+               L.ptr(rs.samples_dirs), L.ptr(gradients), L.ptr(rs.samples_dt), L.ptr(rgb), L.ptr(inv_s),
+               L.c_f(float(cos_anneal_ratio)), L.c_i(int(VolumeRendering.reference_compat)), L.ptr(g_sdf), L.ptr(g_grad),
+               L.ptr(g_rgb), L.ptr(g_inv_s), L.ptr(dy_max), ctypes.byref(n_max), L.stream())
+        assert n_max.value == n_words
+        return g_sdf, g_grad, g_rgb, g_inv_s, dy_max
     g_grad = _per_sample(rs, (N, 3), dev) if need_grad else None
     g_rgb = _per_sample(rs, (N, 3), dev) if need_rgb else None
     g_inv_s = L.zeroed_scalar(dev) if need_inv_s else None
@@ -77,6 +95,11 @@
            L.c_f(float(cos_anneal_ratio)), L.c_i(int(VolumeRendering.reference_compat)), L.ptr(g_sdf), L.ptr(g_grad),
            L.ptr(g_rgb), L.ptr(g_inv_s), L.stream())
     return g_sdf, g_grad, g_rgb, g_inv_s
+
+
+def _covers_every_sample(rs, N):
+    return bool(rs.rays_have_equal_nr_of_samples and N > 0 and
+                rs.fixed_nr_of_samples_per_ray * rs.ray_start_end_idx.shape[0] == N and rs.max_nr_samples >= N)
 
 
 FUSED_MAX_PER_RAY = 256
diff --git a/permuto_sdf_amd/optim.py b/permuto_sdf_amd/optim.py
--- a/permuto_sdf_amd/optim.py
+++ b/permuto_sdf_amd/optim.py
@@ -9,6 +9,7 @@
         self.generation = 0
 
     SMALL = 1 << 16
+    ONE_LAUNCH = True
 
     def attach(self, param, touched_rows):
         if not hasattr(self, "_touched"):
@@ -134,10 +135,9 @@
                     continue
                 c = small_cache.get(p)
                 if c is None or c[1] is not st["exp_avg"] or c[2] is not st["exp_avg_sq"] or c[3] != p.data_ptr():
-                    c = small_cache[p] = (p.numel() < self.SMALL
-                                          and all(t.data_ptr() % 16 == 0 for t in (p, st["exp_avg"], st["exp_avg_sq"])),
+                    c = small_cache[p] = (all(t.data_ptr() % 16 == 0 for t in (p, st["exp_avg"], st["exp_avg_sq"])),
                                           st["exp_avg"], st["exp_avg_sq"], p.data_ptr())
-                small_ok = c[0]
+                small_ok = c[0] and (self.ONE_LAUNCH or p.numel() < self.SMALL)
                 if small_ok and g.data_ptr() % 16 == 0:
                     small.setdefault(st["step"], []).append((p, g, st["exp_avg"], st["exp_avg_sq"]))
                     continue
```

New measurement: 1.043 billion. No clear change (-0.5%).
